# cboin1996/avddpg

Measured on AMD Instinct MI355X. Metric: env-steps/sec + DDPG updates/sec, 4096x5-vehicle platoons, higher is better.
Workload: dtype f32-class (fp16 hi+lo operand pairs on the 16-bit matrix cores, f32 accumulate)

## Files before the change

avddpg_amd/_hip.py:

```python
import ctypes as C
import os

_HERE = os.path.dirname(os.path.abspath(__file__))
LIB_PATH = os.path.join(_HERE, "lib", "libavddpg_hip.so")
if os.environ.get("AVDDPG_HIP_LIB"):
    LIB_PATH = os.path.abspath(os.environ["AVDDPG_HIP_LIB"])
HEADER_PATH = os.path.join(os.path.dirname(_HERE), "include", "avddpg_hip.h")
AVD_MAX_L = 16
AVD_EVAL_NMETRIC = 8


class AvdError(RuntimeError):
    pass


class EnvConsts(C.Structure):
    _fields_ = [("L", C.c_int32), ("model_a", C.c_int32), ("can_terminate", C.c_int32), ("uniform_reset", C.c_int32),
                ("max_ep", C.c_float), ("max_ev", C.c_float), ("abs_action_high", C.c_float),
                ("two_max_a", C.c_float), ("T", C.c_float),
                ("ca", C.c_float), ("cb", C.c_float), ("cc", C.c_float), ("cd", C.c_float),
                ("re_scalar", C.c_float), ("terminal_reward", C.c_float),
                ("stand_still", C.c_float), ("timegap", C.c_float),
                ("reset_ep_max", C.c_float), ("reset_max_ev", C.c_float), ("reset_max_a", C.c_float),
                ("reset_ep_eval", C.c_float), ("reset_ev_eval", C.c_float), ("reset_a_eval", C.c_float),
                ("leader_reset_a", C.c_float),
                ("A", (C.c_float * 16) * AVD_MAX_L), ("B", (C.c_float * 4) * AVD_MAX_L),
                ("C", (C.c_float * 4) * AVD_MAX_L)]


class HParams(C.Structure):
    _fields_ = [("actor_lr", C.c_float), ("critic_lr", C.c_float), ("tau", C.c_float), ("one_minus_tau", C.c_float),
                ("gamma", C.c_float), ("ou_theta", C.c_float), ("ou_scale", C.c_float), ("reserved", C.c_float)]


_LAYOUT_FIELDS = ["S", "A", "H1", "H2", "Ha", "B",
                  "aW1", "ab1", "ag1", "abe1", "aW2", "ab2", "ag2", "abe2", "aW3", "ab3", "actor_size",
                  "cWs", "cbs", "cgs", "cbes", "cWa", "cba", "cga", "cbea", "cW2", "cb2", "cg3", "cbe3", "cW3", "cb3",
                  "theta_size",
                  "amm1", "amv1", "amm2", "amv2", "cmms", "cmvs", "cmma", "cmva", "cmm3", "cmv3", "stats_size"]


class MlpLayout(C.Structure):
    _fields_ = [(n, C.c_int32) for n in _LAYOUT_FIELDS]


_P = C.c_void_p
_i, _f, _d, _u64, _i64 = C.c_int, C.c_float, C.c_double, C.c_uint64, C.c_int64
_LP = C.POINTER(MlpLayout)

_PROTOS = {
    "avd_mlp_layout_init": [_LP, _i, _i, _i, _i, _i, _i],
    "avd_env_step_f32": [_P, _i, _i, _P, _P, _P, _P, _P, _P, _P, _P, _P, _P, _P, _P],
    "avd_env_reset_f32": [_P, _i, _i, _P, _P, _P, _P, _P, _i, _u64, _u64, _P, _P],
    "avd_episode_end_f32": [_P, _i, _i, _i, _P, _P, _P, _P, _P, _P, _i, _P, _P, _P, _P, _i, _u64, _u64, _P],
    "avd_ou_step_f32": [_i, _P, _P, _f, _f, _f, _f, _u64, _u64, _P],
    "avd_policy_f32": [_i, _P, _P, _f, _f, _P, _P],
    "avd_normal_f32": [_i, _P, _f, _u64, _u64, _P],
    "avd_uniform_f32": [_i, _P, _f, _u64, _u64, _P],
    "avd_step_fused_f32": [_P, _i, _i, _i, _P, _P, _P, _P, _P, _P, _P, _P, _P, _P, _P, _P, _P, _f, _f, _f, _f, _f, _f, _f, _i, _u64, _u64,
                           _u64, _P, _i, _i64, _P, _P],
    "avd_replay_sample_f32": [_i, _i, _i, _i, _i, _P, _i, _u64, _u64, _P, _P, _P, _P, _P, _P],
    "avd_step_fused_seeds_f32": [_P, _i, _i, _i, _P, _P, _P, _P, _P, _P, _P, _P, _P, _P, _P, _P, _P, _f, _f, _f, _f, _f, _f, _f, _i, _P,
                                 _i, _u64, _u64, _P, _i, _i64, _P, _P],
    "avd_env_reset_seeds_f32": [_P, _i, _i, _P, _P, _P, _i, _P, _i, _u64, _P, _P],
    "avd_episode_end_seeds_f32": [_P, _i, _i, _i, _P, _P, _P, _P, _P, _P, _i, _P, _P, _P, _P, _i, _P, _i, _u64, _P],
    "avd_replay_sample_seeds_f32": [_i, _i, _i, _i, _i, _P, _i, _P, _i, _i, _u64, _P, _P, _P, _P, _P, _P],
    "avd_step_fused_hp_f32": [_P, _i, _i, _i, _P, _P, _P, _P, _P, _P, _P, _P, _P, _P, _P, _P, _P, _f, _f, _f, _f, _f, _i, _P, _P, _i,
                              _u64, _u64, _P, _i, _i64, _P, _P],
    "avd_learn_hp_f32": [_LP, _i, _i, _P, _P, _P, _P, _P, _P, _P, _P, _f, _P, _P, _P, _i, _i, _P],
    "avd_learn_update_hp_f32": [_LP, _i, _P, _P, _P, _P, _P, _P, _P, _P, _P, _P, _P, _P, _f, _P, _P, _P, _i, _i, _P],
    "avd_learn_update_act_hp_f32": [_LP, _i, _P, _P, _P, _P, _P, _P, _P, _P, _P, _P, _P, _P, _f, _P, _P, _P, _i, _P, _P, _i, _i, _P],
    "avd_adam_polyak_hp_f32": [_LP, _i, _P, _P, _P, _P, _P, _P, _P, _P, _P, _i, _i, _P],
    "avd_adam_polyak_guarded_hp_f32": [_LP, _i, _P, _P, _P, _P, _P, _P, _P, _P, _P, _P, _i, _i, _P],
    "avd_learn_set_split_hp_f16x3": [_LP, _i, _i, _P, _P, _P, _P, _P, _P, _P, _P, _P, _f, _P, _P, _P, C.c_size_t, _P, _i, _i, _P],
    "avd_actor_forward_set_f32": [_LP, _i, _i, _P, _P, _P, _i, _f, _P, _P, _P],
    "avd_copy_experiment_sets_f32": [_LP, _i, _i, _i, _P, _i, _P, _P, _P, _P, _P, _P, _P, _P],
    "avd_replay_add_f32": [_i, _i, _i, _i, _P, _i64, _P, _P, _i, _P, _P, _P],
    "avd_replay_indices": [_i, _i, _i, _u64, _u64, _P, _P],
    "avd_replay_gather_f32": [_i, _i, _i, _i, _i, _P, _P, _P, _P, _P, _P, _P],
    "avd_actor_forward_f32": [_LP, _i, _i, _P, _P, _P, _i, _f, _P, _P],
    "avd_actor_forward_cond_f32": [_LP, _i, _i, _P, _P, _P, _i, _f, _P, _P, _P],
    "avd_critic_forward_f32": [_LP, _i, _i, _P, _P, _P, _i, _P, _P, _P],
    "avd_learn_f32": [_LP, _i, _i, _P, _P, _P, _P, _P, _P, _P, _P, _f, _f, _P, _P, _P],
    "avd_learn_check_shape": [_LP],
    "avd_learn_update_f32": [_LP, _i, _P, _P, _P, _P, _P, _P, _P, _P, _P, _P, _P, _P, _f, _f, _f, _f, _d, _P, _P, _P],
    "avd_learn_update_act_f32": [_LP, _i, _P, _P, _P, _P, _P, _P, _P, _P, _P, _P, _P, _P, _f, _f, _f, _f, _d, _P, _P, _P, _i, _P, _P],
    "avd_learn_update_plan": [_LP, _i, C.POINTER(C.c_int), C.POINTER(C.c_int), C.POINTER(C.c_int)],
    "avd_adam_polyak_f32": [_LP, _i, _P, _P, _P, _P, _P, _P, _P, _P, _f, _f, _d, _P],
    "avd_adam_polyak_guarded_f32": [_LP, _i, _P, _P, _P, _P, _P, _P, _P, _P, _f, _f, _d, _P, _P],
    "avd_polyak_f32": [_i64, _P, _P, _d, _P],
    "avd_fed_sum_f32": [_i, _i, _i, _i, _i, _P, _P, _P, _P, _P],
    "avd_fed_finalize_f32": [_i, _i, _P, _f, _P, _P],
    "avd_fed_scatter_f32": [_i, _i, _i, _i, _i, _i, _P, _P, _P],
    "avd_adam_polyak_intra_f32": [_LP, _i, _i, _i, _P, _P, _P, _P, _P, _P, _P, _P, _P, _f, _f, _d, _P],
    "avd_fed_history_push_f32": [_i, _i, _i, _P, _P, _P, _i, _P, _i, _i, _P, _P, _P],
    "avd_fed_weights_f32": [_i, _i, _i, _P, _P, _i, _P, _P, _P, _P],
    "avd_learn_shared_workspace": [_LP, _i, _i, C.POINTER(C.c_size_t)],
    "avd_learn_shared_bf16": [_LP, _i, _i, _P, _P, _P, _P, _P, _P, _P, _P, _P, _f, _f, _P, _P, _P, C.c_size_t, _P],
    "avd_learn_set_fused_workspace": [_LP, _i, _i, C.POINTER(C.c_size_t)],
    "avd_learn_set_fused_bf16": [_LP, _i, _i, _P, _P, _P, _P, _P, _P, _P, _P, _P, _f, _f, _P, _P, _P, C.c_size_t, _P],
    "avd_learn_set_split_workspace": [_LP, _i, _i, C.POINTER(C.c_size_t)],
    "avd_learn_set_split_mfma_count": [_LP, _i, _i, C.POINTER(C.c_ulonglong)],
    "avd_learn_set_split_critic": [_LP, _i, _i, _P, _P, _P, _P, _P, _P, _P, _P, _P, _f, _f, _P, _P, _P, C.c_size_t, _P],
    "avd_learn_set_split_actor": [_LP, _i, _i, _P, _P, _P, _f, _P, _P, C.c_size_t, _P],
    "avd_learn_set_split_bf16x3": [_LP, _i, _i, _P, _P, _P, _P, _P, _P, _P, _P, _P, _f, _f, _P, _P, _P, C.c_size_t, _P],
    "avd_learn_set_split_f16x3": [_LP, _i, _i, _P, _P, _P, _P, _P, _P, _P, _P, _P, _f, _f, _P, _P, _P, C.c_size_t, _P],
    "avd_actor_forward_shared_workspace": [_LP, _i, _i, C.POINTER(C.c_size_t)],
    "avd_actor_forward_shared_bf16": [_LP, _i, _i, _P, _P, _P, _f, _P, _P, C.c_size_t, _P],
    "avd_eval_rollout_f32": [_LP, _P, _i, _i, _i, _i, _P, _P, _i, _P, _P, _P, _P, _i, _P, _f, _f, _f, _f, _P, _i, _P, _P, _P, _P,
                             _P],
    "avd_eval_cases_f32": [_LP, _P, _i, _i, _i, _i, _i, _P, _P, _i, _P, _P, _P, _P, _f, _f, _f, _f, _P, _P, _P],
    "avd_eval_cases_block": [_i, _i],
    "avd_gemm_bt_bf16": [_i, _i, _i, _P, C.c_long, _P, C.c_long, _P, C.c_long, _P],
}

_lib = None
DIAG_LIB_PATH = os.path.join(_HERE, "lib", "libavddpg_hip_diag.so")


def _load(path):
    if not os.path.exists(path):
        raise AvdError(f"{path} not found: build the HIP extension first (__graft_entry__.build()); "
                       "avddpg_amd has no CPU fallback")
    l = C.CDLL(path)
    missing = []
    for name, args in _PROTOS.items():
        fn = getattr(l, name, None)
        if fn is None:
            missing.append(name)
            continue
        fn.argtypes = args
        fn.restype = C.c_int
    if missing and not os.environ.get("AVDDPG_HIP_LIB"):
        raise AvdError(f"{path} does not export {', '.join(missing)}: rebuild it (make -C avddpg_amd/csrc)")
    l.avd_last_error.restype = C.c_char_p
    l.avd_last_error.argtypes = []
    l.avd_version.restype, l.avd_version.argtypes = C.c_int, []
    if getattr(l, "avd_diagnostics_enabled", None) is None:
        l.avd_diagnostics_enabled = lambda: 0
    else:
        l.avd_diagnostics_enabled.restype, l.avd_diagnostics_enabled.argtypes = C.c_int, []
    return l


def lib():
    global _lib
    if _lib is None:
        _lib = _load(LIB_PATH)
    return _lib


class diag_library:
    _cached = None
    _stack = []

    def __enter__(self):
        global _lib, LIB_PATH
        if diag_library._cached is None:
            diag_library._cached = _load(DIAG_LIB_PATH)
            if not diag_library._cached.avd_diagnostics_enabled():
                raise AvdError(f"{DIAG_LIB_PATH} is not a diagnostic build")
        diag_library._stack.append((lib(), LIB_PATH))
        _lib, LIB_PATH = diag_library._cached, DIAG_LIB_PATH
        return _lib

    def __exit__(self, *exc):
        global _lib, LIB_PATH
        _lib, LIB_PATH = diag_library._stack.pop()
        return False


def call(name, *args):
    fn = getattr(lib(), name, None)
    if fn is None:
        raise AvdError(f"{name} is not exported by the loaded library (an older build?)")
    rc = fn(*args)
    if rc != 0:
        raise AvdError(f"{name} failed ({rc}): {lib().avd_last_error().decode()}")


def ptr(t):
    if t is None:
        return None
    if not t.is_contiguous():
        raise AvdError("non-contiguous tensor passed to the C ABI")
    return C.c_void_p(t.data_ptr())


def stream_handle():
    import torch
    return C.c_void_p(torch.cuda.current_stream().cuda_stream)


def make_layout(S, A, H1, H2, Ha, B):
    lay = MlpLayout()
    call("avd_mlp_layout_init", C.byref(lay), S, A, H1, H2, Ha, B)
    return lay
```

avddpg_amd/csrc/fsplit.hip:

```cpp
#include <type_traits>

#include "fset_common.h"

namespace avd {
namespace fsplit {
using namespace fset;

struct ActorS {
    static constexpr int K = 256, KP = 256, NFT = 8, NKS = 16, LD = 264, NGT = 9, KG = 288;
    static constexpr bool critic = false;
};
struct CriticS {
    static constexpr int K = 304, KP = 320, NFT = 10, NKS = 19, LD = 312, NGT = 10, KG = 320;
    static constexpr bool critic = true;
};
constexpr int NGT_MAX = 10;

template <int I, int N, class F>
__device__ __forceinline__ void static_for(F&& f) {
    if constexpr (I < N) {
        f(std::integral_constant<int, I>{});
        static_for<I + 1, N>(f);
    }
}

typedef _Float16 f16;
typedef _Float16 f16x2 __attribute__((ext_vector_type(2)));
typedef _Float16 f16x8 __attribute__((ext_vector_type(8)));
constexpr float S1 = 64.f;
constexpr float F16_OVERFLOW = 65520.f;
#if defined(FSPLIT_ABL_CONST)
#define FSPLIT_ABL(x) FSPLIT_ABL_CONST
#elif defined(AVD_DIAG)
#define FSPLIT_ABL(x) (x)
#else
#define FSPLIT_ABL(x) 0
#endif
__device__ __forceinline__ void split2h(float a, float b, unsigned& hi, unsigned& lo) {
    const f32x2 f = {a, b};
    const f16x2 h = __builtin_convertvector(f, f16x2);
    hi = __builtin_bit_cast(unsigned, h);
    f32x2 l;
#ifdef __HIP_DEVICE_COMPILE__
    asm("v_fma_mix_f32 %0, -%1, 1.0, %2 op_sel:[0,0,0] op_sel_hi:[1,0,0]" : "=v"(l[0]) : "v"(hi), "v"(a));
    asm("v_fma_mix_f32 %0, -%1, 1.0, %2 op_sel:[1,0,0] op_sel_hi:[1,0,0]" : "=v"(l[1]) : "v"(hi), "v"(b));
#else
    l[0] = a - (float)h[0], l[1] = b - (float)h[1];
#endif
    lo = __builtin_bit_cast(unsigned, __builtin_convertvector(l, f16x2));
}
__device__ __forceinline__ void split1h(float x, f16& hi, f16& lo) {
    hi = (f16)x;
    lo = (f16)(x - (float)hi);
}
template <class V>
__device__ __forceinline__ void pin16(V& x) {
#pragma unroll
    for (int q = 0; q < 2; ++q) {
        float a = x[8 * q], b = x[8 * q + 1], c = x[8 * q + 2], d = x[8 * q + 3], e = x[8 * q + 4], f = x[8 * q + 5], g = x[8 * q + 6], h = x[8 * q + 7];
        asm volatile("" : "+v"(a), "+v"(b), "+v"(c), "+v"(d), "+v"(e), "+v"(f), "+v"(g), "+v"(h));
        x[8 * q] = a, x[8 * q + 1] = b, x[8 * q + 2] = c, x[8 * q + 3] = d, x[8 * q + 4] = e, x[8 * q + 5] = f, x[8 * q + 6] = g, x[8 * q + 7] = h;
    }
}
__device__ __forceinline__ f16x8 fragh(unsigned a, unsigned b, unsigned c, unsigned d) {
    uint4 o;
    o.x = a, o.y = b, o.z = c, o.w = d;
    return __builtin_bit_cast(f16x8, o);
}
__device__ __forceinline__ f32x16 mfmah(f16x8 a, f16x8 b, f32x16 c) {
    return __builtin_amdgcn_mfma_f32_32x32x16_f16(a, b, c, 0, 0, 0);
}
__device__ __forceinline__ f16x8 make_xh(float x0, float x1, float x2, float x3, int h) {
    f16 a0, a1, a2, a3, l0, l1, l2, l3;
    split1h(x0, a0, l0), split1h(x1, a1, l1), split1h(x2, a2, l2), split1h(x3, a3, l3);
    const f16 one = (f16)1.f, zero = (f16)0.f;
    f16x8 v;
    v[0] = a0, v[1] = a1, v[2] = a2, v[3] = a3;
    v[4] = h ? one : l0, v[5] = h ? one : l1, v[6] = h ? zero : l2, v[7] = h ? zero : l3;
    return v;
}
__device__ __forceinline__ f16x8 make_wh(float w0, float w1, float w2, float w3, float b, float sc, int h) {
    f16 a0, a1, a2, a3, l0, l1, l2, l3, bh, bl;
    split1h(sc * w0, a0, l0), split1h(sc * w1, a1, l1), split1h(sc * w2, a2, l2), split1h(sc * w3, a3, l3), split1h(sc * b, bh, bl);
    const f16 zero = (f16)0.f;
    f16x8 v;
    v[0] = h ? l0 : a0, v[1] = h ? l1 : a1, v[2] = h ? l2 : a2, v[3] = h ? l3 : a3;
    v[4] = h ? bh : a0, v[5] = h ? bl : a1, v[6] = h ? bh : a2, v[7] = h ? zero : a3;
    return v;
}
__device__ __forceinline__ f16x8 make_xg(float x0, float x1, float x2, float x3, float g, int h) {
    f16 a0, a1, a2, a3, l0, l1, l2, l3, gh, gl;
    split1h(x0, a0, l0), split1h(x1, a1, l1), split1h(x2, a2, l2), split1h(x3, a3, l3), split1h(g, gh, gl);
    const f16 zero = (f16)0.f;
    f16x8 v;
    v[0] = a0, v[1] = a1, v[2] = a2, v[3] = a3;
    v[4] = h ? gh : l0, v[5] = h ? gh : l1, v[6] = h ? gl : l2, v[7] = h ? zero : l3;
    return v;
}

template <int S>
__device__ __forceinline__ void load_x(const float* xa, long row, float (&x)[4]) {
    if (S == 4) {
        const float4 v = *(const float4*)(xa + 4 * row);
        x[0] = v.x, x[1] = v.y, x[2] = v.z, x[3] = v.w;
    } else {
#pragma unroll
        for (int k = 0; k < 4; ++k) x[k] = k < S ? xa[S * row + k] : 0.f;
    }
}

__host__ __device__ constexpr int wpos(int f) { return (f & ~12) | ((f & 4) << 1) | ((f & 8) >> 1); }

struct NetP {
    const float* th;
    long th_stride;
    const f16* Whi;
    const f16* Wlo;
    const f16* Wchi;
    const f16* Wclo;
    const f16x8* wf1h;
    const float* vec;
    const unsigned* wap;
};

struct PackArgs {
    const float* x[2];
    const float* extra[2];
    f16x8* outh[2];
    long rows;
};
__device__ __forceinline__ void front_flag(unsigned* wave_flags, bool hit) {
    const bool any = __ballot(hit) != 0;
    if ((threadIdx.x & 63) == 0) wave_flags[threadIdx.x >> 6] = any;
}
template <int S>
__device__ __forceinline__ void pack_x_role(const PackArgs& a, int which, long bx, unsigned* wave_flags) {
    const float* x = a.x[which];
    const float* extra = a.extra[which];
    const bool extra_is_action = which == 0;
    const long i = bx * 256 + threadIdx.x;
    bool nf = false;
    if (i < 2 * a.rows) {
        float v[4];
        load_x<S>(x, i >> 1, v);
        nf = not_finite(v[0]) || not_finite(v[1]) || not_finite(v[2]) || not_finite(v[3]);
        nf = nf || fmaxf(fmaxf(fabsf(v[0]), fabsf(v[1])), fmaxf(fabsf(v[2]), fabsf(v[3]))) >= F16_OVERFLOW;
        if (!(i & 1)) {
            const float e = extra[i >> 1];
            nf = nf || not_finite(e) || (extra_is_action && fabsf(e) >= F16_OVERFLOW);
        }
        a.outh[which][i] = make_xh(v[0], v[1], v[2], v[3], (int)(i & 1));
    }
    front_flag(wave_flags, nf);
}

struct PrepArgs {
    avd_mlp_layout L;
    int S;
    const float *theta, *stats, *theta_t, *stats_t;
    f16 *Whi[4], *Wlo[4];
    f16 *Wchi[4], *Wclo[4];
    f16x8* wf1h[4];
    float* vec[4];
    unsigned* wap;
    unsigned* smax;
    int* bad;
    unsigned* fflag;
    int n_fflag;
};
constexpr int SCALE_SLICES = 16;
__device__ __forceinline__ float pow2_for(float mx) {
    int e = 0;
    if (mx > 0.f && !not_finite(mx)) (void)frexpf(mx, &e);
    int k = 13 - e;
    k = k < -14 ? -14 : (k > 30 ? 30 : k);
    return ldexpf(1.f, k);
}
__device__ __forceinline__ void scale_role(const PrepArgs& a, int net, int set, int slice, int n_sets) {
    __shared__ float red[256], red2[256], c3a[H2], inva[CriticS::K];
    const int tid = threadIdx.x;
    const bool critic = net & 1, target = net >= 2;
    const avd_mlp_layout& L = a.L;
    const float* th = (target ? a.theta_t : a.theta) + (long)set * L.theta_size + (critic ? L.actor_size : 0);
    const float* st = (target ? a.stats_t : a.stats) + (long)set * L.stats_size;
    const int K = critic ? CriticS::K : ActorS::K, oW2 = critic ? L.cW2 : L.aW2;
    const int og2 = critic ? L.cg3 : L.ag2, omv2 = critic ? L.cmv3 : L.amv2, oW3 = critic ? L.cW3 : L.aW3;
    if (tid < H2) c3a[tid] = fabsf((1.0f / sqrtf(st[omv2 + tid] + BN_EPS)) * th[og2 + tid] * th[oW3 + tid]);
    for (int f = tid; f < K; f += 256) {
        int og, omv, ff = f;
        if (!critic) og = L.ag1, omv = L.amv1;
        else if (f < H1) og = L.cgs, omv = L.cmvs;
        else og = L.cga, omv = L.cmva, ff = f - H1;
        inva[f] = fabsf((1.0f / sqrtf(st[omv + ff] + BN_EPS)) * th[og + ff]);
    }
    __syncthreads();
    const int total = K * H2, per = (total + SCALE_SLICES - 1) / SCALE_SLICES, lo = slice * per, hi = min(total, lo + per);
    float m = 0.f, m2 = 0.f;
    for (int i = lo + tid; i < hi; i += 256) {
        const float w = fabsf(th[oW2 + i]);
        m = fmaxf(m, inva[i / H2] * w);
        m2 = fmaxf(m2, c3a[i % H2] * w);
    }
    red[tid] = m, red2[tid] = m2;
    __syncthreads();
    for (int o = 128; o > 0; o >>= 1) {
        if (tid < o) red[tid] = fmaxf(red[tid], red[tid + o]), red2[tid] = fmaxf(red2[tid], red2[tid + o]);
        __syncthreads();
    }
    if (tid == 0) {
        unsigned* dst = a.smax + (((long)net * n_sets + set) * SCALE_SLICES + slice) * 2;
        dst[0] = __float_as_uint(red[0]);
        dst[1] = __float_as_uint(red2[0]);
    }
}
__global__ __launch_bounds__(320) void prep_kernel(const PrepArgs a) {
    __shared__ float red[320];
    const int n = blockIdx.x, net = blockIdx.y, set = blockIdx.z, f = threadIdx.x;
    const bool critic = net & 1, target = net >= 2;
    const avd_mlp_layout& L = a.L;
    const float* th = (target ? a.theta_t : a.theta) + (long)set * L.theta_size + (critic ? L.actor_size : 0);
    const float* st = (target ? a.stats_t : a.stats) + (long)set * L.stats_size;
    const int K = critic ? CriticS::K : ActorS::K, KP = critic ? CriticS::KP : ActorS::KP;
    const int oW2 = critic ? L.cW2 : L.aW2, ob2 = critic ? L.cb2 : L.ab2, oW3 = critic ? L.cW3 : L.aW3, ob3 = critic ? L.cb3 : L.ab3;
    const int og2 = critic ? L.cg3 : L.ag2, obe2 = critic ? L.cbe3 : L.abe2, omm2 = critic ? L.cmm3 : L.amm2, omv2 = critic ? L.cmv3 : L.amv2;
    const float inv2n = (1.0f / sqrtf(st[omv2 + n] + BN_EPS)) * th[og2 + n], c3n = inv2n * th[oW3 + n];
    const unsigned* smax = a.smax + ((long)net * gridDim.z + set) * SCALE_SLICES * 2;
    unsigned mx = 0, mxc = 0;
#pragma unroll
    for (int sl = 0; sl < SCALE_SLICES; ++sl) mx = max(mx, smax[2 * sl]), mxc = max(mxc, smax[2 * sl + 1]);
    const float SW = pow2_for(__uint_as_float(mx)), SWC = pow2_for(__uint_as_float(mxc));
    if (net == 0 && set == 0)
        for (int w = n * 320 + f; w < a.n_fflag; w += H2 * 320)
            if (a.fflag[w]) atomicOr(a.bad, 1);
    float shw = 0.f;
    if (f < KP) {
        float w = 0.f, inv = 0.f;
        if (f < K) {
            int og, obe, omm, omv, ff = f;
            if (!critic) og = L.ag1, obe = L.abe1, omm = L.amm1, omv = L.amv1;
            else if (f < H1) og = L.cgs, obe = L.cbes, omm = L.cmms, omv = L.cmvs;
            else og = L.cga, obe = L.cbea, omm = L.cmma, omv = L.cmva, ff = f - H1;
            inv = (1.0f / sqrtf(st[omv + ff] + BN_EPS)) * th[og + ff];
            const float sh = th[obe + ff] - st[omm + ff] * inv;
            w = th[oW2 + (long)f * H2 + n];
            shw = sh * w;
            if (not_finite(w) || not_finite(inv) || not_finite(sh)) atomicOr(a.bad, 1);
            f16 hi, lo;
            const float ws = SW * (inv * w);
            if (fabsf(ws) >= F16_OVERFLOW) atomicOr(a.bad, 1);
            split1h(ws, hi, lo);
            const long at = ((long)set * H2 + n) * K + wpos(f);
            a.Whi[net][at] = hi, a.Wlo[net][at] = lo;
        }
        if (!target) {
            f16 hi, lo;
            const float wc = SWC * (c3n * w);
            if (fabsf(wc) >= F16_OVERFLOW) atomicOr(a.bad, 1);
            split1h(wc, hi, lo);
            const long at = ((long)set * KP + f) * H2 + n;
            a.Wchi[net][at] = hi, a.Wclo[net][at] = lo;
        }
    }
    red[f] = shw;
    __syncthreads();
    if (f < 64) red[f] += red[f + 256];
    __syncthreads();
    for (int o = 128; o > 0; o >>= 1) {
        if (f < o) red[f] += red[f + o];
        __syncthreads();
    }
    float* vec = a.vec[net] + (long)set * VEC;
    if (f == 0) {
        if (n == 0) vec[2 * H2 + 1] = SW, vec[2 * H2 + 2] = SWC;
        vec[n] = th[ob2 + n] + red[0];
        vec[H2 + n] = c3n;
        if (not_finite(vec[n]) || not_finite(c3n) || not_finite(th[ob3])) atomicOr(a.bad, 1);
    }
    if (n == 0) {
        __syncthreads();
        float v = 0.f;
        if (f < H2) {
            const float inv2 = (1.0f / sqrtf(st[omv2 + f] + BN_EPS)) * th[og2 + f];
            v = (th[obe2 + f] - st[omm2 + f] * inv2) * th[oW3 + f];
        }
        red[f] = v;
        __syncthreads();
        for (int o = 64; o > 0; o >>= 1) {
            if (f < o) red[f] += red[f + o];
            __syncthreads();
        }
        if (f == 0) vec[2 * H2] = th[ob3] + red[0];
    }
}
__device__ __forceinline__ bool prep1_role(const PrepArgs& a, int ft, int net, int set, int lane) {
    const int r = lane & 31, h = lane >> 5;
    bool hit = false;
    const bool critic = net & 1, target = net >= 2;
    const avd_mlp_layout& L = a.L;
    const float* th = (target ? a.theta_t : a.theta) + (long)set * L.theta_size + (critic ? L.actor_size : 0);
    const int K = critic ? CriticS::K : ActorS::K;
    const int f = 32 * ft + r;
    float w[4] = {0.f, 0.f, 0.f, 0.f}, b = 0.f;
    if (f == K) {
        b = 1.f;
    } else if (f < K) {
        if (critic && ft >= 8) {
            w[0] = th[L.cWa + (f - H1)], b = th[L.cba + (f - H1)];
        } else {
            const float* W = th + (critic ? L.cWs : L.aW1);
#pragma unroll
            for (int k = 0; k < 4; ++k) w[k] = k < a.S ? W[k * H1 + f] : 0.f;
            b = th[(critic ? L.cbs : L.ab1) + f];
        }
        if (not_finite(w[0]) || not_finite(w[1]) || not_finite(w[2]) || not_finite(w[3]) || not_finite(b)) hit = true;
        if (S1 * fmaxf(fmaxf(fabsf(w[0]), fabsf(w[1])), fmaxf(fmaxf(fabsf(w[2]), fabsf(w[3])), fabsf(b))) >= F16_OVERFLOW) hit = true;
    }
    a.wf1h[net][((long)set * NGT_MAX + ft) * 64 + lane] = make_wh(w[0], w[1], w[2], w[3], b, S1, h);
    if (net == 1 && ft == 0 && lane < 48) {
        const int hl = lane / 24, hh = (lane / 12) & 1, ks = (lane / 4) % 3, m = lane & 3;
        unsigned v = 0;
#pragma unroll
        for (int e = 0; e < 2; ++e) {
            const int jj = 2 * m + e, fa = 16 * ks + 8 * (jj >> 2) + 4 * hh + (jj & 3);
            f16 hi, lo;
            split1h(S1 * th[L.cWa + fa], hi, lo);
            v |= (unsigned)__builtin_bit_cast(unsigned short, hl ? lo : hi) << (16 * e);
        }
        a.wap[(long)set * 48 + lane] = v;
    }
    return hit;
}

struct FrontArgs {
    PrepArgs pa;
    PackArgs pk;
    float* grads;
    long n_grads;
    int n_sets, n_scale, n_prep1, n_zero, n_pack;
};
constexpr int ZERO_PER_BLOCK = 4096;
template <int S>
__global__ __launch_bounds__(256) void front_kernel(const FrontArgs a) {
    int b = blockIdx.x;
    if (b < a.n_scale) {
        scale_role(a.pa, b & 3, (b >> 2) % a.n_sets, (b >> 2) / a.n_sets, a.n_sets);
        return;
    }
    b -= a.n_scale;
    if (b < a.n_prep1) {
        const int q = 4 * b + (threadIdx.x >> 6);
        bool hit = false;
        if (q < NGT_MAX * 4 * a.n_sets) hit = prep1_role(a.pa, q % NGT_MAX, (q / NGT_MAX) & 3, q / (NGT_MAX * 4), threadIdx.x & 63);
        front_flag(a.pa.fflag + 4 * (long)b, hit);
        return;
    }
    b -= a.n_prep1;
    if (b < a.n_zero) {
        if (b == 0 && threadIdx.x == 0) *a.pa.bad = 0;
        const long base = (long)b * ZERO_PER_BLOCK + threadIdx.x;
#pragma unroll
        for (int k = 0; k < ZERO_PER_BLOCK / 256; ++k)
            if (base + 256 * k < a.n_grads) a.grads[base + 256 * k] = 0.f;
        return;
    }
    b -= a.n_zero;
    const int which = b >= a.n_pack;
    pack_x_role<S>(a.pk, which, b - which * a.n_pack, a.pa.fflag + 4 * ((long)a.n_prep1 + b));
}

enum HeadMode { OUT_TANH = 0, OUT_TD = 1, HEAD_BOTH = 5, OUT_TANH_SAVE = 6 };
struct HeadArgs {
    unsigned long long* stamp;
    NetP net;
    int n_agents, n_sets;
    const f16x8* xf;
    const float* act;
    const float* act2;
    const float* r;
    const float* yin;
    const float* aw;
    float* out;
    unsigned* sm;
    float* g3;
    float* dmu;
    float* part_s;
    float* part_s2;
    float* part_m;
    float* tz;
    float gamma, high, inv_n;
    int* bad;
    int abl;
};
#ifndef HEAD_FAST
#define HEAD_FAST 5
#define HEAD_SLOW 3
#endif

template <int S, class NET, int MODE, bool HP = false, class... H>
__global__ __launch_bounds__(NT) void head_kernel(const HeadArgs p, H... hp) {
    constexpr int K = NET::K, NKS = NET::NKS, NFT = NET::NFT, LD = NET::LD;
    constexpr int NTH = NT;
    constexpr bool BOTH = (MODE == HEAD_BOTH);
    static_assert(!BOTH || NET::critic, "HEAD_BOTH is a critic mode");
    __shared__ __attribute__((aligned(16))) f16 wimg[2][H2 * LD];
    __shared__ __attribute__((aligned(16))) float b2s[H2];
    __shared__ __attribute__((aligned(16))) float c3s[H2];
    __shared__ __attribute__((aligned(16))) unsigned waps[BOTH ? 48 : 4];
    const int tid = threadIdx.x, w = tid >> 6, lane = tid & 63, r = lane & 31, h = lane >> 5, q = w >> 1, rh = w & 1;
    const int set = blockIdx.x % p.n_sets, j0 = blockIdx.x / p.n_sets, J = gridDim.x / p.n_sets, P = p.n_agents / p.n_sets;
    for (int i = tid; i < 2 * H2 * (K / 8); i += NTH) {
        const int hl = i / (H2 * (K / 8)), rem = i - hl * (H2 * (K / 8)), n = rem / (K / 8), c = rem - n * (K / 8);
        const f16* src = (hl ? p.net.Wlo : p.net.Whi) + ((long)set * H2 + n) * K + 8 * c;
        *(uint4*)(&wimg[hl][n * LD + 8 * c]) = *(const uint4*)src;
    }
    const float* vec = p.net.vec + (long)set * VEC;
    const float SW = vec[2 * H2 + 1], sc = SW * S1, isc = 1.f / sc;
    if (tid < H2) b2s[tid] = vec[tid] * sc, c3s[tid] = vec[H2 + tid] * isc;
    if (BOTH && tid < 48) waps[tid] = p.net.wap[(long)set * 48 + tid];
    const float d3 = vec[2 * H2];
    const f16x8* wf1 = p.net.wf1h + (long)set * NGT_MAX * 64 + lane;
    const f32x16 zero16 = {};
#ifdef AVD_STAMP
    unsigned long long hacc[4] = {0, 0, 0, 0}, hlast = __builtin_amdgcn_s_memtime();
    const unsigned long long hstart = hlast;
#define HSTAMP(i) { const unsigned long long t_ = __builtin_amdgcn_s_memtime(); hacc[i] += t_ - hlast; hlast = t_; }
#else
#define HSTAMP(i)
#endif
    float Dacc = 0.f, Lacc = 0.f, Dacc2 = 0.f, Lacc2 = 0.f, gmax = 0.f;
    unsigned watch = 0;
    auto look = [&](float x) {
        unsigned u = __float_as_uint(x);
        asm volatile("" : "+v"(u));
        u &= 0x7fffffffu;
        watch = watch > u ? watch : u;
    };
    __syncthreads();

    const int ntile = j0 < P ? (P - j0 + J - 1) / J : 0;
    const int row = 32 * rh + r;
    f16x8 nx = {};
    float na = 0.f, nb = 0.f, ny = 0.f, nw = 1.f;
    auto fetch_in = [&](int k) {
        const int agent = (j0 + k * J) * p.n_sets + set;
        const long ri = (long)agent * TILE + row;
        nx = p.xf[2 * ri + h];
        if (NET::critic) na = p.act[ri];
        if (BOTH) nb = p.act2[ri];
        if (MODE == OUT_TD) ny = p.r[ri];
        if (BOTH) ny = p.yin[ri];
        if (BOTH && p.aw) nw = p.aw[agent];
    };
    const f16* whi0 = &wimg[0][r * LD + 8 * h];
    const f16* wlo0 = &wimg[1][r * LD + 8 * h];
    constexpr int NSEQ = BOTH ? 8 : NFT;
    HSTAMP(3);
    constexpr int FAST = HEAD_FAST, SLOW = HEAD_SLOW, PERIOD = 2 * (FAST + SLOW);
    const int qs = __builtin_amdgcn_readfirstlane(q);
    const int cnt = qs < 2 ? FAST : SLOW, start = qs < 2 ? qs * FAST : 2 * FAST + (qs - 2) * SLOW;
    int k = start, pos = 0;
    auto next_tile = [&](int kk, int pp) { return pp + 1 == cnt ? kk + PERIOD - cnt + 1 : kk + 1; };
    if (k < ntile) fetch_in(k);
    for (int ui = 0; k < ntile; ++ui, k = next_tile(k, pos), pos = pos + 1 == cnt ? 0 : pos + 1) {
        const int agent = (j0 + k * J) * p.n_sets + set;
        const long ri = (long)agent * TILE + row;
        const f16x8 xs = nx, xa = make_xh(na, 0.f, 0.f, 0.f, h), xb = BOTH ? make_xh(nb, 0.f, 0.f, 0.f, h) : xa;
        const float ty = ny, tw = nw;
        if (next_tile(k, pos) < ntile) fetch_in(next_tile(k, pos));
        f32x16 acc[4];
#pragma unroll
        for (int t = 0; t < 4; ++t)
#pragma unroll
            for (int g = 0; g < 4; ++g) {
                const float4 b = *(const float4*)(b2s + 32 * t + 8 * g + 4 * h);
                acc[t][4 * g] = b.x, acc[t][4 * g + 1] = b.y, acc[t][4 * g + 2] = b.z, acc[t][4 * g + 3] = b.w;
            }
        unsigned ph[8], pl[8];
        auto split16 = [&](const f32x16& p1) {
            if (FSPLIT_ABL(p.abl) & 4) {
#pragma unroll
                for (int m = 0; m < 8; ++m) ph[m] = __float_as_uint(p1[2 * m]), pl[m] = __float_as_uint(p1[2 * m + 1]);
                return;
            }
#pragma unroll
            for (int m = 0; m < 8; ++m) split2h(relu(p1[2 * m]), relu(p1[2 * m + 1]), ph[m], pl[m]);
        };
        auto zdot_t = [&](f32x16& a, int t) {
            float zp = 0.f;
#pragma unroll
            for (int g = 0; g < 4; ++g) {
                const float4 c = *(const float4*)(c3s + 32 * t + 8 * g + 4 * h);
                const float cc[4] = {c.x, c.y, c.z, c.w};
#pragma unroll
                for (int j = 0; j < 4; ++j) {
                    a[4 * g + j] = relu(a[4 * g + j]);
                    zp = fmaf(a[4 * g + j], cc[j], zp);
                }
            }
            return zp;
        };
        auto zdot_nd = [&](const f32x16& a, int t) {
            float zp = 0.f;
#pragma unroll
            for (int g = 0; g < 4; ++g) {
                const float4 c = *(const float4*)(c3s + 32 * t + 8 * g + 4 * h);
                const float cc[4] = {c.x, c.y, c.z, c.w};
#pragma unroll
                for (int j = 0; j < 4; ++j) zp = fmaf(relu(a[4 * g + j]), cc[j], zp);
            }
            return zp;
        };
        auto mask_t = [&](const f32x16& a) {
            unsigned b = 0;
#pragma unroll
            for (int g = 0; g < 4; ++g)
#pragma unroll
                for (int j = 0; j < 4; ++j) b |= a[4 * g + j] > 0.f ? 1u << (4 * g + (j >> 1) + 16 * (j & 1)) : 0u;
            return b;
        };
        auto mask_store = [&](const unsigned (&b)[4], unsigned* dst) {
            const auto s0 = __builtin_amdgcn_permlane32_swap(b[0], b[2], false, false);
            const auto s1 = __builtin_amdgcn_permlane32_swap(b[1], b[3], false, false);
            uint2 o;
            o.x = s0[0] | (s0[1] << 2), o.y = s1[0] | (s1[1] << 2);
            *(uint2*)(dst + 2 * h) = o;
        };
        auto out_z = [&](f32x16 (&ac)[4]) {
            float zp = 0.f;
#pragma unroll
            for (int t = 0; t < 4; ++t) zp += zdot_t(ac[t], t);
            zp += __shfl_xor(zp, 32);
            return d3 + zp;
        };
        split16(mfmah(wf1[0], xs, zero16));
        f16x8 wfn = wf1[64];
        f16x8 wg[2][2][2];
        auto read_group = [&](int g, f16x8 (&dst)[2][2]) {
            const int ks = g >> 1, th = g & 1;
#pragma unroll
            for (int tt = 0; tt < 2; ++tt) {
                dst[tt][0] = *(const f16x8*)(whi0 + 32 * (2 * th + tt) * LD + 16 * ks);
                dst[tt][1] = *(const f16x8*)(wlo0 + 32 * (2 * th + tt) * LD + 16 * ks);
            }
        };
        read_group(0, wg[0]);
        auto tile = [&](auto si_c, f32x16 (&ac)[4]) {
            constexpr int si = decltype(si_c)::value;
            constexpr int ft = si;
            f32x16 p1n = zero16;
            if constexpr (si + 1 < NSEQ) {
                p1n = mfmah(wfn, (NET::critic && si + 1 >= 8) ? xa : xs, zero16);
                if constexpr (si + 2 < NSEQ) wfn = wf1[64 * (si + 2)];
            }
#pragma unroll
            for (int s = 0; s < 2; ++s) {
                const int ks = 2 * ft + s;
                if (ks >= NKS) continue;
                const f16x8 bhi = fragh(ph[4 * s], ph[4 * s + 1], ph[4 * s + 2], ph[4 * s + 3]);
                const f16x8 blo = fragh(pl[4 * s], pl[4 * s + 1], pl[4 * s + 2], pl[4 * s + 3]);
#pragma unroll
                for (int th = 0; th < 2; ++th) {
                    const int g = 2 * ks + th;
                    if (g + 1 < 2 * (BOTH ? 16 : NKS)) read_group(g + 1, wg[(g + 1) & 1]);
#pragma unroll
                    for (int tt = 0; tt < 2; ++tt) {
                        const int t = 2 * th + tt;
                        const f16x8 whi = wg[g & 1][tt][0], wlo = wg[g & 1][tt][1];
                        ac[t] = mfmah(whi, bhi, ac[t]);
                        ac[t] = mfmah(wlo, bhi, ac[t]);
                        ac[t] = mfmah(whi, blo, ac[t]);
                    }
                }
            }
            if constexpr (si + 1 < NSEQ) split16(p1n);
            __builtin_amdgcn_sched_group_barrier(0x008, 1, 0);
#pragma unroll
            for (int gi = 0; gi < 4; ++gi) {
                __builtin_amdgcn_sched_group_barrier(0x100, 4, 0);
#pragma unroll
                for (int i = 0; i < 6; ++i) {
                    __builtin_amdgcn_sched_group_barrier(0x008, 1, 0);
                    __builtin_amdgcn_sched_group_barrier(0x002, 3, 0);
                }
            }
            __builtin_amdgcn_sched_barrier(0);
        };
        HSTAMP(0);
        static_for<0, NSEQ>([&](auto si_c) { tile(si_c, acc); });
        HSTAMP(1);
        if constexpr (BOTH) {
            f16x8 fh[3], fl[3];
            auto act_sweep = [&](f32x16 (&c)[4]) {
                f16x8 wq[2][2][2];
                read_group(2 * 16, wq[0]);
#pragma unroll
                for (int g = 0; g < 6; ++g) {
                    if (g + 1 < 6) read_group(2 * 16 + g + 1, wq[(g + 1) & 1]);
#pragma unroll
                    for (int tt = 0; tt < 2; ++tt) {
                        const int t = 2 * (g & 1) + tt;
                        const f16x8 whi = wq[g & 1][tt][0], wlo = wq[g & 1][tt][1];
                        c[t] = mfmah(whi, fh[g >> 1], c[t]);
                        c[t] = mfmah(wlo, fh[g >> 1], c[t]);
                        c[t] = mfmah(whi, fl[g >> 1], c[t]);
                    }
                }
            };
#pragma unroll
            for (int tl = 0; tl < 2; ++tl) {
                const f32x16 p1 = mfmah(wf1[64 * (8 + tl)], xa, zero16);
                split16(p1);
#pragma unroll
                for (int ss = 0; ss < 2 - tl; ++ss) {
                    fh[2 * tl + ss] = fragh(ph[4 * ss], ph[4 * ss + 1], ph[4 * ss + 2], ph[4 * ss + 3]);
                    fl[2 * tl + ss] = fragh(pl[4 * ss], pl[4 * ss + 1], pl[4 * ss + 2], pl[4 * ss + 3]);
                }
            }
            act_sweep(acc);
            look(acc[0][0]);
            {
                float zp = 0.f;
#pragma unroll
                for (int t = 0; t < 4; ++t) zp += zdot_nd(acc[t], t);
                zp += __shfl_xor(zp, 32);
                const float diff = d3 + zp - ty, g3a = 2.f * diff * p.inv_n * tw;
                if (h == 0) p.g3[ri] = g3a, Dacc += g3a, Lacc += diff * diff;
                gmax = fmaxf(gmax, fabsf(g3a));
                unsigned mb[4];
#pragma unroll
                for (int t = 0; t < 4; ++t) mb[t] = mask_t(acc[t]);
                mask_store(mb, p.sm + ri * 4);
            }
            __builtin_amdgcn_sched_barrier(0);
            f16x8 mh[3], ml[3];
#pragma unroll
            for (int tl = 0; tl < 2; ++tl) {
                const f32x16 pa = mfmah(wf1[64 * (8 + tl)], xa, zero16), pm = mfmah(wf1[64 * (8 + tl)], xb, zero16);
                unsigned dh[8], dl[8], mk[8];
#pragma unroll
                for (int m = 0; m < 4 * (2 - tl); ++m) {
                    split2h(relu(pm[2 * m]) - relu(pa[2 * m]), relu(pm[2 * m + 1]) - relu(pa[2 * m + 1]), dh[m], dl[m]);
                    mk[m] = (pm[2 * m] > 0.f ? 0xffffu : 0u) | (pm[2 * m + 1] > 0.f ? 0xffff0000u : 0u);
                }
#pragma unroll
                for (int ss = 0; ss < 2 - tl; ++ss) {
                    const int kk = 2 * tl + ss;
                    fh[kk] = fragh(dh[4 * ss], dh[4 * ss + 1], dh[4 * ss + 2], dh[4 * ss + 3]);
                    fl[kk] = fragh(dl[4 * ss], dl[4 * ss + 1], dl[4 * ss + 2], dl[4 * ss + 3]);
                    const uint4 ch = *(const uint4*)(waps + (0 * 2 + h) * 12 + 4 * kk), cl = *(const uint4*)(waps + (1 * 2 + h) * 12 + 4 * kk);
                    mh[kk] = fragh(ch.x & mk[4 * ss], ch.y & mk[4 * ss + 1], ch.z & mk[4 * ss + 2], ch.w & mk[4 * ss + 3]);
                    ml[kk] = fragh(cl.x & mk[4 * ss], cl.y & mk[4 * ss + 1], cl.z & mk[4 * ss + 2], cl.w & mk[4 * ss + 3]);
                }
            }
            act_sweep(acc);
            look(acc[0][0]);
            float zq = 0.f;
            unsigned pos[2] = {0u, 0u};
#pragma unroll
            for (int t = 0; t < 4; ++t) {
                zq += zdot_nd(acc[t], t);
#pragma unroll
                for (int i = 0; i < 16; ++i) pos[t >> 1] |= acc[t][i] > 0.f ? 1u << (16 * (t & 1) + i) : 0u;
            }
            zq += __shfl_xor(zq, 32);
            asm volatile("" : "+v"(pos[0]), "+v"(pos[1]));
#pragma unroll
            for (int kk = 0; kk < 3; ++kk) fh[kk] = mh[kk], fl[kk] = ml[kk];
#pragma unroll
            for (int t = 0; t < 4; ++t) acc[t] = zero16;
            act_sweep(acc);
// ... 345 lines not shown
    const float* g3;
    const float* part_m;
    const unsigned* sm;
    float* partV;
    int abl;
    unsigned long long* stamp;
};
template <int S, class NET>
__global__ __launch_bounds__(NT) void dx_kernel(const DxArgs p) {
    constexpr int KP = NET::KP, LDZ = 136;
    constexpr float VSH = 1.f / 32.f;
    __shared__ __attribute__((aligned(16))) f16 smimg[2][TILE * LDZ];
    __shared__ __attribute__((aligned(16))) f16 xt[3][2][32 * 32];
    __shared__ __attribute__((aligned(16))) float g3s[3][TILE];
    __shared__ float gred[8];
    const int tid = threadIdx.x, w = __builtin_amdgcn_readfirstlane(tid >> 6), lane = tid & 63, r = lane & 31, h = lane >> 5, ft = w;
    const int set = blockIdx.x % p.n_sets, j0 = blockIdx.x / p.n_sets, J = gridDim.x / p.n_sets, P = p.n_agents / p.n_sets;
    const f32x16 zero16 = {};
    const float gsc = set_gscale(p.part_m, set, p.n_sets, J, gred);
    f16x8 wch[8], wcl[8];
    {
        const long at = ((long)set * KP + 32 * ft + r) * H2 + 8 * h;
#pragma unroll
        for (int s = 0; s < 8; ++s) wch[s] = *(const f16x8*)(p.net.Wchi + at + 16 * s), wcl[s] = *(const f16x8*)(p.net.Wclo + at + 16 * s);
    }
    const float swc = __uint_as_float(__builtin_amdgcn_readfirstlane(__float_as_uint(p.net.vec[(long)set * VEC + 2 * H2 + 2])));
    const float gv = gsc * VSH, vs = gsc * swc * VSH;
    const f16x8 wf = p.net.wf1h[((long)set * NGT_MAX + ft) * 64 + lane];
    f32x16 V = zero16;
    for (int i = tid; i < 3 * 2 * 32 * 32; i += NT) {
        const int k = (i >> 5) & 31;
        (&xt[0][0][0])[i] = (f16)(k == 8 ? 1.f : 0.f);
    }
    const int srow = tid >> 3, sch = tid & 7;
    unsigned dm = 0;
    float gn = 0.f, gs = 0.f;
    auto fetch = [&](int pl) {
        if (FSPLIT_ABL(p.abl) & 1) pl = j0;
        const long agent = (long)pl * p.n_sets + set;
        dm = p.sm[(agent * TILE + srow) * 4 + (sch >> 1)];
        if (NET::critic) gs = p.g3[agent * TILE + srow];
        if (tid < TILE) gn = p.g3[agent * TILE + tid];
    };
    auto stage = [&](int buf, int slot) {
        uint4* dst = (uint4*)(smimg[buf] + srow * LDZ + 16 * sch);
        mask_chunk16(dm, sch, mask_one(gs, NET::critic), dst[0], dst[1]);
        if (tid < TILE) g3s[slot][tid] = (NET::critic ? fabsf(gn) : gn) * gv;
    };
    f16x8 xfn0 = {}, xfn1 = {};
    auto fetch_x = [&](int pl) {
        const long agent = (long)pl * p.n_sets + set;
        xfn0 = p.xfh[(agent * TILE + r) * 2 + h];
        xfn1 = p.xfh[(agent * TILE + 32 + r) * 2 + h];
    };
    auto stage_x = [&](int slot) {
        if (w < 2 && h == 0) {
            f16x8 src = xfn0;
            if (w == 1) src = xfn1;
            asm volatile("" : "+v"(src));
#pragma unroll
            for (int k = 0; k < 8; ++k) xt[slot][w][k * 32 + r] = src[k];
        }
    };
#ifdef AVD_STAMP
    unsigned long long dacc[4] = {0, 0, 0, 0}, dlast = __builtin_amdgcn_s_memtime();
#define DXSTAMP(i) { const unsigned long long t_ = __builtin_amdgcn_s_memtime(); dacc[i] += t_ - dlast; dlast = t_; }
#else
#define DXSTAMP(i)
#endif
    auto read_a = [&](int buf, int e, f16x8 (&smf)[8]) {
        const f16* arow = smimg[buf] + (32 * e + r) * LDZ + 8 * h;
#pragma unroll
        for (int s = 0; s < 8; ++s) smf[s] = *(const f16x8*)(arow + 16 * s);
    };
    typedef _Float16 f16x4 __attribute__((ext_vector_type(4)));
    auto read_img = [&](const f16* img, f16x8 (&xb)[2]) {
#pragma unroll
        for (int s = 0; s < 2; ++s) {
            const f16x4 lo = *(const f16x4*)(img + r * 32 + 16 * s + 4 * h);
            const f16x4 hi = *(const f16x4*)(img + r * 32 + 16 * s + 8 + 4 * h);
#pragma unroll
            for (int j = 0; j < 4; ++j) xb[s][j] = lo[j], xb[s][4 + j] = hi[j];
        }
    };
    auto dc_product = [&](const f16x8 (&smf)[8]) {
        f32x16 dc = zero16;
#pragma unroll
        for (int s = 0; s < 8; ++s) dc = mfmah(smf[s], wch[s], dc), dc = mfmah(smf[s], wcl[s], dc);
        return dc;
    };
    auto backward = [&](int slot, int e, const f32x16& dc, const f32x16& p1, unsigned (&vh)[8], unsigned (&vl)[8]) {
        if (FSPLIT_ABL(p.abl) & 4) {
#pragma unroll
            for (int m = 0; m < 8; ++m) vh[m] = __float_as_uint(dc[2 * m]) ^ __float_as_uint(p1[2 * m]), vl[m] = __float_as_uint(dc[2 * m + 1]);
            return;
        }
#pragma unroll
        for (int g = 0; g < 4; ++g) {
            const float4 gq = *(const float4*)(&g3s[slot][32 * e + 8 * g + 4 * h]);
            const float gg[4] = {gq.x, gq.y, gq.z, gq.w};
            float dm[4];
#pragma unroll
            for (int j = 0; j < 4; ++j) {
                const int k = 4 * g + j;
                dm[j] = p1[k] > 0.f ? dc[k] * gg[j] : 0.f;
            }
            split2h(dm[0], dm[1], vh[2 * g], vl[2 * g]);
            split2h(dm[2], dm[3], vh[2 * g + 1], vl[2 * g + 1]);
        }
    };
    auto v_product = [&](const unsigned (&vh)[8], const unsigned (&vl)[8], const f16x8 (&xb)[2]) {
#pragma unroll
        for (int s = 0; s < 2; ++s) {
            V = mfmah(fragh(vh[4 * s], vh[4 * s + 1], vh[4 * s + 2], vh[4 * s + 3]), xb[s], V);
            V = mfmah(fragh(vl[4 * s], vl[4 * s + 1], vl[4 * s + 2], vl[4 * s + 3]), xb[s], V);
        }
    };
    f16x8 xf0, xf1;
    f32x16 dc1 = zero16, p11 = zero16;
    auto iteration = [&](auto has_prev_c, int pi, int buf, int slot) {
        constexpr bool has_prev = decltype(has_prev_c)::value;
        const int pslot = slot == 0 ? 2 : slot - 1, nslot = slot == 2 ? 0 : slot + 1;
        const int nn = pi + 2 * J < P ? pi + 2 * J : (pi + J < P ? pi + J : pi);
        DXSTAMP(0);
        f16x8 smf[8], xb0[2], xb1[2];
        unsigned vh0[8], vl0[8], vh1[8], vl1[8];
        read_a(buf, 0, smf);
        const f32x16 dc0 = dc_product(smf);
        const f32x16 p10 = mfmah(xf0, wf, zero16);
        if constexpr (has_prev) {
            read_img(xt[pslot][1], xb1);
            backward(pslot, 1, dc1, p11, vh1, vl1);
            __builtin_amdgcn_sched_group_barrier(0x100, 12, 0);
#pragma unroll
            for (int i = 0; i < 17; ++i) {
                __builtin_amdgcn_sched_group_barrier(0x008, 1, 0);
                __builtin_amdgcn_sched_group_barrier(0x002, 5, 0);
                __builtin_amdgcn_sched_group_barrier(0x100, 1, 0);
            }
        }
        __builtin_amdgcn_sched_barrier(0);
        DXSTAMP(1);
        if constexpr (has_prev) v_product(vh1, vl1, xb1);
        read_a(buf, 1, smf);
        read_img(xt[slot][0], xb0);
        dc1 = dc_product(smf);
        p11 = mfmah(xf1, wf, zero16);
        backward(slot, 0, dc0, p10, vh0, vl0);
        stage(buf ^ 1, nslot);
        stage_x(nslot);
        xf0 = xfn0, xf1 = xfn1;
        fetch(nn), fetch_x(nn);
        __builtin_amdgcn_sched_group_barrier(0x100, 16, 0);
#pragma unroll
        for (int i = 0; i < (has_prev ? 21 : 17); ++i) {
            __builtin_amdgcn_sched_group_barrier(0x008, 1, 0);
            __builtin_amdgcn_sched_group_barrier(0x002, 6, 0);
            __builtin_amdgcn_sched_group_barrier(0x200, 1, 0);
        }
        __builtin_amdgcn_sched_barrier(0);
        v_product(vh0, vl0, xb0);
        DXSTAMP(2);
        if (!(FSPLIT_ABL(p.abl) & 2)) __syncthreads();
        DXSTAMP(3);
    };
    __syncthreads();
    if (j0 < P) {
        fetch(j0), fetch_x(j0), stage(0, 0), stage_x(0);
        xf0 = xfn0, xf1 = xfn1;
        const int n1 = j0 + J < P ? j0 + J : j0;
        fetch(n1), fetch_x(n1);
    }
    __syncthreads();
    if (j0 < P) {
        iteration(std::false_type{}, j0, 0, 0);
        int buf = 1, slot = 1, pi = j0 + J;
        for (; pi < P; pi += J, buf ^= 1, slot = slot == 2 ? 0 : slot + 1) iteration(std::true_type{}, pi, buf, slot);
        const int pslot = slot == 0 ? 2 : slot - 1;
        f16x8 xb1[2];
        unsigned vh1[8], vl1[8];
        read_img(xt[pslot][1], xb1);
        backward(pslot, 1, dc1, p11, vh1, vl1);
        v_product(vh1, vl1, xb1);
    }
#ifdef AVD_STAMP
    if (p.stamp && blockIdx.x == 16 && lane == 0)
        for (int i = 0; i < 4; ++i) p.stamp[w * 8 + i] = dacc[i];
#endif
    const float ivs = 1.f / vs;
    if (r < 16) {
        float* pv = p.partV + ((long)blockIdx.x * KP + 32 * ft) * 16 + r;
#pragma unroll
        for (int k = 0; k < 16; ++k) pv[(long)acc_row(k, h) * 16] = V[k] * ivs;
    }
}

template <int S>
__global__ __launch_bounds__(NT) void dxa_kernel(const DxArgs p) {
    typedef CriticS NET;
    constexpr int KP = NET::KP;
    constexpr float VSH = 1.f / 32.f;
    __shared__ __attribute__((aligned(16))) float ga[8][2][2][32];
    __shared__ float comb[8][64][2];
    __shared__ float gred[8];
    const int tid = threadIdx.x, w = __builtin_amdgcn_readfirstlane(tid >> 6), lane = tid & 63, r = lane & 31, h = lane >> 5;
    const int rh = w & 1, ftl = (w >> 1) & 1, par = w >> 2;
    const int set = blockIdx.x % p.n_sets, j0 = blockIdx.x / p.n_sets, J = gridDim.x / p.n_sets, P = p.n_agents / p.n_sets;
    const f32x16 zero16 = {};
    const int ft = 8 + ftl, f = 32 * ftl + r;
    const float gsc = set_gscale(p.part_m, set, p.n_sets, J, gred);
    f16x8 wch[8], wcl[8];
    {
        const long at = ((long)set * KP + 32 * ft + r) * H2 + 8 * h;
#pragma unroll
        for (int s = 0; s < 8; ++s) wch[s] = *(const f16x8*)(p.net.Wchi + at + 16 * s), wcl[s] = *(const f16x8*)(p.net.Wclo + at + 16 * s);
    }
    const float swc = __uint_as_float(__builtin_amdgcn_readfirstlane(__float_as_uint(p.net.vec[(long)set * VEC + 2 * H2 + 2])));
    const float gv = gsc * VSH, vs = gsc * swc * VSH;
    const float* th = p.net.th + (long)set * p.net.th_stride;
    const float wa = f < HA ? th[p.L_cWa + f] : 0.f, ba = f < HA ? th[p.L_cba + f] : 0.f;
    float Sa = 0.f, Sb = 0.f;
    const int ntile = j0 < P ? (P - j0 + J - 1) / J : 0;
    uint4 mA = {}, mB = {};
    float gA = 0.f, aA = 0.f, gB = 0.f, aB = 0.f;
#define DXA_FETCH(k_, m_, g_, a_)                                                                                   \
    {                                                                                                               \
        const long r0_ = (long)((j0 + (k_) * J) * p.n_sets + set) * TILE + 32 * rh;                                 \
        m_ = *(const uint4*)(p.sm + (r0_ + r) * 4);                                                                 \
        g_ = p.g3[r0_ + r], a_ = p.act[r0_ + r];                                                                    \
    }
#define DXA_PUT(buf_, g_, a_)                                                                                       \
    {                                                                                                               \
        if (h == 0) ga[w][buf_][0][r] = fabsf(g_) * gv, ga[w][buf_][1][r] = a_;                                     \
        __builtin_amdgcn_fence(__ATOMIC_RELEASE, "wavefront");                                                      \
        __builtin_amdgcn_wave_barrier();                                                                            \
    }
    auto unit = [&](int buf, const uint4 mw, float g) {
        f32x16 dc = zero16;
        const unsigned m = mask_one(g, true);
        const unsigned mwt[4] = {mw.x >> (4 * h), mw.y >> (4 * h), mw.z >> (4 * h), mw.w >> (4 * h)};
#pragma unroll
        for (int s = 0; s < 8; ++s) {
            const unsigned d = mwt[s >> 1] >> (8 * (s & 1));
            const f16x8 af = fragh(mask_pair(d, 0, m), mask_pair(d, 1, m >> 1), mask_pair(d, 2, m >> 2), mask_pair(d, 3, m >> 3));
            dc = mfmah(af, wch[s], dc), dc = mfmah(af, wcl[s], dc);
        }
        float sa = 0.f, sb = 0.f;
#pragma unroll
        for (int q = 0; q < 4; ++q) {
            const float4 gq = *(const float4*)(&ga[w][buf][0][8 * q + 4 * h]), aq = *(const float4*)(&ga[w][buf][1][8 * q + 4 * h]);
            const float gg[4] = {gq.x, gq.y, gq.z, gq.w}, av[4] = {aq.x, aq.y, aq.z, aq.w};
#pragma unroll
            for (int j = 0; j < 4; ++j) {
                const float m = fmaf(av[j], wa, ba) > 0.f ? dc[4 * q + j] * gg[j] : 0.f;
                sa = fmaf(m, av[j], sa);
                sb += m;
            }
        }
        Sa += sa, Sb += sb;
        __builtin_amdgcn_fence(__ATOMIC_ACQ_REL, "wavefront");
        __builtin_amdgcn_wave_barrier();
    };
    if (par < ntile) DXA_FETCH(par, mA, gA, aA);
    if (par + 2 < ntile) DXA_FETCH(par + 2, mB, gB, aB);
    for (int k = par; k < ntile; k += 4) {
        DXA_PUT(0, gA, aA);
        {
            const uint4 mc = mA;
            const float gc = gA;
            if (k + 4 < ntile) DXA_FETCH(k + 4, mA, gA, aA);
            unit(0, mc, gc);
        }
        if (k + 2 < ntile) {
            DXA_PUT(1, gB, aB);
            const uint4 mc = mB;
            const float gc = gB;
            if (k + 6 < ntile) DXA_FETCH(k + 6, mB, gB, aB);
            unit(1, mc, gc);
        }
    }
#undef DXA_FETCH
#undef DXA_PUT
    comb[w][lane][0] = Sa, comb[w][lane][1] = Sb;
    __syncthreads();
    if (rh == 0 && par == 0 && h == 0) {
        const int ws[4] = {w, w + 1, w + 4, w + 5};
        float t[2] = {0.f, 0.f};
#pragma unroll
        for (int i = 0; i < 4; ++i)
#pragma unroll
            for (int c = 0; c < 2; ++c) t[c] += comb[ws[i]][r][c] + comb[ws[i]][32 + r][c];
        const float ivs = 1.f / vs;
        float* pv = p.partV + ((long)blockIdx.x * KP + 32 * ft + r) * 16;
#pragma unroll
        for (int c = 0; c < 9; ++c) pv[c] = c == 0 ? t[0] * ivs : (c == 8 ? t[1] * ivs : 0.f);
    }
}

struct Plan {
    int grid, J;
    size_t Whi[4], Wlo[4], Wchi[2], Wclo[2], wf1h[4], vec[4], wap, a2, y, mu, dmu, g3, sm, sma, tz, t1p, s2raw, xfs, xfs2, partHs[3], partM[2],
        partV[2], partG[2], bad, smax, fflag, total;
    int n_prep1, n_pack, n_fflag;
};
static Plan make_plan(int n_agents, int n_sets) {
    Plan pl;
    const int P = n_agents / n_sets;
    int J = cu_count() / n_sets;
    if (const char* e = AVD_DIAG_ENV("FSPLIT_J")) J = atoi(e);
    if (J < 1) J = 1;
    if (J > P) J = P;
    pl.J = J, pl.grid = J * n_sets;
    size_t o = 0;
    auto take = [&](size_t bytes) {
        const size_t at = o;
        o += (bytes + 255) / 256 * 256;
        return at;
    };
    for (int i = 0; i < 4; ++i) {
        const int K = (i & 1) ? CriticS::K : ActorS::K, KP = (i & 1) ? CriticS::KP : ActorS::KP;
        pl.Whi[i] = take(sizeof(f16) * (size_t)n_sets * H2 * K), pl.Wlo[i] = take(sizeof(f16) * (size_t)n_sets * H2 * K);
        pl.vec[i] = take(sizeof(float) * (size_t)n_sets * VEC);
        pl.wf1h[i] = take(16 * (size_t)n_sets * NGT_MAX * 64);
        if (i < 2) pl.Wchi[i] = take(sizeof(f16) * (size_t)n_sets * KP * H2), pl.Wclo[i] = take(sizeof(f16) * (size_t)n_sets * KP * H2);
    }
    pl.wap = take(4 * (size_t)n_sets * 48);
    const size_t rows = (size_t)n_agents * TILE;
    pl.a2 = take(4 * rows), pl.y = take(4 * rows), pl.mu = take(4 * rows), pl.dmu = take(4 * rows), pl.g3 = take(4 * rows);
    pl.sm = take(16 * rows);
    pl.sma = take(16 * rows);
    pl.tz = take(4 * rows);
    pl.t1p = take(2 * 4 * (size_t)n_sets * CriticS::K * H2), pl.s2raw = take(2 * 4 * (size_t)n_sets * H2);
    pl.xfs = take(32 * rows), pl.xfs2 = take(32 * rows);
    for (int i = 0; i < 2; ++i) {
        const int KP = i ? CriticS::KP : ActorS::KP, KG = i ? CriticS::KG : ActorS::KG;
        pl.partM[i] = take(4 * (size_t)pl.grid * 8);
        pl.partV[i] = take(4 * (size_t)pl.grid * KP * 16);
        pl.partG[i] = take(4 * (size_t)pl.grid * KG * H2);
    }
    for (int i = 0; i < 3; ++i) pl.partHs[i] = take(4 * (size_t)pl.grid * 8 * 2);
    pl.n_prep1 = (NGT_MAX * 4 * n_sets + 3) / 4, pl.n_pack = (int)((2 * rows + 255) / 256);
    pl.n_fflag = 4 * (pl.n_prep1 + 2 * pl.n_pack);
    pl.bad = take(sizeof(int));
    pl.smax = take(sizeof(unsigned) * 4 * (size_t)n_sets * SCALE_SLICES * 2);
    pl.fflag = take(sizeof(unsigned) * (size_t)pl.n_fflag);
    pl.total = o;
    return pl;
}
static int check_shape(const avd_mlp_layout* L, int n_agents, int n_sets, const char* who) {
    AVD_REQUIRE(L, "%s: null layout", who);
    if (L->H1 != H1 || L->H2 != H2 || L->Ha != HA || L->A != 1 || (L->S != 3 && L->S != 4) || L->B != TILE) {
        set_error("%s: serves the reference widths only (layer1 256, layer2 128, action layer 48, A = 1, S in {3, 4}, B = 64); "
                  "got H1=%d H2=%d Ha=%d A=%d S=%d B=%d (avd_learn_shared_bf16 takes other widths)",
                  who, L->H1, L->H2, L->Ha, L->A, L->S, L->B);
        return AVD_E_UNSUPPORTED;
    }
    AVD_REQUIRE(n_sets > 0 && n_sets <= 64 && n_agents > 0 && n_agents % n_sets == 0, "%s: n_agents=%d n_sets=%d", who, n_agents,
                n_sets);
    return AVD_OK;
}

enum Phase { PH_CRITIC = 1, PH_ACTOR = 2, PH_BOTH = 3 };
template <int S, class... H>
static int run(int phases, const avd_mlp_layout& L, int n_agents, int n_sets, const float* theta, const float* stats, const float* theta_t,
               const float* stats_t, const float* s, const float* a, const float* r, const float* s2, const float* aw, float gamma,
               float high, float* grads, float* losses, unsigned char* ws, const Plan& pl, hipStream_t st, H... hp) {
    PrepArgs pa;
    pa.L = L, pa.S = S, pa.theta = theta, pa.stats = stats, pa.theta_t = theta_t, pa.stats_t = stats_t;
    pa.wap = (unsigned*)(ws + pl.wap), pa.bad = (int*)(ws + pl.bad), pa.smax = (unsigned*)(ws + pl.smax);
    pa.fflag = (unsigned*)(ws + pl.fflag), pa.n_fflag = pl.n_fflag;
    NetP net[4];
    for (int i = 0; i < 4; ++i) {
        const bool critic = i & 1, target = i >= 2;
        pa.Whi[i] = (f16*)(ws + pl.Whi[i]), pa.Wlo[i] = (f16*)(ws + pl.Wlo[i]), pa.vec[i] = (float*)(ws + pl.vec[i]);
        pa.wf1h[i] = (f16x8*)(ws + pl.wf1h[i]);
        pa.Wchi[i] = i < 2 ? (f16*)(ws + pl.Wchi[i]) : nullptr, pa.Wclo[i] = i < 2 ? (f16*)(ws + pl.Wclo[i]) : nullptr;
        NetP& n = net[i];
        n.th = (target ? theta_t : theta) + (critic ? L.actor_size : 0), n.th_stride = L.theta_size;
        n.Whi = pa.Whi[i], n.Wlo = pa.Wlo[i], n.Wchi = pa.Wchi[i], n.Wclo = pa.Wclo[i], n.wf1h = pa.wf1h[i], n.vec = pa.vec[i];
        n.wap = pa.wap;
    }
    const int P = n_agents / n_sets;
    const float inv_n = 1.0f / ((float)P * TILE);
    const long nrows = (long)n_agents * TILE;
    f16x8 *xfs = (f16x8*)(ws + pl.xfs), *xfs2 = (f16x8*)(ws + pl.xfs2);
    int* bad = (int*)(ws + pl.bad);
    float *a2 = (float*)(ws + pl.a2), *y = (float*)(ws + pl.y), *mu = (float*)(ws + pl.mu), *dmu = (float*)(ws + pl.dmu);
    float* g3 = (float*)(ws + pl.g3);
    unsigned *sm = (unsigned*)(ws + pl.sm), *sma = (unsigned*)(ws + pl.sma);
    auto F = [&](size_t off) { return (float*)(ws + off); };
    const dim3 grid(pl.grid), block(NT);
    HeadArgs h;
    h.n_agents = n_agents, h.n_sets = n_sets, h.gamma = gamma, h.high = high, h.inv_n = inv_n, h.aw = aw, h.sm = sm, h.g3 = g3, h.dmu = dmu;
    h.act2 = nullptr, h.part_s2 = nullptr, h.stamp = nullptr, h.bad = bad, h.part_m = nullptr, h.tz = F(pl.tz), h.abl = 0;
    if (const char* e = AVD_DIAG_ENV("FSPLIT_ABL")) h.abl = atoi(e);
    auto head = [&](auto kern, int ni, const f16x8* x, const float* act, const float* rr, const float* yin, float* out, float* part_s,
                    auto... extra) {
        h.net = net[ni], h.xf = x, h.act = act, h.r = rr, h.yin = yin, h.out = out, h.part_s = part_s;
        hipLaunchKernelGGL(kern, grid, block, 0, st, h, extra...);
    };
    DwArgs dw;
    dw.n_agents = n_agents, dw.n_sets = n_sets, dw.sm = sm, dw.g3 = g3, dw.x = s, dw.stamp = nullptr, dw.abl = 0;
    if (const char* e = AVD_DIAG_ENV("FSPLIT_ABL")) dw.abl = atoi(e);
#ifdef AVD_STAMP
    static unsigned long long* d_stamp = nullptr;
    if (!d_stamp) (void)hipMalloc(&d_stamp, 128 * 8);
    dw.stamp = d_stamp;
#endif
    DxArgs dx;
    dx.n_agents = n_agents, dx.n_sets = n_sets, dx.sm = sm, dx.g3 = g3, dx.xfh = xfs, dx.stamp = nullptr, dx.L_cWa = dx.L_cba = 0;
    dx.abl = dw.abl;
#ifdef AVD_STAMP
    dx.stamp = d_stamp;
#endif
    FinArgs fa;
    fa.L = L, fa.n_sets = n_sets, fa.J = pl.J, fa.S = S, fa.nrh = 1, fa.theta = theta, fa.stats = stats, fa.grads = grads, fa.losses = losses;
    fa.inv_n = inv_n, fa.partLa = F(pl.partHs[2]), fa.bad = bad;
    for (int i = 0; i < 2; ++i)
        fa.partH[i] = nullptr, fa.partHs[i] = F(pl.partHs[i]), fa.partU[i] = nullptr, fa.partV[i] = F(pl.partV[i]),
        fa.partG[i] = F(pl.partG[i]), fa.c3[i] = F(pl.vec[i]);
    fa.t1_from_g[0] = fa.t1_from_g[1] = 1, fa.t1p = F(pl.t1p), fa.s2raw = F(pl.s2raw);
    if (phases & PH_CRITIC) {
        FrontArgs fr;
        fr.pa = pa, fr.grads = grads, fr.n_grads = (long)n_sets * L.theta_size, fr.n_sets = n_sets;
        fr.pk.x[0] = s, fr.pk.extra[0] = a, fr.pk.outh[0] = xfs, fr.pk.x[1] = s2, fr.pk.extra[1] = r, fr.pk.outh[1] = xfs2, fr.pk.rows = nrows;
        fr.n_scale = 4 * n_sets * SCALE_SLICES, fr.n_prep1 = pl.n_prep1, fr.n_pack = pl.n_pack;
        fr.n_zero = (int)((fr.n_grads + ZERO_PER_BLOCK - 1) / ZERO_PER_BLOCK);
        hipLaunchKernelGGL(front_kernel<S>, dim3((unsigned)(fr.n_scale + fr.n_prep1 + fr.n_zero + 2 * fr.n_pack)), dim3(256), 0, st, fr);
        hipLaunchKernelGGL(prep_kernel, dim3(H2, 4, n_sets), dim3(320), 0, st, pa);
        head(head_kernel<S, ActorS, OUT_TANH>, 2, xfs2, nullptr, nullptr, nullptr, a2, nullptr);
        if constexpr (sizeof...(H) > 0)
            head(head_kernel<S, CriticS, OUT_TD, true, H...>, 3, xfs2, a2, r, nullptr, y, nullptr, hp...);
        else
            head(head_kernel<S, CriticS, OUT_TD>, 3, xfs2, a2, r, nullptr, y, nullptr);
        h.sm = sma;
        head(head_kernel<S, ActorS, OUT_TANH_SAVE>, 0, xfs, nullptr, nullptr, nullptr, mu, nullptr);
        h.sm = sm;
        h.act2 = mu, h.part_s2 = F(pl.partHs[2]), h.part_m = F(pl.partM[1]);
        head(head_kernel<S, CriticS, HEAD_BOTH>, 1, xfs, a, nullptr, y, nullptr, F(pl.partHs[1]));
        dw.net = net[1], dw.act = a, dw.partG = F(pl.partG[1]), dw.part_m = F(pl.partM[1]);
        hipLaunchKernelGGL((dw_kernel<S, CriticS>), grid, block, 0, st, dw);
        dx.net = net[1], dx.partV = F(pl.partV[1]), dx.act = a, dx.part_m = F(pl.partM[1]);
        hipLaunchKernelGGL((dx_kernel<S, CriticS>), grid, block, 0, st, dx);
        dx.L_cWa = L.cWa, dx.L_cba = L.cba;
        hipLaunchKernelGGL((dxa_kernel<S>), grid, block, 0, st, dx);
        if (phases == PH_CRITIC) launch_finalize(fa, st, 1, 1);
    }
    if (phases & PH_ACTOR) {
        SeedArgs sd;
        sd.n_agents = n_agents, sd.n_sets = n_sets, sd.dmu = dmu, sd.tz = F(pl.tz), sd.high = high, sd.g3 = g3, sd.part_m = F(pl.partM[0]),
        sd.part_s = F(pl.partHs[0]);
        hipLaunchKernelGGL(actor_seed_kernel, grid, block, 0, st, sd);
        dw.sm = sma, dx.sm = sma;
        dw.net = net[0], dw.act = nullptr, dw.partG = F(pl.partG[0]), dw.part_m = F(pl.partM[0]);
        hipLaunchKernelGGL((dw_kernel<S, ActorS>), grid, block, 0, st, dw);
        dx.net = net[0], dx.partV = F(pl.partV[0]), dx.act = nullptr, dx.part_m = F(pl.partM[0]), dx.L_cWa = dx.L_cba = 0;
        hipLaunchKernelGGL((dx_kernel<S, ActorS>), grid, block, 0, st, dx);
        if (phases == PH_ACTOR) launch_finalize(fa, st, 0, 1);
        else launch_finalize(fa, st, 0, 2);
    }
    return check_launch("avd_learn_set_split");
}

}
}

using namespace avd;

namespace avd { namespace fsplit {
constexpr long MFMA_PER_TILE = 2 * (200 + 238 + 200 + 314)
                               + 8 * (2 + 32 + 1 + 2 * 2 * 2)
                               + 8 * (2 + 32 + 1 + 2 * 1 * 2)
                               + 2 * 8 * (32 + 2 + 8)
                               + 4 * 16;
static_assert(MFMA_PER_TILE == 3296, "update DESIGN.md 3.4 and the count above together");
}}
extern "C" int avd_learn_set_split_mfma_count(const avd_mlp_layout* lay, int n_agents, int n_sets, unsigned long long* mfma_32x32x16) {
    int rc = fsplit::check_shape(lay, n_agents, n_sets, "avd_learn_set_split_mfma_count");
    if (rc) return rc;
    AVD_REQUIRE(mfma_32x32x16, "avd_learn_set_split_mfma_count: null pointer");
    *mfma_32x32x16 = (unsigned long long)fsplit::MFMA_PER_TILE * (unsigned long long)n_agents;
    return AVD_OK;
}

extern "C" int avd_learn_set_split_workspace(const avd_mlp_layout* lay, int n_agents, int n_sets, size_t* bytes) {
    int rc = fsplit::check_shape(lay, n_agents, n_sets, "avd_learn_set_split_workspace");
    if (rc) return rc;
    AVD_REQUIRE(bytes, "avd_learn_set_split_workspace: null pointer");
    *bytes = fsplit::make_plan(n_agents, n_sets).total;
    return AVD_OK;
}

template <class... H>
static int split_entry(int phases, const char* who, const avd_mlp_layout* lay, int n_agents, int n_sets, const float* theta, const float* stats,
                       const float* theta_t, const float* stats_t, const float* s, const float* a, const float* r, const float* s2,
                       const float* agent_weight, float gamma, float high, float* grads, float* losses, void* workspace,
                       size_t workspace_bytes, void* stream, H... hp) {
    int rc = fsplit::check_shape(lay, n_agents, n_sets, who);
    if (rc) return rc;
    const bool cr = phases & fsplit::PH_CRITIC;
    AVD_REQUIRE(theta && stats && s && grads && workspace && (!cr || (theta_t && stats_t && a && r && s2)), "%s: null pointer", who);
    const fsplit::Plan pl = fsplit::make_plan(n_agents, n_sets);
    AVD_REQUIRE(workspace_bytes >= pl.total, "%s: workspace %zu B < %zu B", who, workspace_bytes, pl.total);
    if (lay->S == 4)
        return fsplit::run<4>(phases, *lay, n_agents, n_sets, theta, stats, theta_t, stats_t, s, a, r, s2, agent_weight, gamma, high, grads,
                              losses, (unsigned char*)workspace, pl, (hipStream_t)stream, hp...);
    return fsplit::run<3>(phases, *lay, n_agents, n_sets, theta, stats, theta_t, stats_t, s, a, r, s2, agent_weight, gamma, high, grads, losses,
                          (unsigned char*)workspace, pl, (hipStream_t)stream, hp...);
}

extern "C" int avd_learn_set_split_f16x3(const avd_mlp_layout* lay, int n_agents, int n_sets, const float* theta, const float* stats,
                                          const float* theta_t, const float* stats_t, const float* s, const float* a, const float* r,
                                          const float* s2, const float* agent_weight, float gamma, float high, float* grads,
                                          float* losses, void* workspace, size_t workspace_bytes, void* stream) {
    return split_entry(fsplit::PH_BOTH, "avd_learn_set_split_f16x3", lay, n_agents, n_sets, theta, stats, theta_t, stats_t, s, a, r, s2,
                       agent_weight, gamma, high, grads, losses, workspace, workspace_bytes, stream);
}

extern "C" int avd_learn_set_split_hp_f16x3(const avd_mlp_layout* lay, int n_agents, int n_sets, const float* theta, const float* stats,
                                            const float* theta_t, const float* stats_t, const float* s, const float* a, const float* r,
                                            const float* s2, const float* agent_weight, float high, float* grads, float* losses,
                                            void* workspace, size_t workspace_bytes, const avd_hparams* d_hp, int n_groups, int set_block,
                                            void* stream) {
    AVD_REQUIRE_HP("avd_learn_set_split_hp_f16x3", d_hp, n_groups, set_block, n_sets);
    return split_entry(fsplit::PH_BOTH, "avd_learn_set_split_hp_f16x3", lay, n_agents, n_sets, theta, stats, theta_t, stats_t, s, a, r, s2,
                       agent_weight, 0.f, high, grads, losses, workspace, workspace_bytes, stream, HpRef{d_hp, n_groups, set_block});
}

extern "C" int avd_learn_set_split_bf16x3(const avd_mlp_layout* lay, int n_agents, int n_sets, const float* theta, const float* stats,
                                          const float* theta_t, const float* stats_t, const float* s, const float* a, const float* r,
                                          const float* s2, const float* agent_weight, float gamma, float high, float* grads,
                                          float* losses, void* workspace, size_t workspace_bytes, void* stream) {
    return avd_learn_set_split_f16x3(lay, n_agents, n_sets, theta, stats, theta_t, stats_t, s, a, r, s2, agent_weight, gamma, high, grads,
                                     losses, workspace, workspace_bytes, stream);
}

extern "C" int avd_learn_set_split_critic(const avd_mlp_layout* lay, int n_agents, int n_sets, const float* theta, const float* stats,
                                          const float* theta_t, const float* stats_t, const float* s, const float* a, const float* r,
                                          const float* s2, const float* agent_weight, float gamma, float high, float* grads,
                                          float* losses, void* workspace, size_t workspace_bytes, void* stream) {
    return split_entry(fsplit::PH_CRITIC, "avd_learn_set_split_critic", lay, n_agents, n_sets, theta, stats, theta_t, stats_t, s, a, r, s2,
                       agent_weight, gamma, high, grads, losses, workspace, workspace_bytes, stream);
}

extern "C" int avd_learn_set_split_actor(const avd_mlp_layout* lay, int n_agents, int n_sets, const float* theta, const float* stats,
                                         const float* s, float high, float* grads, void* workspace, size_t workspace_bytes, void* stream) {
    return split_entry(fsplit::PH_ACTOR, "avd_learn_set_split_actor", lay, n_agents, n_sets, theta, stats, nullptr, nullptr, s, nullptr, nullptr,
                       nullptr, nullptr, 0.f, high, grads, nullptr, workspace, workspace_bytes, stream);
}
```

avddpg_amd/csrc/replay.hip:

```cpp
#include "common.h"

namespace avd {

__global__ void replay_add_kernel(int n_agents, int cap, int S, int A, float* __restrict__ ring, int slot,
                                  const float* __restrict__ s_prev, const float* __restrict__ s_next, int x_stride,
                                  const float* __restrict__ action, const float* __restrict__ reward) {
    const int row = 2 * S + A + 1;
    const long t = (long)blockIdx.x * blockDim.x + threadIdx.x;
    if (t >= (long)n_agents * row) return;
    const int a = (int)(t / row);
    const int j = (int)(t - (long)a * row);
    float val;
    if (j < S)
        val = s_prev[(long)a * x_stride + j];
    else if (j < S + A)
        val = action[(long)a * A + (j - S)];
    else if (j == S + A)
        val = reward[a];
    else
        val = s_next[(long)a * x_stride + (j - S - A - 1)];
    ring[((long)a * cap + slot) * row + j] = val;
}

__global__ void replay_indices_kernel(int n_agents, int B, uint32_t range, uint64_t seed, uint64_t counter,
                                      int32_t* __restrict__ idx) {
    const long t = (long)blockIdx.x * blockDim.x + threadIdx.x;
    const long total = (long)n_agents * B;
    const long base = t * 4;
    if (base >= total) return;
    const u32x4 r = philox_at(seed, counter, (uint32_t)t, STREAM_REPLAY);
    const uint32_t w[4] = {r.x, r.y, r.z, r.w};
#pragma unroll
    for (int k = 0; k < 4; ++k)
        if (base + k < total) idx[base + k] = (int32_t)(((uint64_t)w[k] * range) >> 32);
}

__global__ void replay_gather_kernel(int n_agents, int cap, int S, int A, int B, const float* __restrict__ ring,
                                     const int32_t* __restrict__ idx, float* __restrict__ s, float* __restrict__ a,
                                     float* __restrict__ r, float* __restrict__ s2) {
    const int row = 2 * S + A + 1;
    const long t = (long)blockIdx.x * blockDim.x + threadIdx.x;
    const long total = (long)n_agents * B * row;
    if (t >= total) return;
    const long ab = t / row;
    const int j = (int)(t - ab * row);
    const int ag = (int)(ab / B);
    const int ix = idx[ab];
    const float val = ring[((long)ag * cap + ix) * row + j];
    if (j < S)
        s[ab * S + j] = val;
    else if (j < S + A)
        a[ab * A + (j - S)] = val;
    else if (j == S + A)
        r[ab] = val;
    else
        s2[ab * S + (j - S - A - 1)] = val;
}

template <int S, bool G>
__global__ __launch_bounds__(256) void replay_sample_kernel(int n_agents, int cap, int B, const float* __restrict__ ring,
                                                            uint32_t range, uint64_t seed, uint64_t counter,
                                                            int32_t* __restrict__ idx, float* __restrict__ s,
                                                            float* __restrict__ a, float* __restrict__ r,
                                                            float* __restrict__ s2, const uint64_t* __restrict__ seeds, int E,
                                                            int M) {
    constexpr int row = 2 * S + 2;
    const long t = (long)blockIdx.x * blockDim.x + threadIdx.x;
    const long total = (long)n_agents * B, base = t * 4;
    if (base >= total) return;
    const int ag = (int)(base / B);
    uint64_t key = seed;
    uint32_t ti = (uint32_t)t;
    if constexpr (G) {
        const int g = ag / M, e = g % E;
        key = seeds[e];
        ti = (uint32_t)(((long)(g / E) * M + (ag - g * M)) * (B / 4) + (base - (long)ag * B) / 4);
    }
    const u32x4 rr = philox_at(key, counter, ti, STREAM_REPLAY);
    const uint32_t w[4] = {rr.x, rr.y, rr.z, rr.w};
    int ix[4];
    float v[4][row];
#pragma unroll
    for (int k = 0; k < 4; ++k) {
        ix[k] = (int32_t)(((uint64_t)w[k] * range) >> 32);
        const float2* src = (const float2*)(ring + ((long)ag * cap + ix[k]) * row);
#pragma unroll
        for (int j = 0; j < row / 2; ++j) {
            const float2 q = src[j];
            v[k][2 * j] = q.x, v[k][2 * j + 1] = q.y;
        }
    }
    *(int4*)(idx + base) = make_int4(ix[0], ix[1], ix[2], ix[3]);
    *(float4*)(a + base) = make_float4(v[0][S], v[1][S], v[2][S], v[3][S]);
    *(float4*)(r + base) = make_float4(v[0][S + 1], v[1][S + 1], v[2][S + 1], v[3][S + 1]);
#pragma unroll
    for (int k = 0; k < 4; ++k) {
        if (S == 4) {
            *(float4*)(s + (base + k) * 4) = make_float4(v[k][0], v[k][1], v[k][2], v[k][3]);
            *(float4*)(s2 + (base + k) * 4) = make_float4(v[k][6], v[k][7], v[k][8], v[k][9]);
        } else {
#pragma unroll
            for (int j = 0; j < S; ++j) s[(base + k) * S + j] = v[k][j], s2[(base + k) * S + j] = v[k][S + 2 + j];
        }
    }
}

}

using namespace avd;

template <bool G>
static int replay_sample_launch(const char* who, int n_agents, int cap, int S, int A, int B, const float* ring, int range, uint64_t seed,
                                const uint64_t* d_seeds, int n_groups, int M, uint64_t counter, int32_t* idx, float* s, float* a,
                                float* r, float* s2, void* stream) {
    AVD_REQUIRE(n_agents > 0 && cap > 0 && (S == 3 || S == 4) && A == 1 && B > 0 && B % 4 == 0 && range > 0 && range <= cap,
                "%s: n=%d cap=%d S=%d A=%d B=%d range=%d (S in {3, 4}, A = 1, B a multiple of 4)", who, n_agents, cap, S, A, B, range);
    AVD_REQUIRE(ring && idx && s && a && r && s2, "%s: null pointer", who);
    const long calls = (long)n_agents * B / 4;
    const dim3 grid((unsigned)((calls + 255) / 256));
    if (S == 4)
        hipLaunchKernelGGL((replay_sample_kernel<4, G>), grid, dim3(256), 0, (hipStream_t)stream, n_agents, cap, B, ring, (uint32_t)range,
                           seed, counter, idx, s, a, r, s2, d_seeds, n_groups, M);
    else
        hipLaunchKernelGGL((replay_sample_kernel<3, G>), grid, dim3(256), 0, (hipStream_t)stream, n_agents, cap, B, ring, (uint32_t)range,
                           seed, counter, idx, s, a, r, s2, d_seeds, n_groups, M);
    return check_launch(who);
}

extern "C" int avd_replay_sample_f32(int n_agents, int cap, int S, int A, int B, const float* ring, int range, uint64_t seed,
                                     uint64_t counter, int32_t* idx, float* s, float* a, float* r, float* s2, void* stream) {
    return replay_sample_launch<false>("avd_replay_sample_f32", n_agents, cap, S, A, B, ring, range, seed, nullptr, 1, 1, counter, idx, s,
                                       a, r, s2, stream);
}

extern "C" int avd_replay_sample_seeds_f32(int n_agents, int cap, int S, int A, int B, const float* ring, int range,
                                           const uint64_t* d_seeds, int n_groups, int agents_per_platoon, uint64_t counter, int32_t* idx,
                                           float* s, float* a, float* r, float* s2, void* stream) {
    AVD_REQUIRE(d_seeds && n_groups >= 1 && agents_per_platoon >= 1 && n_agents > 0 &&
                    n_agents % ((long)n_groups * agents_per_platoon) == 0,
                "avd_replay_sample_seeds_f32: d_seeds=%p n_groups=%d agents_per_platoon=%d n=%d (n must be a multiple of "
                "n_groups x agents_per_platoon)", (const void*)d_seeds, n_groups, agents_per_platoon, n_agents);
    return replay_sample_launch<true>("avd_replay_sample_seeds_f32", n_agents, cap, S, A, B, ring, range, 0, d_seeds, n_groups,
                                      agents_per_platoon, counter, idx, s, a, r, s2, stream);
}

extern "C" int avd_replay_add_f32(int n_agents, int cap, int S, int A, float* ring, int64_t counter,
                                  const float* s_prev, const float* s_next, int x_stride, const float* action,
                                  const float* reward, void* stream) {
    AVD_REQUIRE(n_agents > 0 && cap > 0 && S > 0 && A > 0 && counter >= 0 && x_stride >= S,
                "avd_replay_add_f32: n=%d cap=%d S=%d A=%d counter=%ld x_stride=%d", n_agents, cap, S, A, (long)counter,
                x_stride);
    AVD_REQUIRE(ring && s_prev && s_next && action && reward, "avd_replay_add_f32: null pointer");
    const int slot = (int)(counter % cap);
    const long total = (long)n_agents * (2 * S + A + 1);
    hipLaunchKernelGGL(replay_add_kernel, dim3((unsigned)((total + 255) / 256)), dim3(256), 0, (hipStream_t)stream,
                       n_agents, cap, S, A, ring, slot, s_prev, s_next, x_stride, action, reward);
    return check_launch("avd_replay_add_f32");
}

extern "C" int avd_replay_indices(int n_agents, int B, int range, uint64_t seed, uint64_t counter, int32_t* idx,
                                  void* stream) {
    AVD_REQUIRE(n_agents > 0 && B > 0 && range > 0 && idx, "avd_replay_indices: n=%d B=%d range=%d", n_agents, B,
                range);
    const long calls = ((long)n_agents * B + 3) / 4;
    hipLaunchKernelGGL(replay_indices_kernel, dim3((unsigned)((calls + 255) / 256)), dim3(256), 0,
                       (hipStream_t)stream, n_agents, B, (uint32_t)range, seed, counter, idx);
    return check_launch("avd_replay_indices");
}

extern "C" int avd_replay_gather_f32(int n_agents, int cap, int S, int A, int B, const float* ring,
                                     const int32_t* idx, float* s, float* a, float* r, float* s2, void* stream) {
    AVD_REQUIRE(n_agents > 0 && cap > 0 && S > 0 && A > 0 && B > 0, "avd_replay_gather_f32: bad sizes");
    AVD_REQUIRE(ring && idx && s && a && r && s2, "avd_replay_gather_f32: null pointer");
    const long total = (long)n_agents * B * (2 * S + A + 1);
    hipLaunchKernelGGL(replay_gather_kernel, dim3((unsigned)((total + 255) / 256)), dim3(256), 0,
                       (hipStream_t)stream, n_agents, cap, S, A, B, ring, idx, s, a, r, s2);
    return check_launch("avd_replay_gather_f32");
}
```

avddpg_amd/trainer.py:

```python
import logging

import numpy as np
import torch

from . import vec
from ._hip import call, ptr, stream_handle

log = logging.getLogger(__name__)


def is_fed_enabled(conf):
    return (conf.fed_method == conf.interfrl or conf.fed_method == conf.intrafrl) and (conf.framework == conf.dcntrl)


def is_gradient_updates_enabled(conf):
    return conf.aggregation_method == conf.gradients


def is_model_weight_updates_enabled(conf):
    return conf.aggregation_method == conf.weights


def is_weighted_fed_enabled(conf, training_episode):
    return conf.weighted_average_enabled and training_episode >= conf.weighted_window


def is_valid_update_episode(conf, training_episode):
    return conf.fed_enabled and (training_episode % conf.fed_update_count) == 0 and \
        training_episode <= conf.fed_cutoff_episode


def is_valid_update_step(conf, training_step):
    return (training_step % conf.fed_update_delay_steps) == 0


def is_valid_step_for_federated_training_with_gradients(conf, training_episode, training_step):
    return is_fed_enabled(conf) and is_valid_update_episode(conf, training_episode) and \
        is_valid_update_step(conf, training_step) and is_gradient_updates_enabled(conf)


def is_valid_step_for_federated_training_with_weights(conf, training_episode, training_step):
    return is_fed_enabled(conf) and is_valid_update_episode(conf, training_episode) and \
        is_valid_update_step(conf, training_step) and is_model_weight_updates_enabled(conf)


def check_seed_batch(conf, rng, auto_reset, group, fused_step=None):
    if rng != "device":
        raise ValueError("a seed batch needs rng='device': the host-RNG parity mode consumes one global np.random stream")
    if auto_reset != "platoon":
        raise ValueError("a seed batch needs per-platoon episodes (auto_reset='platoon', --episodes platoon): the reference rule "
                         "(any terminal platoon ends the episode of all) would couple the experiments")
    if conf.framework == conf.cntrl:
        raise ValueError("a seed batch needs the decentralized framework: the centralized one has no fused step and its draw "
                         "kernels have no seed table")
    if conf.fed_method == conf.intrafrl:
        raise ValueError("a seed batch covers nofrl and interfrl; intrafrl is not supported")
    if is_fed_enabled(conf) and is_model_weight_updates_enabled(conf):
        raise ValueError("a seed batch covers gradient aggregation only: weights aggregation writes one group's average into every "
                         "agent (workers/trainer.py:442-446)")
    if group is not None:
        raise ValueError("a seed batch runs on one GPU: no process group")
    if fused_step is not None and not fused_step:
        raise ValueError("a seed batch needs the fused step (its draws are keyed per experiment; the separate draw kernels are not)")


def check_sweep(conf, seeds, hparams, shared_engine=None, pipeline_chunks=1):
    from .vec import hparams_rows

    hparams = list(hparams)
    if len(hparams) != len(seeds):
        raise ValueError(f"hparams has {len(hparams)} rows for {len(seeds)} seeds: one dict per experiment")
    rows = hparams_rows(conf, hparams)
    pairs = [(int(k), tuple(r[n] for n in sorted(r))) for k, r in zip(seeds, rows)]
    if len(set(pairs)) != len(pairs):
        raise ValueError("a hyperparameter sweep lists the same (seed, hparams) experiment twice: the experiments would be identical")
    if shared_engine not in (None, "per_agent", "fused3"):
        raise ValueError(f"a hyperparameter sweep runs the per_agent and fused3 engines only; shared_engine={shared_engine!r} has no "
                         "per-experiment table")
    widths = (conf.actor_layer1_size, conf.actor_layer2_size, conf.critic_layer1_size, conf.critic_layer2_size,
              conf.critic_act_layer_size, conf.batch_size)
    if widths != (256, 128, 256, 128, 48, 64):
        raise ValueError(f"a hyperparameter sweep runs the reference widths 256/128/48 with batch 64 only, got layers {widths[:5]} and "
                         f"batch {widths[5]}")
    if int(pipeline_chunks) > 1:
        raise ValueError("a hyperparameter sweep does not run the chunked learn || update pipeline (pipeline_chunks > 1)")
    return rows


SET_ENGINE_MAX_SETS = {"fused": 64, "fused3": 64}


class VecTrainer:
    def __init__(self, conf, device=None, rng="device", group=None, shared_sets=None, seed=None, auto_reset=False,
                 pipeline_chunks=1, fused_update=False, shared_engine=None, init_seed=None, fused_step=None,
                 replay_ring=None, overlap_allreduce=None, seeds=None, hparams=None):
        conf.refresh()
        self.conf, self.rng, self.group = conf, rng, group
        self.device = torch.device(device if device is not None else "cuda")
        self.seeds = self.hp_rows = None
        if hparams is not None and seeds is None:
            raise ValueError("hparams= needs seeds= (one seed per experiment of the sweep)")
        if seeds is not None:
            if seed is not None or init_seed is not None:
                raise ValueError("seeds= is mutually exclusive with seed= / init_seed=")
            self.seeds = vec.seed_table(seeds, "cpu", distinct=hparams is None)[0]
            check_seed_batch(conf, rng, auto_reset, group, fused_step)
            if hparams is not None:
                self.hp_rows = check_sweep(conf, self.seeds, hparams, shared_engine, pipeline_chunks)
        distinct = self.hp_rows is None
        self.E = 1 if self.seeds is None else len(self.seeds)
        self.P, self.L = conf.num_platoons * self.E, conf.pl_size
        self.P_exp = conf.num_platoons
        seed = (conf.random_seed if seed is None else seed) if self.seeds is None else None
        self.env = vec.VecPlatoon(self.P, self.L, conf, self.device, rand_states=conf.rand_states, rng=rng, seed=seed or 0,
                                  seeds=self.seeds, distinct_seeds=distinct)
        self.centralized = conf.framework == conf.cntrl
        self.M = self.env.num_models
        self.S, self.A = self.env.num_states, self.env.num_actions
        if self.centralized and conf.model == conf.modelA and self.L > 1:
            raise ValueError("centralized + Model A with pl_size > 1: the reference's observation is 4L wide but its "
                             "network input 3L (src/environment.py:45-63, 518); not a runnable configuration")
        self.x_stride = 4 * self.L // self.M
        n_agents = self.P * self.M
        self.n_agents = n_agents
        self.ou = vec.VecOUNoise(n_agents, conf, self.device, rng=rng, seed=seed or 0, seeds=self.seeds, distinct_seeds=distinct)
        fed = is_fed_enabled(conf)
        can_share = (fed and conf.fed_method == conf.interfrl and is_gradient_updates_enabled(conf)
                     and conf.fed_update_delay_steps == 1 and conf.fed_update_count == 1
                     and conf.fed_cutoff_ratio >= 1.0)
        self.shared = can_share if shared_sets is None else bool(shared_sets)
        if self.shared and not can_share:
            raise ValueError("shared weight sets are only exact for interfrl+gradients with every step federated")
        self.Pf, self.Mf = self.P_exp, self.E * self.M
        self.set_mod = self.Mf if self.shared else 0
        self.agents = vec.AgentGroup(self.Mf if self.shared else n_agents, self.S, self.A, conf, self.device,
                                     seed=None if self.seeds else (conf.random_seed if init_seed is None else init_seed),
                                     hidd_mult=self.env.hidden_multiplier, seeds=self.seeds, seed_block=self.M)
        self.d_hp = None
        if self.hp_rows is not None:
            self.d_hp = vec.hparams_table(self.hp_rows, conf.ou_dt, self.device)
            self.agents.set_hparams(self.d_hp, self.E, self.M)
        from . import dist as _dist
        _dist.broadcast_agents(self.agents, group)
        self.total_platoons = _dist.total_platoons(self.P, group, self.device)
        self.replay = vec.VecReplay(n_agents, conf.buffer_size, conf.batch_size, self.S, self.A, self.device, rng=rng,
                                    seed=seed or 0, ring=replay_ring, seeds=self.seeds, agents_per_platoon=self.M,
                                    distinct_seeds=distinct)
        f32 = dict(dtype=torch.float32, device=self.device)
        lay = self.agents.lay
        fits = lay.H2 <= 256
        self.shared_engine = shared_engine or ("batched" if (self.shared and not fits) else "per_agent")
        if self.shared_engine not in ("per_agent", "batched", "fused", "fused3"):
            raise ValueError(f"shared_engine={shared_engine!r}")
        if self.shared_engine in ("batched", "fused", "fused3") and not self.shared:
            raise ValueError("the batched learners need shared weight sets (interfrl + gradients, every step federated)")
        if self.shared_engine in ("fused", "fused3") and (lay.H1, lay.H2, lay.Ha, lay.A, lay.B) != (256, 128, 48, 1, 64):
            raise ValueError("shared_engine='fused' / 'fused3' (csrc/fset.hip, fsplit.hip) serve the reference widths 256/128/48, A = 1, batch 64 only; "
                             f"got {lay.H1}/{lay.H2}/{lay.Ha}, A = {lay.A}, batch {lay.B}: use shared_engine='batched'")
        if self.seeds is not None and self.shared and self.Mf > SET_ENGINE_MAX_SETS.get(self.shared_engine, self.Mf):
            raise ValueError(f"a seed batch of {self.E} experiments x {self.M} weight sets needs {self.Mf} sets; shared_engine="
                             f"{self.shared_engine!r} takes at most {SET_ENGINE_MAX_SETS[self.shared_engine]}")
        if self.shared_engine == "per_agent":
            call("avd_learn_check_shape", self.agents._layp)
        self.actor_out = torch.zeros(n_agents, self.A, **f32)
        self.actions = torch.zeros(self.P, self.M, self.A, **f32)
        self.leader_exog = torch.zeros(self.P, **f32)
        batched = self.shared and self.shared_engine in ("batched", "fused", "fused3")
        self.grads = None if batched else torch.zeros(n_agents, self.agents.lay.theta_size, **f32)
        self.losses = torch.zeros(n_agents, 2, **f32)
        self.ep_reward = torch.zeros(self.P, self.M, **f32)
        self.all_ep_reward_lists = [[[] for _ in range(self.M)] for _ in range(self.P)]
        self.all_avg_reward_lists = [[[] for _ in range(self.M)] for _ in range(self.P)]
        self.fed_weights = None
        self.exog_calls = 0
        self.seed = seed
        if auto_reset not in (False, True, "platoon"):
            raise ValueError(f"auto_reset={auto_reset!r}: False, True (any-terminal, all platoons) or 'platoon'")
        self.auto_reset = auto_reset
        if auto_reset and rng != "device":
            raise ValueError("auto_reset needs rng='device'")
        self._dev_weighted = bool(auto_reset and fed and conf.weighted_average_enabled)
        if self._dev_weighted:
            W = int(conf.weighted_window)
            self._hist_ring = torch.zeros(n_agents, W, **f32)
            self._hist_cnt = torch.zeros(self.P, dtype=torch.int32, device=self.device)
            self._w_raw, self._aw = torch.ones(n_agents, **f32), torch.ones(n_agents, **f32)
            self._wsum = torch.full((self.Mf,), float(self.Pf), **f32)
        self.steps_total = 0
        can_fuse_step = rng == "device" and not self.centralized and self.A == 1 and self.S in (3, 4)
        self.fused_step = can_fuse_step if fused_step is None else bool(fused_step)
        if self.fused_step and not can_fuse_step:
            raise ValueError("fused_step needs rng='device' and the decentralized framework")
        self.act_mfma = (self.shared and self.shared_engine in ("fused", "fused3")
                         and (lay.H1, lay.H2, lay.A) == (256, 128, 1) and lay.S in (3, 4))
        can_overlap = group is not None and self.shared and self.shared_engine == "fused3"
        self.overlap_allreduce = False if overlap_allreduce is None else bool(overlap_allreduce)
        if self.overlap_allreduce and not can_overlap:
            raise ValueError("overlap_allreduce needs a process group and shared_engine='fused3' (the two-phase learn call)")
        self._side = None
        self._xbuf = None
        self._flag_exchanged = False
        ws = 1
        if group is not None:
            import torch.distributed as _td
            ws = _td.get_world_size(group)
        self._equal_shards = abs(self.total_platoons - self.P * ws) < 0.5
        self._step_parity = 0
        self._added = False
        self.fused_update = bool(fused_update)
        self._act_ready = False
        self.pipeline_chunks = int(pipeline_chunks)
        self.intra_fused = True
        self.timers = None
        self.episode, self.ep_step = 0, 0
        self.updates = 0
        self.env_steps = 0

    def _timed(self, name, fn, *args, **kw):
        if self.timers is None:
            return fn(*args, **kw)
        e0, e1 = torch.cuda.Event(enable_timing=True), torch.cuda.Event(enable_timing=True)
        e0.record()
        out = fn(*args, **kw)
        e1.record()
        self.timers.setdefault(name, []).append((e0, e1))
        return out

    def reset_episode(self):
        self._act_ready = False
        self.env.reset()
        self.ep_reward.zero_()
        self.ep_step = 0

    def _act(self):
        conf, P, M = self.conf, self.P, self.M
        states = self.env.x.view(P * M, self.x_stride)
        if self.shared and self.shared_engine == "batched" and self.agents.lay.H2 > 256:
            sm = self.env.x.view(self.Pf, self.Mf, 4)[..., :self.S].transpose(0, 1).contiguous()
            o = self.agents.actor_shared(sm, P * M)
            self.actor_out.copy_(o.transpose(0, 1).reshape(P * M, 1))
        elif self._act_ready:
            self.agents.actor(states, self.set_mod, x_stride=self.x_stride, out=self.actor_out,
                              run_if_nonzero=self.env.any_done)
        elif self.act_mfma:
            self.agents.actor_set(states, P * M, x_stride=self.x_stride, out=self.actor_out.view(-1))
        else:
            self.agents.actor(states, self.set_mod, x_stride=self.x_stride, out=self.actor_out)
        if self.fused_step:
            self._step_fused()
            return
        if self.seeds is not None:
            vec._no_scalar_draw("VecTrainer._act (separate draw kernels)")
        if self.rng == "host":
            normals = np.empty((P, M))
            exog = np.empty(P)
            for p in range(P):
                for m in range(M):
                    normals[p, m] = np.random.normal(0, 1.0)
                exog[p] = (np.random.uniform(-conf.reset_max_u, conf.reset_max_u) if conf.rand_gen == conf.uniform
                           else np.random.normal(0, conf.reset_max_u))
            noise = self.ou(normals.reshape(-1))
            self.leader_exog.copy_(torch.from_numpy(exog.astype(np.float32)))
        else:
            noise = self.ou()
            call("avd_uniform_f32" if conf.rand_gen == conf.uniform else "avd_normal_f32", P, ptr(self.leader_exog),
                 conf.reset_max_u, self.seed, self.exog_calls, stream_handle())
            self.exog_calls += 1
        if self.A > 1:
            noise = noise.view(-1, 1).expand(-1, self.A).contiguous()
        call("avd_policy_f32", self.n_agents * self.A, ptr(self.actor_out), ptr(noise), conf.action_low,
             conf.action_high, ptr(self.actions), stream_handle())
        self.env.any_done.zero_()
        self.env.step(self.actions.view(P, self.L), self.leader_exog)

    def _step_fused(self):
        conf, env, ou, rp = self.conf, self.env, self.ou, self.replay
        k = self._step_parity
        self._step_parity ^= 1
        env.any_done = env._any_flags[k:k + 1]
        other = env._any_flags[1 - k:2 - k]
        env.x, env.x_prev = env.x_prev, env.x
        if self.d_hp is not None:
            call("avd_step_fused_hp_f32", ptr(env.d_consts), self.P, self.L, self.S, ptr(env.x_prev), ptr(env.x), ptr(env.prev_a),
                 ptr(env.cum_accel), ptr(env.reward), ptr(env.term), ptr(env.done), ptr(env.any_done), ptr(other), ptr(self.actor_out),
                 ptr(ou.state), ptr(self.actions), ptr(self.leader_exog), ou.mean, conf.ou_dt, conf.action_low, conf.action_high,
                 conf.reset_max_u, 1 if conf.rand_gen == conf.uniform else 0, ptr(env.d_seeds), ptr(self.d_hp), self.E, ou.calls,
                 self.exog_calls, ptr(rp.ring), rp.cap, rp.buffer_counter, ptr(self.ep_reward), stream_handle())
            ou.calls += 1
            self.exog_calls += 1
            env.step_count += 1
            rp.buffer_counter += 1
            self._added = True
            return
        fn, key = ("avd_step_fused_f32", (self.seed,)) if self.seeds is None else ("avd_step_fused_seeds_f32", (ptr(env.d_seeds), self.E))
        call(fn, ptr(env.d_consts), self.P, self.L, self.S, ptr(env.x_prev), ptr(env.x), ptr(env.prev_a),
             ptr(env.cum_accel), ptr(env.reward), ptr(env.term), ptr(env.done), ptr(env.any_done), ptr(other),
             ptr(self.actor_out), ptr(ou.state), ptr(self.actions), ptr(self.leader_exog), conf.theta, ou.mean, conf.ou_dt,
             conf.std_dev, conf.action_low, conf.action_high, conf.reset_max_u, 1 if conf.rand_gen == conf.uniform else 0,
             *key, ou.calls, self.exog_calls, ptr(rp.ring), rp.cap, rp.buffer_counter, ptr(self.ep_reward), stream_handle())
        ou.calls += 1
        self.exog_calls += 1
        env.step_count += 1
        rp.buffer_counter += 1
        self._added = True

    def _weights_for_fed(self, ep):
        w = np.empty((self.P, self.M), dtype=np.float32)
        for p in range(self.P):
            for m in range(self.M):
                hist = self.all_ep_reward_lists[p][m][-self.conf.weighted_window:]
                if not hist:
                    raise RuntimeError(f"weighted federated averaging at episode {ep} needs the episodic rewards of agent "
                                       f"({p}, {m}), but none were recorded (update_reward_list is called by run())")
                w[p, m] = abs(1 / np.mean(hist))
        if not np.all(np.isfinite(w)):
            raise FloatingPointError(f"non-finite federated weights at episode {ep} (an episodic-reward mean of 0?)")
        return torch.from_numpy(w).to(self.device)

    def _train(self, ep, i):
        conf, P, M = self.conf, self.P, self.M
        env = self.env

        def replay_part():
            reward = env.reward_mean.view(P, 1) if self.centralized else env.reward
            xs = self.x_stride
            if self._added:
                self._added = False
            else:
                self.replay.add(env.x_prev.view(P * M, xs), self.actions.view(P * M, self.A), reward.view(-1),
                                env.x.view(P * M, xs), xs)
                self.ep_reward += reward
            if not self.replay.buffer_counter > conf.batch_size:
                return None
            return self.replay.sample()

        batch = self._timed("replay", replay_part)
        if batch is None:
            return
        s, a, r, s2 = batch
        fed = is_fed_enabled(conf)
        self.updates += self.n_agents
        if not fed and self.fused_update:
            nxt = self.A == 1 and self.auto_reset
            self._timed("learn+update", self.agents.learn_update, s, a, r, s2, self.grads, self.losses,
                        next_states=env.x.view(P * M, self.x_stride) if nxt else None, x_stride=self.x_stride,
                        next_actions=self.actor_out.view(-1) if nxt else None)
            self._act_ready = nxt
            return
        if not fed and self.pipeline_chunks > 1:
            self.agents.learn_apply(s, a, r, s2, self.grads, self.losses, chunks=self.pipeline_chunks,
                                    timers=self.timers)
            return
        if (fed and conf.fed_method == conf.intrafrl and not self.shared and self.pipeline_chunks > 1
                and is_valid_update_step(conf, i) and is_valid_step_for_federated_training_with_gradients(conf, ep, i)):
            w = self._intra_weights(ep)
            e0, e1 = torch.cuda.Event(enable_timing=True), torch.cuda.Event(enable_timing=True)
            if self.timers is not None:
                e0.record()
            self.agents.learn_apply_intra(s, a, r, s2, self.grads, P, M, losses=self.losses, chunks=self.pipeline_chunks, weights=w,
                                          lead_skip=bool(conf.intra_directional_averaging), timers=self.timers)
            if self.timers is not None:
                e1.record()
                self.timers.setdefault("learn+update", []).append((e0, e1))
            return
        if self.shared and self.shared_engine in ("batched", "fused", "fused3"):
            weights = None
            if self._dev_weighted:
                weights = "device"
            elif is_weighted_fed_enabled(conf, ep):
                if self.fed_weights is None or self.fed_weights[0] != ep:
                    self.fed_weights = (ep, self._weights_for_fed(ep))
                weights = self.fed_weights[1]
            self._timed("learn", self._learn_batched, s, a, r, s2, weights)
            self._timed("update", self.agents.apply, self.set_grads, guarded=self.shared_engine in ("fused", "fused3"))
            return
        self._timed("learn", self.agents.learn, s, a, r, s2, self.set_mod, grads=self.grads, losses=self.losses)
        self._timed("update", self._update, ep, i, fed)

    def _learn_batched(self, s, a, r, s2, weights=None):
        P, M, B = self.Pf, self.Mf, self.conf.batch_size
        sm = lambda x: x.view(P, M, *x.shape[1:]).transpose(0, 1).reshape(M, P * B, *x.shape[2:]).contiguous()
        if getattr(self, "set_grads", None) is None:
            from .dist import set_exchange_buffer
            self._xbuf, self.set_grads = set_exchange_buffer(M, self.agents.lay.theta_size, self.device)
            self.set_losses = torch.zeros(M, 2, dtype=torch.float32, device=self.device)
        carry = self.env.any_done if (self.group is not None and self.auto_reset is True) else None
        rw = wsum = aw_dev = None
        if isinstance(weights, str):
            aw_dev, wsum, weights = self._aw, self._wsum, None
        elif weights is not None:
            wsum = weights.sum(dim=0)
        if self.shared_engine in ("fused", "fused3"):
            aw = aw_dev if aw_dev is not None else (None if weights is None else (weights * (float(P) / wsum)).reshape(P * M).contiguous())
            if self.overlap_allreduce:
                self._learn_split_overlapped(s, a, r, s2, aw, wsum, carry)
                self._flag_exchanged = carry is not None
                return
            self.agents.learn_set_fused(s, a, r, s2, P * M, grads=self.set_grads, losses=self.set_losses, agent_weight=aw,
                                        split=self.shared_engine == "fused3")
        else:
            if aw_dev is not None:
                rw = aw_dev.view(P, M).transpose(0, 1).reshape(M, P, 1).expand(M, P, B).reshape(M, P * B).contiguous()
            elif weights is not None:
                rw = (weights * (float(P) / wsum)).transpose(0, 1).reshape(M, P, 1).expand(M, P, B).reshape(M, P * B).contiguous()
            self.agents.learn_shared(sm(s), sm(a), sm(r), sm(s2), P * M, grads=self.set_grads, losses=self.set_losses,
                                     row_weight=rw)
        if self.group is not None:
            from .dist import exchange_set_slab
            self._timed("allreduce", exchange_set_slab, self._xbuf, M, self.agents.lay.theta_size, wsum, P, self.total_platoons,
                        self.group, flag=carry, equal_shards=self._equal_shards)
            self._flag_exchanged = carry is not None

    def _learn_split_overlapped(self, s, a, r, s2, aw, wsum, flag=None):
        from .dist import exchange_two_phase

        P, M = self.P, self.M
        lay = self.agents.lay
        A, T = lay.actor_size, lay.theta_size
        if self._side is None:
            f32 = dict(dtype=torch.float32, device=self.device)
            self._side = dict(stream=torch.cuda.Stream(device=self.device), ready=torch.cuda.Event(),
                              crit=torch.empty(M, T - A, **f32), act=torch.empty(M * A + M + 1, **f32))
        scale = float(P) if wsum is None else wsum.view(M, 1)
        learn = lambda phase: self.agents.learn_set_fused(s, a, r, s2, P * M, grads=self.set_grads, losses=self.set_losses,
                                                          agent_weight=aw, split=True, phase=phase)
        learn("critic")
        exchange_two_phase(self.set_grads, A, scale, wsum, self.total_platoons, self.group, self._side,
                           lambda: learn("actor"), timers=self.timers, flag=flag)

    def _update(self, ep, i, fed):
        conf, P, M = self.conf, self.Pf, self.Mf
        if not fed or not is_valid_update_step(conf, i):
            if self.shared:
                raise RuntimeError("local update requested in shared-set mode")
            self.agents.apply(self.grads)
            return
        weights = None
        if self._dev_weighted:
            weights = self._w_raw.view(P, M)
        elif is_weighted_fed_enabled(conf, ep):
            if self.fed_weights is None or self.fed_weights[0] != ep:
                self.fed_weights = (ep, self._weights_for_fed(ep))
            weights = self.fed_weights[1]
        method = conf.fed_method
        if is_valid_step_for_federated_training_with_gradients(conf, ep, i):
            if method == conf.intrafrl and self.intra_fused and not self.shared:
                self.agents.apply_intra(self.grads, P, M, weights=weights, lead_skip=bool(conf.intra_directional_averaging))
                return
            avg = vec.fed_mean(self.grads, P, M, weights=weights, group=self.group, method=method,
                               total=self.total_platoons)
            if self.shared:
                self.agents.apply(avg)
            elif method == conf.intrafrl and self.intra_fused:
                pass
            else:
                directional = method == conf.intrafrl and conf.intra_directional_averaging
                vec.fed_scatter(avg, self.grads, P, M, method)
                if directional:
                    ag = self.agents
                    lead = lambda x: x.view(P, M, -1)[:, 0]
                    keep = [lead(x).clone() for x in (ag.theta, ag.theta_t, ag.stats_t, ag.m, ag.v)]
                    keep_step = ag.step.view(P, M)[:, 0].clone()
                    ag.apply(self.grads)
                    for x, k in zip((ag.theta, ag.theta_t, ag.stats_t, ag.m, ag.v), keep):
                        lead(x).copy_(k)
                    ag.step.view(P, M)[:, 0].copy_(keep_step)
                else:
                    self.agents.apply(self.grads)
        elif is_valid_step_for_federated_training_with_weights(conf, ep, i):
            if self.shared:
                raise RuntimeError("weights aggregation needs per-agent weight sets")
            ag = self.agents
            tp = self.total_platoons
            avg_th = vec.fed_mean(ag.theta, P, M, weights=weights, group=self.group, method=method, total=tp)[0]
            avg_st = vec.fed_mean(ag.stats, P, M, weights=weights, group=self.group, method=method, total=tp)[0]
            directional = method == conf.intrafrl and conf.intra_directional_averaging
            for dst, src in ((ag.theta, avg_th), (ag.theta_t, avg_th), (ag.stats, avg_st), (ag.stats_t, avg_st)):
                view = dst.view(P, M, -1)
                (view[:, 1:] if directional else view).copy_(src.expand_as(view[:, 1:] if directional else view))

    def step(self, ep=None, i=None, sync=True):
        ep = self.episode if ep is None else ep
        i = self.ep_step if i is None else i
        self._flag_exchanged = False
        self._timed("act+env", self._act)
        self._train(ep, i)
        self.env_steps += self.P
        self.ep_step += 1
        if self.group is not None and self.auto_reset is True and not self._flag_exchanged:
            import torch.distributed as _td
            _td.all_reduce(self.env.any_done, op=_td.ReduceOp.MAX, group=self.group)
        self.steps_total += 1
        limit = self.conf.steps_per_episode
        if self.auto_reset == "platoon":
            if self._dev_weighted:
                self.env.ensure_episode_state()
                self._push_history(done=self.env.done, ep_len=self.env.ep_len, limit=limit, zero_after=0)
            self.env.episode_end(self.ep_reward, self.M, limit, any_reset=self.env.any_done)
            self.episode = self.steps_total // limit
            if self._dev_weighted:
                self._refresh_weights(1 if self.steps_total >= int(self.conf.weighted_window) * limit else 0)
            return None
        if self.auto_reset:
            if self.ep_step >= limit:
                if self._dev_weighted:
                    self._push_history(force=1, zero_after=1)
                self.env.reset()
                self._act_ready = False
                self.ep_step = 0
                self.episode += 1
            else:
                if self._dev_weighted:
                    self._push_history(cond=self.env.any_done, zero_after=1)
                self.env.reset(cond=self.env.any_done)
            if self._dev_weighted:
                self._refresh_weights(-1)
            return None
        if not sync:
            return None
        from .dist import any_terminal
        return any_terminal(self.env.any_done, self.group)

    def _intra_weights(self, ep):
        if self._dev_weighted:
            return self._w_raw.view(self.P, self.M)
        if is_weighted_fed_enabled(self.conf, ep):
            if self.fed_weights is None or self.fed_weights[0] != ep:
                self.fed_weights = (ep, self._weights_for_fed(ep))
            return self.fed_weights[1]
        return None

    def _push_history(self, done=None, ep_len=None, limit=0, cond=None, force=0, zero_after=0):
        call("avd_fed_history_push_f32", self.P, self.M, int(self.conf.weighted_window), ptr(self.ep_reward), ptr(done), ptr(ep_len),
             int(limit), ptr(cond), int(force), int(zero_after), ptr(self._hist_ring), ptr(self._hist_cnt), stream_handle())

    def _refresh_weights(self, host_enabled):
        call("avd_fed_weights_f32", self.Pf, self.Mf, int(self.conf.weighted_window), ptr(self._hist_ring), ptr(self._hist_cnt),
             int(host_enabled), ptr(self._w_raw), ptr(self._aw), ptr(self._wsum), stream_handle())

    def nonfinite_updates(self):
        n = getattr(self.agents, "nonfinite_skipped", None)
        return 0 if n is None else int(n.item())

    def update_reward_list(self, ep):
        rew = self.ep_reward.cpu().numpy()
        for p in range(self.P):
            for m in range(self.M):
                self.all_ep_reward_lists[p][m].append(rew[p, m])
                self.all_avg_reward_lists[p][m].append(
                    np.mean(self.all_ep_reward_lists[p][m][-self.conf.reward_averaging_window:]))

    def run(self, number_of_episodes=None):
        conf = self.conf
        n = conf.number_of_episodes if number_of_episodes is None else number_of_episodes
        for ep in range(n):
            self.episode = ep
            self.reset_episode()
            for i in range(conf.steps_per_episode):
                if self.step(ep, i):
                    break
            self.update_reward_list(ep)
        return self.all_ep_reward_lists, self.all_avg_reward_lists

    def evaluator_scores(self, platoons=None):
        from . import evaluator

        if self.seeds is not None:
            E, M = self.E, self.M
            platoons = list(range(self.P_exp)) if platoons is None else list(platoons)
            if self.shared:
                sc = evaluator.run_many(self.conf, self.agents, list(range(E)), set_mod=M, set_bases=[e * M for e in range(E)])[0]
                return np.repeat(sc[:, :1], len(platoons), axis=1)
            glob = [vec.batch_platoon(e, p, E) for e in range(E) for p in platoons]
            return evaluator.run_many(self.conf, self.agents, glob)[0][:, 0].reshape(E, len(platoons))
        platoons = list(range(self.P)) if platoons is None else list(platoons)
        if self.shared:
            sc = evaluator.run_many(self.conf, self.agents, [0], set_mod=self.M)[0]
            return np.repeat(sc[:, 0], len(platoons))
        return evaluator.run_many(self.conf, self.agents, platoons)[0][:, 0]

    def evaluate_scenarios(self, scenarios, seeds=None, platoons=None, amp=None, period_s=10.0):
        from . import evaluator

        kw = dict(scenarios=scenarios, seeds=seeds, amp=amp, period_s=period_s)
        if self.seeds is not None:
            E, M = self.E, self.M
            platoons = list(range(self.P_exp)) if platoons is None else list(platoons)
            n = len(platoons)
            if self.shared:
                r = evaluator.run_cases(self.conf, self.agents, list(range(E)), set_mod=M, set_bases=[e * M for e in range(E)], **kw)
                lift = lambda x: np.repeat(x[:, None], n, axis=1)
            else:
                r = evaluator.run_cases(self.conf, self.agents, [vec.batch_platoon(e, p, E) for e in range(E) for p in platoons], **kw)
                lift = lambda x: x.reshape(E, n, *x.shape[1:])
            return evaluator.CaseResults(r.scenarios, r.seeds, r.T, lift(r.scores), lift(r.counters), {k: lift(v) for k, v in r.metrics.items()})
        platoons = list(range(self.P)) if platoons is None else list(platoons)
        if self.shared:
            r = evaluator.run_cases(self.conf, self.agents, [0], set_mod=self.M, **kw)
            rep = lambda x: np.repeat(x, len(platoons), axis=0)
            return evaluator.CaseResults(r.scenarios, r.seeds, r.T, rep(r.scores), rep(r.counters), {k: rep(v) for k, v in r.metrics.items()})
        return evaluator.run_cases(self.conf, self.agents, platoons, **kw)

    def run_simulations(self):
        if self.seeds is not None:
            return [[float(r / self.conf.re_scalar) for r in row] for row in self.evaluator_scores()]
        return [float(r / self.conf.re_scalar) for r in self.evaluator_scores()]

    def experiment_agents(self, e):
        if self.seeds is None:
            raise ValueError("experiment_agents needs a seed batch (VecTrainer(seeds=...))")
        return self.agents.experiment_view(e, self.E, self.M, self.shared)

    def exploit(self, pairs):
        if self.seeds is None:
            raise ValueError("exploit needs a seed batch (VecTrainer(seeds=...))")
        self.agents.copy_experiments(pairs, self.E, self.M)
        self._act_ready = False

    def set_hparams(self, hparams):
        if self.hp_rows is None:
            raise ValueError("set_hparams needs a hyperparameter sweep (VecTrainer(seeds=..., hparams=...))")
        hparams = list(hparams)
        if len(hparams) != self.E:
            raise ValueError(f"hparams has {len(hparams)} rows for {self.E} experiments: one dict per experiment")
        rows = vec.hparams_rows(self.conf, hparams)
        self.d_hp.copy_(vec.hparams_table(rows, self.conf.ou_dt, self.device))
        self.hp_rows = rows

    def experiment_conf(self, e):
        import copy

        if self.seeds is None:
            raise ValueError("experiment_conf needs a seed batch (VecTrainer(seeds=...))")
        c = copy.copy(self.conf)
        c.random_seed = self.seeds[e]
        if self.hp_rows is not None:
            for k, v in self.hp_rows[e].items():
                setattr(c, k, v)
        return c


class Trainer:

    def __init__(self, base_dir, timestamp, debug_enabled, conf, rng="host", device=None):
        self.base_dir, self.timestamp, self.debug_enabled, self.conf = base_dir, timestamp, debug_enabled, conf
        self.rng, self.device = rng, device
        self.engine = None

    def initialize(self):
        self.conf.timestamp = str(self.timestamp)
        self.conf.fed_enabled = is_fed_enabled(self.conf)
        self.engine = VecTrainer(self.conf, device=self.device, rng=self.rng)
        self.num_models, self.num_platoons = self.engine.M, self.engine.P
        self.num_states, self.num_actions = self.engine.S, self.engine.A
        self.all_ep_reward_lists = self.engine.all_ep_reward_lists
        self.all_avg_reward_lists = self.engine.all_avg_reward_lists

    def run(self, number_of_episodes=None):
        return self.engine.run(number_of_episodes)


def learn(rbuffer, actor_model, critic_model, target_actor, target_critic, gamma=0.99):
    from . import _hip, params

    lay = actor_model.lay
    s, a, r, s2 = rbuffer.sample()
    A = lay.actor_size
    theta = torch.cat([actor_model.theta[:, :A], critic_model.theta[:, A:]], dim=1).contiguous()
    theta_t = torch.cat([target_actor.theta[:, :A], target_critic.theta[:, A:]], dim=1).contiguous()

    def stats_of(act, cri):
        st = act.stats.clone()
        st[:, lay.cmms:] = cri.stats[:, lay.cmms:]
        return st

    stats, stats_t = stats_of(actor_model, critic_model), stats_of(target_actor, target_critic)
    grads = torch.empty(1, lay.theta_size, dtype=torch.float32, device=theta.device)
    call("avd_learn_f32", _hip.C.byref(lay), 1, 1, ptr(theta), ptr(stats), ptr(theta_t), ptr(stats_t),
         ptr(s.reshape(1, lay.B, lay.S).contiguous()), ptr(a.reshape(1, lay.B, lay.A).contiguous()),
         ptr(r.reshape(1, lay.B).contiguous()), ptr(s2.reshape(1, lay.B, lay.S).contiguous()), gamma,
         actor_model.high, ptr(grads), None, stream_handle())
    g = grads[0].cpu().numpy()
    dummy = np.zeros(lay.stats_size, dtype=np.float32)
    dims = getattr(actor_model, "dims", None)
    return (params.unpack(lay, g, dummy, "critic", trainable_only=True, dims=dims),
            params.unpack(lay, g, dummy, "actor", trainable_only=True, dims=dims))


Trainer.learn = staticmethod(learn)
```

avddpg_amd/vec.py:

```python
import ctypes as C

import numpy as np
import torch

from . import _hip, dynamics, params
from ._hip import call, ptr, stream_handle


def _dev(device):
    return torch.device(device if device is not None else "cuda")


def seed_table(seeds, device, distinct=True):
    seeds = tuple(int(k) for k in seeds)
    if not seeds:
        raise ValueError("an experiment batch needs at least one seed")
    if distinct and len(set(seeds)) != len(seeds):
        raise ValueError(f"duplicate seeds in {list(seeds)}: the experiments would be identical")
    if any(k < 0 or k >= 2 ** 64 for k in seeds):
        raise ValueError(f"seeds must lie in [0, 2**64): {list(seeds)}")
    bits = np.array(seeds, dtype=np.uint64).view(np.int64)
    return seeds, torch.from_numpy(bits.copy()).to(device)


# ... 155 lines not shown
        fa = np.zeros(P, dtype=np.float64)
        train = self._mode() == 0
        for p in range(P):
            fa[p] = self._rand(c.pl_leader_reset_a)
            for i in range(L):
                self.front_u[p] = self._rand(c.reset_max_u)
                if train:
                    draws[p, i, 0] = self._rand(c.reset_ep_max)
                    draws[p, i, 1] = self._rand(c.reset_max_ev)
                    draws[p, i, 2] = self._rand(c.reset_max_a)
        self.front_accel = fa.copy()
        return draws, fa

    def observations(self, x=None):
        x = self.x if x is None else x
        return x[..., : self.obs_width]

    def reset(self, cond=None):
        draws = fa = None
        if self.rng == "host":
            if cond is not None:
                raise ValueError("conditional reset needs rng='device'")
            draws, fa = self._host_reset_draws()
        self._upload_reset(draws, fa, cond)
        self.reset_count += 1
        return self.observations()

    def episode_end(self, ep_reward, M, limit, any_reset=None):
        if self.rng != "device":
            raise ValueError("per-platoon episode ends need rng='device'")
        self.ensure_episode_state()
        st = self.ep_stats
        if self.seeds is not None:
            call("avd_episode_end_seeds_f32", ptr(self.d_consts), self.P, self.L, M, ptr(self.x), ptr(self.prev_a), ptr(self.cum_accel),
                 ptr(self.done), ptr(self.ep_len), ptr(ep_reward), int(limit), ptr(st["ret_sum"]), ptr(st["len_sum"]),
                 ptr(st["count"]), ptr(any_reset), self._mode(), ptr(self.d_seeds), self.n_groups, self.reset_count, stream_handle())
        else:
            call("avd_episode_end_f32", ptr(self.d_consts), self.P, self.L, M, ptr(self.x), ptr(self.prev_a), ptr(self.cum_accel),
                 ptr(self.done), ptr(self.ep_len), ptr(ep_reward), int(limit), ptr(st["ret_sum"]), ptr(st["len_sum"]),
                 ptr(st["count"]), ptr(any_reset), self._mode(), self.seed, self.reset_count, stream_handle())
        self.reset_count += 1

    def ensure_episode_state(self):
        if self.ep_len is None:
            z = lambda dt: torch.zeros(self.P, dtype=dt, device=self.device)
            self.ep_len = z(torch.int32)
            self.ep_stats = dict(ret_sum=z(torch.float32), len_sum=z(torch.float32), count=z(torch.int32))

    def pop_episode_stats(self, per_experiment=False):
        st = self.ep_stats
        if per_experiment:
            E = self.n_groups
            parts = [{k: t.view(-1, E)[:, e].contiguous() for k, t in st.items()} for e in range(E)]
            n = np.array([int(q["count"].sum()) for q in parts], dtype=np.int64)
            ret = np.array([float(q["ret_sum"].double().sum()) for q in parts])
            ln = np.array([float(q["len_sum"].double().sum()) for q in parts])
            for t in st.values():
                t.zero_()
            with np.errstate(invalid="ignore", divide="ignore"):
                return np.where(n > 0, ret / np.maximum(n, 1), np.nan), np.where(n > 0, ln / np.maximum(n, 1), np.nan), n
        n = int(st["count"].sum())
        ret, ln = float(st["ret_sum"].double().sum()), float(st["len_sum"].double().sum())
        for t in st.values():
            t.zero_()
        return (ret / n if n else float("nan")), (ln / n if n else float("nan")), n

    def step(self, actions, leader_exog):
        self.x, self.x_prev = self.x_prev, self.x
        call("avd_env_step_f32", ptr(self.d_consts), self.P, self.L, ptr(self.x_prev), ptr(self.x), ptr(self.prev_a),
             ptr(self.cum_accel), ptr(actions), ptr(leader_exog), ptr(self.reward), ptr(self.term), ptr(self.done),
             ptr(self.reward_mean), ptr(self.any_done), stream_handle())
        self.step_count += 1
        return self.observations(), self.reward, self.done

    def get_jerk_from(self, x_before, prev_a_before):
        return (x_before[..., 2] - prev_a_before) / self.config.sample_rate


class VecOUNoise:

    def __init__(self, n, config, device=None, rng="host", seed=1, mean=0.0, seeds=None, distinct_seeds=True):
        self.n, self.config, self.device = int(n), config, _dev(device)
        self.rng, self.seed, self.calls = rng, int(seed), 0
        self.seeds = None if seeds is None else seed_table(seeds, "cpu", distinct_seeds)[0]
        if self.seeds is not None and rng != "device":
            raise ValueError("an experiment batch (seeds=...) needs rng='device'")
        self.mean = float(mean)
        self.state = torch.zeros(self.n, dtype=torch.float32, device=self.device)

    def reset(self):
        self.state.zero_()

    def __call__(self, normals=None):
        if self.seeds is not None:
            _no_scalar_draw("VecOUNoise()")
        c = self.config
        d_n = None
        if self.rng == "host":
            if normals is None:
                normals = np.random.normal(0, 1.0, size=self.n)
            d_n = torch.from_numpy(np.asarray(normals, dtype=np.float32).reshape(self.n)).to(self.device)
        call("avd_ou_step_f32", self.n, ptr(self.state), ptr(d_n), c.theta, self.mean, c.ou_dt, c.std_dev, self.seed,
             self.calls, stream_handle())
        self.calls += 1
        return self.state


class VecReplay:

    def __init__(self, n_agents, buffer_capacity, batch_size, num_states, num_actions, device=None, rng="host",
                 seed=1, ring=None, seeds=None, agents_per_platoon=1, distinct_seeds=True):
        self.n, self.cap, self.B = int(n_agents), int(buffer_capacity), int(batch_size)
        self.S, self.A = int(num_states), int(num_actions)
        self.row = 2 * self.S + self.A + 1
        self.device, self.rng, self.seed = _dev(device), rng, int(seed)
        self.seeds = self.d_seeds = None
        self.agents_per_platoon = int(agents_per_platoon)
        if seeds is not None:
            if rng != "device":
                raise ValueError("an experiment batch (seeds=...) needs rng='device'")
            self.seeds, self.d_seeds = seed_table(seeds, self.device, distinct_seeds)
            if self.n % (len(self.seeds) * self.agents_per_platoon):
                raise ValueError(f"n_agents={self.n} is not a multiple of {len(self.seeds)} experiments x {self.agents_per_platoon} agents")
        if ring is not None:
            if tuple(ring.shape) != (self.n, self.cap, self.row) or ring.dtype != torch.float32 or not ring.is_contiguous():
                raise _hip.AvdError(f"replay ring must be contiguous float32 {(self.n, self.cap, self.row)}, got {tuple(ring.shape)}")
            self.ring = ring
        else:
            self.ring = torch.zeros(self.n, self.cap, self.row, dtype=torch.float32, device=self.device)
        self.buffer_counter = 0
        self.samples = 0
        f32 = dict(dtype=torch.float32, device=self.device)
        self.idx = torch.zeros(self.n, self.B, dtype=torch.int32, device=self.device)
        self.s = torch.zeros(self.n, self.B, self.S, **f32)
        self.a = torch.zeros(self.n, self.B, self.A, **f32)
        self.r = torch.zeros(self.n, self.B, **f32)
        self.s2 = torch.zeros(self.n, self.B, self.S, **f32)

    def add(self, s_prev, action, reward, s_next, x_stride):
        call("avd_replay_add_f32", self.n, self.cap, self.S, self.A, ptr(self.ring), self.buffer_counter, ptr(s_prev),
             ptr(s_next), x_stride, ptr(action), ptr(reward), stream_handle())
        self.buffer_counter += 1

    def sample_range(self):
        return min(self.buffer_counter, self.cap)

    def draw_indices(self, host_idx=None):
        if self.seeds is not None:
            _no_scalar_draw("VecReplay.draw_indices")
        if self.rng == "host":
            if host_idx is None:
                rr = self.sample_range()
                host_idx = np.stack([np.random.choice(rr, self.B) for _ in range(self.n)])
            self.idx.copy_(torch.from_numpy(np.asarray(host_idx).astype(np.int32)))
        else:
            call("avd_replay_indices", self.n, self.B, self.sample_range(), self.seed, self.samples, ptr(self.idx),
                 stream_handle())
        self.samples += 1
        return self.idx

    def gather(self):
        call("avd_replay_gather_f32", self.n, self.cap, self.S, self.A, self.B, ptr(self.ring), ptr(self.idx),
             ptr(self.s), ptr(self.a), ptr(self.r), ptr(self.s2), stream_handle())
        return self.s, self.a, self.r, self.s2

    def sample(self, host_idx=None):
        if self.seeds is not None:
            if host_idx is not None or not (self.A == 1 and self.S in (3, 4) and self.B % 4 == 0):
                _no_scalar_draw("VecReplay.sample (host indices, or a shape avd_replay_sample_seeds_f32 does not serve)")
            call("avd_replay_sample_seeds_f32", self.n, self.cap, self.S, self.A, self.B, ptr(self.ring), self.sample_range(),
                 ptr(self.d_seeds), len(self.seeds), self.agents_per_platoon, self.samples, ptr(self.idx), ptr(self.s), ptr(self.a),
                 ptr(self.r), ptr(self.s2), stream_handle())
            self.samples += 1
            return self.s, self.a, self.r, self.s2
        if self.rng != "host" and host_idx is None and self.A == 1 and self.S in (3, 4) and self.B % 4 == 0:
            call("avd_replay_sample_f32", self.n, self.cap, self.S, self.A, self.B, ptr(self.ring), self.sample_range(), self.seed,
                 self.samples, ptr(self.idx), ptr(self.s), ptr(self.a), ptr(self.r), ptr(self.s2), stream_handle())
            self.samples += 1
            return self.s, self.a, self.r, self.s2
        self.draw_indices(host_idx)
        return self.gather()


class AgentGroup:

    def __init__(self, n_sets, num_states, num_actions, config, device=None, hidd_mult=1, seed=None, high_bound=None, seeds=None,
                 seed_block=1):
        c = config
        self.config, self.device, self.n_sets = c, _dev(device), int(n_sets)
        if (c.critic_layer1_size, c.critic_layer2_size) != (c.actor_layer1_size, c.actor_layer2_size):
            raise _hip.AvdError("actor and critic layer1/layer2 sizes must match (reference defaults do)")
        self.dims = params.Dims(num_states, num_actions, int(c.actor_layer1_size * hidd_mult),
                                int(c.actor_layer2_size * hidd_mult), int(c.critic_act_layer_size * hidd_mult))
        H1p, H2p, Hap = params.padded_widths(self.dims.H1, self.dims.H2, self.dims.Ha)
        self.lay = _hip.make_layout(num_states, num_actions, H1p, H2p, Hap, c.batch_size)
        self.high = float(c.action_high if high_bound is None else high_bound)
        f32 = dict(dtype=torch.float32, device=self.device)
        n, T, S = self.n_sets, self.lay.theta_size, self.lay.stats_size
        self.theta = torch.zeros(n, T, **f32)
        self.stats = torch.zeros(n, S, **f32)
        self.theta_t = torch.zeros(n, T, **f32)
        self.stats_t = torch.zeros(n, S, **f32)
        self.m = torch.zeros(n, T, **f32)
        self.v = torch.zeros(n, T, **f32)
        self.step = torch.zeros(n, dtype=torch.int32, device=self.device)
        self._layp = C.byref(self.lay)
        if seeds is not None and seed is not None:
            raise ValueError("AgentGroup: seed and seeds are mutually exclusive")
        init = lambda k: params.init_weights(self.lay, np.random.RandomState(k), nominal=(c.actor_layer1_size, c.actor_layer2_size),
                                             dims=self.dims)
        if seeds is None:
            th, st = init(c.random_seed if seed is None else seed)
            self.theta.copy_(torch.from_numpy(th).to(self.device).expand(n, T))
            self.stats.copy_(torch.from_numpy(st).to(self.device).expand(n, S))
        else:
            E, blk = len(seeds), int(seed_block)
            if n % (E * blk):
                raise ValueError(f"AgentGroup: {n} sets are not a multiple of {E} experiments x {blk}")
            for e, k in enumerate(seeds):
                th, st = init(int(k))
                self.theta.view(-1, E, blk, T)[:, e].copy_(torch.from_numpy(th).to(self.device).expand(n // (E * blk), blk, T))
                self.stats.view(-1, E, blk, S)[:, e].copy_(torch.from_numpy(st).to(self.device).expand(n // (E * blk), blk, S))
        self.theta_t.copy_(self.theta)
        self.stats_t.copy_(self.stats)
        self.hp = None

    def set_hparams(self, table, n_groups, set_block):
        if self.n_sets % (int(n_groups) * int(set_block)):
            raise ValueError(f"AgentGroup: {self.n_sets} sets are not a multiple of {n_groups} experiments x {set_block}")
        self.hp = (table, int(n_groups), int(set_block))

    def copy_experiments(self, pairs, n_groups, set_block):
        flat = [int(x) for pr in pairs for x in pr]
        if len(flat) != 2 * len(pairs):
            raise ValueError(f"pairs must be (src, dst) experiment pairs, got {pairs!r}")
        arr = (C.c_int32 * max(1, len(flat)))(*flat)
        call("avd_copy_experiment_sets_f32", self._layp, self.n_sets, int(n_groups), int(set_block), arr, len(pairs), ptr(self.theta),
             ptr(self.stats), ptr(self.theta_t), ptr(self.stats_t), ptr(self.m), ptr(self.v), ptr(self.step), stream_handle())

    def _no_hp(self, what):
        if self.hp is not None:
            raise _hip.AvdError(f"{what}: a hyperparameter sweep (set_hparams) has no per-experiment form of this path")

    def actor(self, states, set_mod, x_stride=None, out=None, target=False, run_if_nonzero=None):
        n_agents = states.shape[0]
        x_stride = states.shape[-1] if x_stride is None else x_stride
        shape = (n_agents,) if self.lay.A == 1 else (n_agents, self.lay.A)
        out = torch.empty(*shape, dtype=torch.float32, device=self.device) if out is None else out
        th, st = (self.theta_t, self.stats_t) if target else (self.theta, self.stats)
        if run_if_nonzero is not None:
            call("avd_actor_forward_cond_f32", self._layp, n_agents, set_mod, ptr(th), ptr(st), ptr(states), x_stride,
                 self.high, ptr(out), ptr(run_if_nonzero), stream_handle())
        else:
            call("avd_actor_forward_f32", self._layp, n_agents, set_mod, ptr(th), ptr(st), ptr(states), x_stride,
                 self.high, ptr(out), stream_handle())
        return out

    def actor_set(self, states, n_agents, x_stride=None, out=None, run_if_nonzero=None):
        x_stride = states.shape[-1] if x_stride is None else x_stride
        out = torch.empty(n_agents, dtype=torch.float32, device=self.device) if out is None else out
        call("avd_actor_forward_set_f32", self._layp, n_agents, self.n_sets, ptr(self.theta), ptr(self.stats), ptr(states), x_stride,
             self.high, ptr(out), ptr(run_if_nonzero), stream_handle())
        return out

    def critic(self, states, actions, set_mod, x_stride=None, out=None, target=False):
        n_agents = states.shape[0]
        x_stride = states.shape[-1] if x_stride is None else x_stride
        shape = (n_agents,) if self.lay.A == 1 else (n_agents, self.lay.A)
        out = torch.empty(*shape, dtype=torch.float32, device=self.device) if out is None else out
        th, st = (self.theta_t, self.stats_t) if target else (self.theta, self.stats)
        call("avd_critic_forward_f32", self._layp, n_agents, set_mod, ptr(th), ptr(st), ptr(states), x_stride,
             ptr(actions), ptr(out), stream_handle())
        return out

    def learn(self, s, a, r, s2, set_mod, grads=None, losses=None):
        n_agents = s.shape[0]
        if grads is None:
            grads = torch.empty(n_agents, self.lay.theta_size, dtype=torch.float32, device=self.device)
        if self.hp is not None:
            tbl, E, blk = self.hp
            call("avd_learn_hp_f32", self._layp, n_agents, set_mod, ptr(self.theta), ptr(self.stats), ptr(self.theta_t),
                 ptr(self.stats_t), ptr(s), ptr(a), ptr(r), ptr(s2), self.high, ptr(grads), ptr(losses), ptr(tbl), E, blk,
                 stream_handle())
            return grads
        call("avd_learn_f32", self._layp, n_agents, set_mod, ptr(self.theta), ptr(self.stats), ptr(self.theta_t),
             ptr(self.stats_t), ptr(s), ptr(a), ptr(r), ptr(s2), self.config.gamma, self.high, ptr(grads),
             ptr(losses), stream_handle())
        return grads

    def learn_shared(self, s, a, r, s2, n_agents, grads=None, losses=None, row_weight=None):
        import ctypes
        if grads is None:
            grads = torch.empty(self.n_sets, self.lay.theta_size, dtype=torch.float32, device=self.device)
        need = ctypes.c_size_t(0)
        call("avd_learn_shared_workspace", self._layp, n_agents, self.n_sets, ctypes.byref(need))
        ws = getattr(self, "_wide_ws", None)
        if ws is None or ws.numel() < need.value:
            ws = self._wide_ws = torch.empty(need.value, dtype=torch.uint8, device=self.device)
        call("avd_learn_shared_bf16", self._layp, n_agents, self.n_sets, ptr(self.theta), ptr(self.stats),
             ptr(self.theta_t), ptr(self.stats_t), ptr(s), ptr(a), ptr(r), ptr(s2), ptr(row_weight), self.config.gamma,
             self.high, ptr(grads), ptr(losses), ptr(ws), ws.numel(), stream_handle())
        return grads

    def learn_set_fused(self, s, a, r, s2, n_agents, grads=None, losses=None, agent_weight=None, split=False, phase=None):
        import ctypes
        if self.hp is not None and not (split and phase is None):
            self._no_hp("learn_set_fused (bf16 operands, or a phase of the split call)")
        self._check_agent_major(s, a, r, s2, n_agents, agent_weight)
        if grads is None:
            grads = torch.empty(self.n_sets, self.lay.theta_size, dtype=torch.float32, device=self.device)
        wsf, fn, attr = (("avd_learn_set_split_workspace", "avd_learn_set_split_f16x3", "_fsplit_ws") if split else
                         ("avd_learn_set_fused_workspace", "avd_learn_set_fused_bf16", "_fset_ws"))
        need = ctypes.c_size_t(0)
        call(wsf, self._layp, n_agents, self.n_sets, ctypes.byref(need))
        ws = getattr(self, attr, None)
        if ws is None or ws.numel() < need.value:
            ws = torch.empty(need.value, dtype=torch.uint8, device=self.device)
            setattr(self, attr, ws)
        if phase is not None and not split:
            raise _hip.AvdError("phase= needs split=True (csrc/fsplit.hip)")
        if phase == "actor":
            call("avd_learn_set_split_actor", self._layp, n_agents, self.n_sets, ptr(self.theta), ptr(self.stats), ptr(s), self.high,
                 ptr(grads), ptr(ws), ws.numel(), stream_handle())
            return grads
        if phase not in (None, "critic"):
            raise _hip.AvdError(f"phase={phase!r}")
        if self.hp is not None:
            tbl, E, blk = self.hp
            call("avd_learn_set_split_hp_f16x3", self._layp, n_agents, self.n_sets, ptr(self.theta), ptr(self.stats), ptr(self.theta_t),
                 ptr(self.stats_t), ptr(s), ptr(a), ptr(r), ptr(s2), ptr(agent_weight), self.high, ptr(grads), ptr(losses), ptr(ws),
                 ws.numel(), ptr(tbl), E, blk, stream_handle())
            return grads
        call("avd_learn_set_split_critic" if phase == "critic" else fn, self._layp, n_agents, self.n_sets, ptr(self.theta), ptr(self.stats),
             ptr(self.theta_t), ptr(self.stats_t), ptr(s), ptr(a), ptr(r), ptr(s2), ptr(agent_weight), self.config.gamma, self.high,
             ptr(grads), ptr(losses), ptr(ws), ws.numel(), stream_handle())
        return grads

    def learn_set_split(self, s, a, r, s2, n_agents, grads=None, losses=None, agent_weight=None):
        return self.learn_set_fused(s, a, r, s2, n_agents, grads=grads, losses=losses, agent_weight=agent_weight, split=True)

    def _check_agent_major(self, s, a, r, s2, n_agents, agent_weight):
        lay = self.lay
        want = {"s": (n_agents, lay.B, lay.S), "s2": (n_agents, lay.B, lay.S), "r": (n_agents, lay.B)}
        for name, x in (("s", s), ("s2", s2), ("r", r)):
            if tuple(x.shape) != want[name] or x.dtype != torch.float32 or not x.is_contiguous():
                raise _hip.AvdError(f"set learner: {name} must be contiguous float32 {want[name]} (agent-major), got "
                                    f"{tuple(x.shape)} {x.dtype} contiguous={x.is_contiguous()}")
        if a.numel() != n_agents * lay.B * lay.A or a.dtype != torch.float32 or not a.is_contiguous() or a.shape[0] != n_agents:
            raise _hip.AvdError(f"set learner: a must be contiguous float32 [{n_agents}, {lay.B}(, {lay.A})], got {tuple(a.shape)} {a.dtype}")
        if n_agents <= 0 or n_agents % self.n_sets:
            raise _hip.AvdError(f"set learner: n_agents={n_agents} is not a multiple of n_sets={self.n_sets}")
        if agent_weight is not None and (agent_weight.numel() != n_agents or agent_weight.dtype != torch.float32
                                         or not agent_weight.is_contiguous()):
            raise _hip.AvdError(f"set learner: agent_weight must be contiguous float32 [{n_agents}]")

    def actor_shared(self, states_set_major, n_agents, out=None):
        import ctypes
        rows = n_agents // self.n_sets
        if out is None:
            out = torch.empty(self.n_sets, rows, dtype=torch.float32, device=self.device)
        need = ctypes.c_size_t(0)
        call("avd_actor_forward_shared_workspace", self._layp, n_agents, self.n_sets, ctypes.byref(need))
        ws = getattr(self, "_wide_act_ws", None)
        if ws is None or ws.numel() < need.value:
            ws = self._wide_act_ws = torch.empty(need.value, dtype=torch.uint8, device=self.device)
        call("avd_actor_forward_shared_bf16", self._layp, n_agents, self.n_sets, ptr(self.theta), ptr(self.stats),
             ptr(states_set_major), self.high, ptr(out), ptr(ws), ws.numel(), stream_handle())
        return out

    def apply(self, grads, guarded=False):
        c = self.config
        self.step += 1
        if self.hp is not None:
            tbl, E, blk = self.hp
            if guarded:
                if getattr(self, "nonfinite_skipped", None) is None:
                    self.nonfinite_skipped = torch.zeros(1, dtype=torch.int32, device=self.device)
                call("avd_adam_polyak_guarded_hp_f32", self._layp, self.n_sets, ptr(self.theta), ptr(self.stats), ptr(self.theta_t),
                     ptr(self.stats_t), ptr(self.m), ptr(self.v), ptr(grads), ptr(self.step), ptr(self.nonfinite_skipped), ptr(tbl), E,
                     blk, stream_handle())
            else:
                call("avd_adam_polyak_hp_f32", self._layp, self.n_sets, ptr(self.theta), ptr(self.stats), ptr(self.theta_t),
                     ptr(self.stats_t), ptr(self.m), ptr(self.v), ptr(grads), ptr(self.step), ptr(tbl), E, blk, stream_handle())
            return
        if guarded:
            if getattr(self, "nonfinite_skipped", None) is None:
                self.nonfinite_skipped = torch.zeros(1, dtype=torch.int32, device=self.device)
            call("avd_adam_polyak_guarded_f32", self._layp, self.n_sets, ptr(self.theta), ptr(self.stats), ptr(self.theta_t),
                 ptr(self.stats_t), ptr(self.m), ptr(self.v), ptr(grads), ptr(self.step), c.actor_lr, c.critic_lr,
                 float(c.tau), ptr(self.nonfinite_skipped), stream_handle())
            return
        call("avd_adam_polyak_f32", self._layp, self.n_sets, ptr(self.theta), ptr(self.stats), ptr(self.theta_t),
             ptr(self.stats_t), ptr(self.m), ptr(self.v), ptr(grads), ptr(self.step), c.actor_lr, c.critic_lr,
             float(c.tau), stream_handle())

    def apply_intra(self, grads, P, M, weights=None, lead_skip=False, lo=0, hi=None, stream=None, advance=True):
        self._no_hp("apply_intra")
        c = self.config
        hi = P if hi is None else hi
        if self.n_sets != P * M:
            raise _hip.AvdError("apply_intra needs one weight set per agent (P * M sets)")
        if advance:
            if stream is None:
                self.step.view(P, M)[lo:hi, (1 if lead_skip else 0):] += 1
            else:
                with torch.cuda.stream(stream):
                    self.step.view(P, M)[lo:hi, (1 if lead_skip else 0):] += 1
        a, b = lo * M, hi * M
        call("avd_adam_polyak_intra_f32", self._layp, hi - lo, M, 1 if lead_skip else 0, ptr(self.theta[a:b]), ptr(self.stats[a:b]),
             ptr(self.theta_t[a:b]), ptr(self.stats_t[a:b]), ptr(self.m[a:b]), ptr(self.v[a:b]), ptr(grads[a:b]), ptr(self.step[a:b]),
             ptr(None if weights is None else weights.reshape(-1)[a:b]), c.actor_lr, c.critic_lr, float(c.tau),
             stream_handle() if stream is None else _hip.C.c_void_p(stream.cuda_stream))

    def learn_apply_intra(self, s, a, r, s2, grads, P, M, losses=None, chunks=8, weights=None, lead_skip=False, timers=None):
        main = torch.cuda.current_stream()
        if getattr(self, "_side", None) is None:
            self._side = torch.cuda.Stream(device=self.device)
        side = self._side
        c = self.config
        chunks = max(1, min(chunks, P))
        bounds = [(P * i) // chunks for i in range(chunks + 1)]
        T = lambda: torch.cuda.Event(enable_timing=timers is not None)
        self.step.view(P, M)[:, (1 if lead_skip else 0):] += 1
        for i in range(chunks):
            lo, hi = bounds[i] * M, bounds[i + 1] * M
            if hi == lo:
                continue
            t0, t1 = T(), T()
            if timers is not None:
                t0.record(main)
            call("avd_learn_f32", self._layp, hi - lo, 0, ptr(self.theta[lo:hi]), ptr(self.stats[lo:hi]), ptr(self.theta_t[lo:hi]),
                 ptr(self.stats_t[lo:hi]), ptr(s[lo:hi]), ptr(a[lo:hi]), ptr(r[lo:hi]), ptr(s2[lo:hi]), c.gamma, self.high,
                 ptr(grads[lo:hi]), ptr(losses[lo:hi]) if losses is not None else None, _hip.C.c_void_p(main.cuda_stream))
            t1.record(main)
            side.wait_event(t1)
            u0, u1 = T(), T()
            if timers is not None:
                u0.record(side)
            self.apply_intra(grads, P, M, weights=weights, lead_skip=lead_skip, lo=bounds[i], hi=bounds[i + 1], stream=side, advance=False)
            if timers is not None:
                u1.record(side)
                timers.setdefault("learn", []).append((t0, t1))
                timers.setdefault("update", []).append((u0, u1))
        done = torch.cuda.Event()
        done.record(side)
        main.wait_event(done)

    def learn_update(self, s, a, r, s2, grads, losses=None, next_states=None, x_stride=None, next_actions=None):
        n = self.n_sets
        if s.shape[0] != n:
            raise _hip.AvdError("learn_update needs one weight set per agent (set_mod == 0)")
        if getattr(self, "theta_alt", None) is None:
            self.theta_alt = self.theta.clone()
        c = self.config
        self.step += 1
        if self.hp is not None:
            tbl, E, blk = self.hp
            args = (self._layp, n, ptr(self.theta), ptr(self.stats), ptr(self.theta_alt), ptr(self.theta_t), ptr(self.stats_t),
                    ptr(self.m), ptr(self.v), ptr(self.step), ptr(s), ptr(a), ptr(r), ptr(s2), self.high, ptr(grads), ptr(losses))
            if next_actions is not None:
                if self.lay.A != 1:
                    raise _hip.AvdError("next-action epilogue: A == 1 only")
                xs = next_states.shape[-1] if x_stride is None else x_stride
                call("avd_learn_update_act_hp_f32", *args, ptr(next_states), xs, ptr(next_actions), ptr(tbl), E, blk, stream_handle())
            else:
                call("avd_learn_update_hp_f32", *args, ptr(tbl), E, blk, stream_handle())
            self.theta, self.theta_alt = self.theta_alt, self.theta
            return
        args = (self._layp, n, ptr(self.theta), ptr(self.stats), ptr(self.theta_alt), ptr(self.theta_t), ptr(self.stats_t),
                ptr(self.m), ptr(self.v), ptr(self.step), ptr(s), ptr(a), ptr(r), ptr(s2), c.gamma, self.high, c.actor_lr,
                c.critic_lr, float(c.tau), ptr(grads), ptr(losses))
        if next_actions is not None:
            if self.lay.A != 1:
                raise _hip.AvdError("next-action epilogue: A == 1 only")
            xs = next_states.shape[-1] if x_stride is None else x_stride
            call("avd_learn_update_act_f32", *args, ptr(next_states), xs, ptr(next_actions), stream_handle())
        else:
            call("avd_learn_update_f32", *args, stream_handle())
        self.theta, self.theta_alt = self.theta_alt, self.theta

    def learn_apply(self, s, a, r, s2, grads, losses=None, chunks=4, timers=None):
        self._no_hp("learn_apply")
        n = self.n_sets
        if s.shape[0] != n:
            raise _hip.AvdError("learn_apply needs one weight set per agent (set_mod == 0)")
        main = torch.cuda.current_stream()
        if getattr(self, "_side", None) is None:
            self._side = torch.cuda.Stream(device=self.device)
        side = self._side
        c = self.config
        self.step += 1
        chunks = max(1, min(chunks, n))
        bounds = [(n * i) // chunks for i in range(chunks + 1)]
        T = lambda: torch.cuda.Event(enable_timing=timers is not None)
        for i in range(chunks):
            lo, hi = bounds[i], bounds[i + 1]
            if hi == lo:
                continue
            t0, t1 = T(), T()
            if timers is not None:
                t0.record(main)
            call("avd_learn_f32", self._layp, hi - lo, 0, ptr(self.theta[lo:hi]), ptr(self.stats[lo:hi]),
                 ptr(self.theta_t[lo:hi]), ptr(self.stats_t[lo:hi]), ptr(s[lo:hi]), ptr(a[lo:hi]), ptr(r[lo:hi]),
                 ptr(s2[lo:hi]), c.gamma, self.high, ptr(grads[lo:hi]), ptr(losses[lo:hi]) if losses is not None else None,
                 _hip.C.c_void_p(main.cuda_stream))
            t1.record(main)
            side.wait_event(t1)
            u0, u1 = T(), T()
            if timers is not None:
                u0.record(side)
            call("avd_adam_polyak_f32", self._layp, hi - lo, ptr(self.theta[lo:hi]), ptr(self.stats[lo:hi]),
                 ptr(self.theta_t[lo:hi]), ptr(self.stats_t[lo:hi]), ptr(self.m[lo:hi]), ptr(self.v[lo:hi]),
                 ptr(grads[lo:hi]), ptr(self.step[lo:hi]), c.actor_lr, c.critic_lr, float(c.tau),
                 _hip.C.c_void_p(side.cuda_stream))
            if timers is not None:
                u1.record(side)
                timers.setdefault("learn", []).append((t0, t1))
                timers.setdefault("update", []).append((u0, u1))
        done = torch.cuda.Event()
        done.record(side)
        main.wait_event(done)

    def experiment_view(self, e, E, M, shared):
        import copy
        g = copy.copy(self)
        T, S = self.lay.theta_size, self.lay.stats_size
        pick = (lambda x, w: x.view(E, M, w)[e]) if shared else (lambda x, w: x.view(-1, E, M, w)[:, e].reshape(-1, w).contiguous())
        for name, w in (("theta", T), ("stats", S), ("theta_t", T), ("stats_t", S)):
            setattr(g, name, pick(getattr(self, name), w))
        g.n_sets = g.theta.shape[0]
        for name in ("m", "v", "step", "theta_alt", "hp"):
            setattr(g, name, None)
        return g

    def get_weights(self, set_idx, which, target=False, trainable_only=False):
        th, st = (self.theta_t, self.stats_t) if target else (self.theta, self.stats)
        return params.unpack(self.lay, th[set_idx].cpu().numpy(), st[set_idx].cpu().numpy(), which, trainable_only,
                             dims=self.dims)

    def set_weights(self, set_idx, which, weights, target=False):
        th, st = (self.theta_t, self.stats_t) if target else (self.theta, self.stats)
        h_th, h_st = th[set_idx].cpu().numpy(), st[set_idx].cpu().numpy()
        params.pack(self.lay, weights, h_th, h_st, which, dims=self.dims)
        th[set_idx].copy_(torch.from_numpy(h_th))
        st[set_idx].copy_(torch.from_numpy(h_st))

    def grads_as_lists(self, grads_row):
        g = grads_row.cpu().numpy()
        dummy = np.zeros(self.lay.stats_size, dtype=np.float32)
        return (params.unpack(self.lay, g, dummy, "critic", trainable_only=True, dims=self.dims),
                params.unpack(self.lay, g, dummy, "actor", trainable_only=True, dims=self.dims))


def fed_mean(grads, P, M, weights=None, group=None, method="interfrl", total=None):
    n = grads.shape[-1]
    if method == "interfrl":
        n_out, n_in, so, si = M, P, 1, M
    elif method == "intrafrl":
        n_out, n_in, so, si = P, M, M, 1
    else:
        raise ValueError(method)
    out = torch.empty(n_out, n, dtype=torch.float32, device=grads.device)
    wsum = torch.empty(n_out, dtype=torch.float32, device=grads.device) if weights is not None else None
    call("avd_fed_sum_f32", n_out, n_in, so, si, n, ptr(grads), ptr(weights), ptr(out), ptr(wsum), stream_handle())
    count = float(n_in)
    if group is not None and method == "interfrl":
        from .dist import exchange_fed_sums
        count = exchange_fed_sums(out, wsum, n_in, group, total=total)
    call("avd_fed_finalize_f32", n_out, n, ptr(out), count, ptr(wsum), stream_handle())
    return out


def fed_scatter(avg, dst, P, M, method="interfrl", i_begin=0):
    n = avg.shape[-1]
    n_out, n_in, so, si = (M, P, 1, M) if method == "interfrl" else (P, M, M, 1)
    call("avd_fed_scatter_f32", n_out, n_in, so, si, i_begin, n, ptr(avg), ptr(dst), stream_handle())
    return dst
```

include/avddpg_hip.h:

```cpp
#ifndef AVDDPG_HIP_H
#define AVDDPG_HIP_H

#include <stddef.h>
#include <stdint.h>

#ifdef __cplusplus
extern "C" {
#pragma GCC visibility push(default)
#endif

#define AVD_MAX_L 16

#define AVD_OK 0
#define AVD_E_INVALID (-1)
#define AVD_E_LAUNCH (-2)
#define AVD_E_UNSUPPORTED (-3)

typedef struct avd_env_consts {
    int32_t L;
    int32_t model_a;
    int32_t can_terminate;
    int32_t uniform_reset;
    float max_ep, max_ev;
    float abs_action_high;
    float two_max_a;
    float T;
    float ca, cb, cc, cd;
    float re_scalar, terminal_reward;
    float stand_still, timegap;
    float reset_ep_max, reset_max_ev, reset_max_a;
    float reset_ep_eval, reset_ev_eval, reset_a_eval;
    float leader_reset_a;
    float A[AVD_MAX_L][16];
    float B[AVD_MAX_L][4];
    float C[AVD_MAX_L][4];
} avd_env_consts;

typedef struct avd_mlp_layout {
    int32_t S, A, H1, H2, Ha, B;
    int32_t aW1, ab1, ag1, abe1, aW2, ab2, ag2, abe2, aW3, ab3;
    int32_t actor_size;
    int32_t cWs, cbs, cgs, cbes, cWa, cba, cga, cbea, cW2, cb2, cg3, cbe3, cW3, cb3;
    int32_t theta_size;
    int32_t amm1, amv1, amm2, amv2, cmms, cmvs, cmma, cmva, cmm3, cmv3;
    int32_t stats_size;
} avd_mlp_layout;

const char* avd_last_error(void);
int avd_version(void);
int avd_diagnostics_enabled(void);

int avd_mlp_layout_init(avd_mlp_layout* out, int S, int A, int H1, int H2, int Ha, int B);

int avd_env_step_f32(const avd_env_consts* d_consts, int P, int L, const float* x_in, float* x_out, float* prev_a,
                     float* cum_accel, const float* u, const float* leader_exog, float* reward, uint8_t* term,
                     uint8_t* done, float* reward_mean, int32_t* any_done, void* stream);

int avd_env_reset_f32(const avd_env_consts* d_consts, int P, int L, float* x, float* prev_a, float* cum_accel,
                      const float* draws, const float* front_accel, int mode, uint64_t seed, uint64_t counter,
                      const int32_t* cond, void* stream);

int avd_episode_end_f32(const avd_env_consts* d_consts, int P, int L, int M, float* x, float* prev_a, float* cum_accel,
                        const uint8_t* done, int32_t* ep_len, float* ep_reward, int limit, float* ret_sum, float* len_sum,
                        int32_t* ep_cnt, int32_t* any_reset, int mode, uint64_t seed, uint64_t counter, void* stream);


int avd_ou_step_f32(int n, float* ou_state, const float* normals, float theta, float mean, float dt, float std_dev,
                    uint64_t seed, uint64_t counter, void* stream);

int avd_policy_f32(int n, const float* actor_out, const float* noise, float lo, float hi, float* action,
                   void* stream);

int avd_normal_f32(int n, float* out, float std_dev, uint64_t seed, uint64_t counter, void* stream);

int avd_uniform_f32(int n, float* out, float half_width, uint64_t seed, uint64_t counter, void* stream);

int avd_replay_add_f32(int n_agents, int cap, int S, int A, float* ring, int64_t counter, const float* s_prev,
                       const float* s_next, int x_stride, const float* action, const float* reward, void* stream);

int avd_replay_indices(int n_agents, int B, int range, uint64_t seed, uint64_t counter, int32_t* idx, void* stream);

int avd_replay_gather_f32(int n_agents, int cap, int S, int A, int B, const float* ring, const int32_t* idx, float* s,
                          float* a, float* r, float* s2, void* stream);


int avd_actor_forward_f32(const avd_mlp_layout* lay, int n_agents, int set_mod, const float* theta, const float* stats,
                          const float* state, int x_stride, float high, float* out, void* stream);

int avd_actor_forward_cond_f32(const avd_mlp_layout* lay, int n_agents, int set_mod, const float* theta,
                               const float* stats, const float* state, int x_stride, float high, float* out,
                               const int32_t* run_if_nonzero, void* stream);

int avd_critic_forward_f32(const avd_mlp_layout* lay, int n_agents, int set_mod, const float* theta,
                           const float* stats, const float* state, int x_stride, const float* action, float* q,
                           void* stream);

int avd_learn_f32(const avd_mlp_layout* lay, int n_agents, int set_mod, const float* theta, const float* stats,
                  const float* theta_t, const float* stats_t, const float* s, const float* a, const float* r,
                  const float* s2, float gamma, float high, float* grads, float* losses, void* stream);

int avd_learn_check_shape(const avd_mlp_layout* lay);

int avd_adam_polyak_f32(const avd_mlp_layout* lay, int n_sets, float* theta, float* stats, float* theta_t,
                        float* stats_t, float* m, float* v, const float* grads, const int32_t* step, float actor_lr,
                        float critic_lr, double tau, void* stream);

int avd_adam_polyak_guarded_f32(const avd_mlp_layout* lay, int n_sets, float* theta, float* stats, float* theta_t, float* stats_t,
                                float* m, float* v, const float* grads, int32_t* step, float actor_lr, float critic_lr, double tau,
                                int32_t* skipped, void* stream);

int avd_learn_update_f32(const avd_mlp_layout* lay, int n_agents, const float* theta, const float* stats,
                         float* theta_out, float* theta_t, float* stats_t, float* m, float* v, const int32_t* step,
                         const float* s, const float* a, const float* r, const float* s2, float gamma, float high,
                         float actor_lr, float critic_lr, double tau, float* grads_scratch, float* losses,
                         void* stream);

int avd_learn_update_plan(const avd_mlp_layout* lay, int n_agents, int* chunk_agents, int* n_chunks, int* update_groups);

int avd_learn_update_act_f32(const avd_mlp_layout* lay, int n_agents, const float* theta, const float* stats,
                             float* theta_out, float* theta_t, float* stats_t, float* m, float* v, const int32_t* step,
                             const float* s, const float* a, const float* r, const float* s2, float gamma, float high,
                             float actor_lr, float critic_lr, double tau, float* grads_scratch, float* losses,
                             const float* next_state, int x_stride, float* next_action, void* stream);

int avd_polyak_f32(int64_t n, const float* w, float* t, double tau, void* stream);

int avd_fed_sum_f32(int n_out, int n_in, int stride_out, int stride_in, int n, const float* g, const float* weights,
                    float* out, float* wsum, void* stream);
int avd_fed_finalize_f32(int n_out, int n, float* out, float count, const float* wsum, void* stream);
int avd_fed_scatter_f32(int n_out, int n_in, int stride_out, int stride_in, int i_begin, int n, const float* src,
                        float* dst, void* stream);

int avd_adam_polyak_intra_f32(const avd_mlp_layout* lay, int P, int M, int lead_skip, float* theta, float* stats, float* theta_t,
                              float* stats_t, float* m, float* v, const float* grads, const int32_t* step, const float* weights,
                              float actor_lr, float critic_lr, double tau, void* stream);

int avd_fed_history_push_f32(int P, int M, int W, float* ep_reward, const uint8_t* done, const int32_t* ep_len, int limit,
                             const int32_t* cond, int force, int zero_after, float* ring, int32_t* hist_cnt, void* stream);
int avd_fed_weights_f32(int P, int M, int W, const float* ring, const int32_t* hist_cnt, int host_enabled, float* w_raw,
                        float* agent_weight, float* wsum, void* stream);

int avd_step_fused_f32(const avd_env_consts* d_consts, int P, int L, int S, const float* x_in, float* x_out, float* prev_a,
                       float* cum_accel, float* reward, uint8_t* term, uint8_t* done, int32_t* any_done, int32_t* any_done_other,
                       const float* actor_out, float* ou_state, float* action, float* leader_exog, float ou_theta, float ou_mean,
                       float ou_dt, float ou_std_dev, float action_low, float action_high, float exog_scale, int exog_uniform,
                       uint64_t seed, uint64_t ou_counter, uint64_t exog_counter, float* ring, int cap, int64_t replay_counter,
                       float* ep_reward, void* stream);

int avd_replay_sample_f32(int n_agents, int cap, int S, int A, int B, const float* ring, int range, uint64_t seed, uint64_t counter,
                          int32_t* idx, float* s, float* a, float* r, float* s2, void* stream);

int avd_step_fused_seeds_f32(const avd_env_consts* d_consts, int P, int L, int S, const float* x_in, float* x_out, float* prev_a,
                             float* cum_accel, float* reward, uint8_t* term, uint8_t* done, int32_t* any_done, int32_t* any_done_other,
                             const float* actor_out, float* ou_state, float* action, float* leader_exog, float ou_theta,
                             float ou_mean, float ou_dt, float ou_std_dev, float action_low, float action_high, float exog_scale,
                             int exog_uniform, const uint64_t* d_seeds, int n_groups, uint64_t ou_counter, uint64_t exog_counter,
                             float* ring, int cap, int64_t replay_counter, float* ep_reward, void* stream);
int avd_env_reset_seeds_f32(const avd_env_consts* d_consts, int P, int L, float* x, float* prev_a, float* cum_accel, int mode,
                            const uint64_t* d_seeds, int n_groups, uint64_t counter, const int32_t* cond, void* stream);
int avd_episode_end_seeds_f32(const avd_env_consts* d_consts, int P, int L, int M, float* x, float* prev_a, float* cum_accel,
                              const uint8_t* done, int32_t* ep_len, float* ep_reward, int limit, float* ret_sum, float* len_sum,
                              int32_t* ep_cnt, int32_t* any_reset, int mode, const uint64_t* d_seeds, int n_groups, uint64_t counter,
                              void* stream);
int avd_replay_sample_seeds_f32(int n_agents, int cap, int S, int A, int B, const float* ring, int range, const uint64_t* d_seeds,
                                int n_groups, int agents_per_platoon, uint64_t counter, int32_t* idx, float* s, float* a, float* r,
                                float* s2, void* stream);

typedef struct avd_hparams {
    float actor_lr, critic_lr;
    float tau, one_minus_tau;
    float gamma;
    float ou_theta, ou_scale;
    float reserved;
} avd_hparams;

int avd_step_fused_hp_f32(const avd_env_consts* d_consts, int P, int L, int S, const float* x_in, float* x_out, float* prev_a,
                          float* cum_accel, float* reward, uint8_t* term, uint8_t* done, int32_t* any_done, int32_t* any_done_other,
                          const float* actor_out, float* ou_state, float* action, float* leader_exog, float ou_mean, float ou_dt,
                          float action_low, float action_high, float exog_scale, int exog_uniform, const uint64_t* d_seeds,
                          const avd_hparams* d_hp, int n_groups, uint64_t ou_counter, uint64_t exog_counter, float* ring, int cap,
                          int64_t replay_counter, float* ep_reward, void* stream);
int avd_learn_hp_f32(const avd_mlp_layout* lay, int n_agents, int set_mod, const float* theta, const float* stats,
                     const float* theta_t, const float* stats_t, const float* s, const float* a, const float* r, const float* s2,
                     float high, float* grads, float* losses, const avd_hparams* d_hp, int n_groups, int set_block, void* stream);
int avd_learn_update_hp_f32(const avd_mlp_layout* lay, int n_agents, const float* theta, const float* stats, float* theta_out,
                            float* theta_t, float* stats_t, float* m, float* v, const int32_t* step, const float* s, const float* a,
                            const float* r, const float* s2, float high, float* grads_scratch, float* losses, const avd_hparams* d_hp,
                            int n_groups, int set_block, void* stream);
int avd_learn_update_act_hp_f32(const avd_mlp_layout* lay, int n_agents, const float* theta, const float* stats, float* theta_out,
                                float* theta_t, float* stats_t, float* m, float* v, const int32_t* step, const float* s,
                                const float* a, const float* r, const float* s2, float high, float* grads_scratch, float* losses,
                                const float* next_state, int x_stride, float* next_action, const avd_hparams* d_hp, int n_groups,
                                int set_block, void* stream);
int avd_adam_polyak_hp_f32(const avd_mlp_layout* lay, int n_sets, float* theta, float* stats, float* theta_t, float* stats_t,
                           float* m, float* v, const float* grads, const int32_t* step, const avd_hparams* d_hp, int n_groups,
                           int set_block, void* stream);
int avd_adam_polyak_guarded_hp_f32(const avd_mlp_layout* lay, int n_sets, float* theta, float* stats, float* theta_t,
                                   float* stats_t, float* m, float* v, const float* grads, int32_t* step, int32_t* skipped,
                                   const avd_hparams* d_hp, int n_groups, int set_block, void* stream);

int avd_learn_set_split_hp_f16x3(const avd_mlp_layout* lay, int n_agents, int n_sets, const float* theta, const float* stats,
                                 const float* theta_t, const float* stats_t, const float* s, const float* a, const float* r, const float* s2,
                                 const float* agent_weight, float high, float* grads, float* losses, void* workspace, size_t workspace_bytes,
                                 const avd_hparams* d_hp, int n_groups, int set_block, void* stream);

int avd_copy_experiment_sets_f32(const avd_mlp_layout* lay, int n_sets, int n_groups, int set_block, const int32_t* pairs, int n_pairs,
                                 float* theta, float* stats, float* theta_t, float* stats_t, float* m, float* v, int32_t* step,
                                 void* stream);

int avd_actor_forward_set_f32(const avd_mlp_layout* lay, int n_agents, int n_sets, const float* theta, const float* stats,
                              const float* states, int x_stride, float high, float* out, const int32_t* run_if_nonzero, void* stream);

int avd_learn_shared_workspace(const avd_mlp_layout* lay, int n_agents, int n_sets, size_t* bytes);
int avd_learn_shared_bf16(const avd_mlp_layout* lay, int n_agents, int n_sets, const float* theta, const float* stats,
                          const float* theta_t, const float* stats_t, const float* s, const float* a, const float* r,
                          const float* s2, const float* row_weight, float gamma, float high, float* grads, float* losses,
                          void* workspace, size_t workspace_bytes, void* stream);

int avd_learn_set_fused_workspace(const avd_mlp_layout* lay, int n_agents, int n_sets, size_t* bytes);
int avd_learn_set_fused_bf16(const avd_mlp_layout* lay, int n_agents, int n_sets, const float* theta, const float* stats,
                             const float* theta_t, const float* stats_t, const float* s, const float* a, const float* r,
                             const float* s2, const float* agent_weight, float gamma, float high, float* grads, float* losses,
                             void* workspace, size_t workspace_bytes, void* stream);

int avd_learn_set_split_mfma_count(const avd_mlp_layout* lay, int n_agents, int n_sets, unsigned long long* mfma_32x32x16);
int avd_learn_set_split_critic(const avd_mlp_layout* lay, int n_agents, int n_sets, const float* theta, const float* stats,
                               const float* theta_t, const float* stats_t, const float* s, const float* a, const float* r,
                               const float* s2, const float* agent_weight, float gamma, float high, float* grads, float* losses,
                               void* workspace, size_t workspace_bytes, void* stream);
int avd_learn_set_split_actor(const avd_mlp_layout* lay, int n_agents, int n_sets, const float* theta, const float* stats,
                              const float* s, float high, float* grads, void* workspace, size_t workspace_bytes, void* stream);
int avd_learn_set_split_workspace(const avd_mlp_layout* lay, int n_agents, int n_sets, size_t* bytes);
int avd_learn_set_split_f16x3(const avd_mlp_layout* lay, int n_agents, int n_sets, const float* theta, const float* stats,
                               const float* theta_t, const float* stats_t, const float* s, const float* a, const float* r,
                               const float* s2, const float* agent_weight, float gamma, float high, float* grads, float* losses,
                               void* workspace, size_t workspace_bytes, void* stream);

int avd_learn_set_split_bf16x3(const avd_mlp_layout* lay, int n_agents, int n_sets, const float* theta, const float* stats,
                               const float* theta_t, const float* stats_t, const float* s, const float* a, const float* r,
                               const float* s2, const float* agent_weight, float gamma, float high, float* grads, float* losses,
                               void* workspace, size_t workspace_bytes, void* stream);

int avd_actor_forward_shared_workspace(const avd_mlp_layout* lay, int n_agents, int n_sets, size_t* bytes);
int avd_actor_forward_shared_bf16(const avd_mlp_layout* lay, int n_agents, int n_sets, const float* theta,
                                  const float* stats, const float* state, float high, float* out, void* workspace,
                                  size_t workspace_bytes, void* stream);

int avd_eval_rollout_f32(const avd_mlp_layout* lay, const avd_env_consts* d_consts, int R, int L, int M, int T, const float* theta,
                         const float* stats, int n_sets, const int32_t* set_base, const float* x0, const float* prev_a0,
                         const float* leader, int n_start, const int32_t* start_idx, float high, float lo, float hi,
                         float sample_rate, float* counters, int n_trace, const int32_t* trace_idx, float* tr_states,
                         float* tr_actions, float* tr_jerks, void* stream);

#define AVD_EVAL_NMETRIC 8
int avd_eval_cases_f32(const avd_mlp_layout* lay, const avd_env_consts* d_consts, int G, int K, int L, int M, int T,
                       const float* theta, const float* stats, int n_sets, const int32_t* set_base, const float* x0,
                       const float* prev_a0, const float* leader, float high, float lo, float hi, float sample_rate,
                       float* counters, float* metrics, void* stream);

int avd_eval_cases_block(int K, int L);

int avd_gemm_bt_bf16(int M, int Nc, int K, const void* A, long lda, const void* B, long ldb, float* D, long ldd,
                     void* stream);

#ifdef __cplusplus
#pragma GCC visibility pop
}
#endif
#endif
```

Before: 2.108 million.

## Fuse replay sampling into the split learner's front kernel

Adds a sample_front kernel that draws the replay batch and, in the same launch, scales and preps the weights, zeroes the gradients and packs the sampled states into f16 hi/lo operands with the finite/overflow flag check. A 'prepared' learn path then skips the separate front kernel. This removes one kernel launch and a global round-trip of the sampled batch between the sampler and the pack stage. In exchange the sampler must run on device with a matching shape, and the Python side has to track that the workspace and grads buffers line up with the prepared batch.

```diff
diff --git a/avddpg_amd/_hip.py b/avddpg_amd/_hip.py
--- a/avddpg_amd/_hip.py
+++ b/avddpg_amd/_hip.py
@@ -105,6 +105,12 @@
     "avd_learn_set_split_actor": [_LP, _i, _i, _P, _P, _P, _f, _P, _P, C.c_size_t, _P],
     "avd_learn_set_split_bf16x3": [_LP, _i, _i, _P, _P, _P, _P, _P, _P, _P, _P, _P, _f, _f, _P, _P, _P, C.c_size_t, _P],
     "avd_learn_set_split_f16x3": [_LP, _i, _i, _P, _P, _P, _P, _P, _P, _P, _P, _P, _f, _f, _P, _P, _P, C.c_size_t, _P],
+    "avd_replay_sample_split_front_f32": [_LP, _i, _i, _i, _P, _i, _u64, _u64, _P, _P, _P, _P, _P, _P, _P, _P, _P, _P, _P, C.c_size_t, _P],
+    "avd_replay_sample_seeds_split_front_f32": [_LP, _i, _i, _i, _P, _i, _P, _i, _i, _u64, _P, _P, _P, _P, _P, _P, _P, _P, _P, _P, _P,
+                                                C.c_size_t, _P],
+    "avd_learn_set_split_prepared_f16x3": [_LP, _i, _i, _P, _P, _P, _P, _P, _P, _P, _P, _P, _f, _f, _P, _P, _P, C.c_size_t, _P],
+    "avd_learn_set_split_hp_prepared_f16x3": [_LP, _i, _i, _P, _P, _P, _P, _P, _P, _P, _P, _P, _f, _P, _P, _P, C.c_size_t, _P, _i, _i, _P],
+    "avd_learn_set_split_critic_prepared": [_LP, _i, _i, _P, _P, _P, _P, _P, _P, _P, _P, _P, _f, _f, _P, _P, _P, C.c_size_t, _P],
     "avd_actor_forward_shared_workspace": [_LP, _i, _i, C.POINTER(C.c_size_t)],
     "avd_actor_forward_shared_bf16": [_LP, _i, _i, _P, _P, _P, _f, _P, _P, C.c_size_t, _P],
     "avd_eval_rollout_f32": [_LP, _P, _i, _i, _i, _i, _P, _P, _i, _P, _P, _P, _P, _i, _P, _f, _f, _f, _f, _P, _i, _P, _P, _P, _P,
diff --git a/avddpg_amd/csrc/fsplit.hip b/avddpg_amd/csrc/fsplit.hip
--- a/avddpg_amd/csrc/fsplit.hip
+++ b/avddpg_amd/csrc/fsplit.hip
@@ -1,6 +1,7 @@
 #include <type_traits>
 
 #include "fset_common.h"
+#include "replay_sample.h"
 
 namespace avd {
 namespace fsplit {
@@ -339,33 +340,85 @@
     int n_sets, n_scale, n_prep1, n_zero, n_pack;
 };
 constexpr int ZERO_PER_BLOCK = 4096;
+__device__ __forceinline__ bool front_small_roles(const PrepArgs& pa, float* grads, long n_grads, int n_sets, int n_scale, int n_prep1,
+                                                  int n_zero, int& b) {
+    if (b < n_scale) {
+        scale_role(pa, b & 3, (b >> 2) % n_sets, (b >> 2) / n_sets, n_sets);
+        return true;
+    }
+    b -= n_scale;
+    if (b < n_prep1) {
+        const int q = 4 * b + (threadIdx.x >> 6);
+        bool hit = false;
+        if (q < NGT_MAX * 4 * n_sets) hit = prep1_role(pa, q % NGT_MAX, (q / NGT_MAX) & 3, q / (NGT_MAX * 4), threadIdx.x & 63);
+        front_flag(pa.fflag + 4 * (long)b, hit);
+        return true;
+    }
+    b -= n_prep1;
+    if (b < n_zero) {
+        if (b == 0 && threadIdx.x == 0) *pa.bad = 0;
+        const long base = (long)b * ZERO_PER_BLOCK + threadIdx.x;
+#pragma unroll
+        for (int k = 0; k < ZERO_PER_BLOCK / 256; ++k)
+            if (base + 256 * k < n_grads) grads[base + 256 * k] = 0.f;
+        return true;
+    }
+    b -= n_zero;
+    return false;
+}
 template <int S>
 __global__ __launch_bounds__(256) void front_kernel(const FrontArgs a) {
     int b = blockIdx.x;
-    if (b < a.n_scale) {
-        scale_role(a.pa, b & 3, (b >> 2) % a.n_sets, (b >> 2) / a.n_sets, a.n_sets);
-        return;
-    }
-    b -= a.n_scale;
-    if (b < a.n_prep1) {
-        const int q = 4 * b + (threadIdx.x >> 6);
-        bool hit = false;
-        if (q < NGT_MAX * 4 * a.n_sets) hit = prep1_role(a.pa, q % NGT_MAX, (q / NGT_MAX) & 3, q / (NGT_MAX * 4), threadIdx.x & 63);
-        front_flag(a.pa.fflag + 4 * (long)b, hit);
-        return;
-    }
-    b -= a.n_prep1;
-    if (b < a.n_zero) {
-        if (b == 0 && threadIdx.x == 0) *a.pa.bad = 0;
-        const long base = (long)b * ZERO_PER_BLOCK + threadIdx.x;
-#pragma unroll
-        for (int k = 0; k < ZERO_PER_BLOCK / 256; ++k)
-            if (base + 256 * k < a.n_grads) a.grads[base + 256 * k] = 0.f;
-        return;
-    }
-    b -= a.n_zero;
+    if (front_small_roles(a.pa, a.grads, a.n_grads, a.n_sets, a.n_scale, a.n_prep1, a.n_zero, b)) return;
     const int which = b >= a.n_pack;
     pack_x_role<S>(a.pk, which, b - which * a.n_pack, a.pa.fflag + 4 * ((long)a.n_prep1 + b));
+}
+
+struct SampleArgs {
+    int n_agents, cap, B;
+    const float* ring;
+    uint32_t range;
+    uint64_t seed, counter;
+    int32_t* idx;
+    float *s, *a, *r, *s2;
+    const uint64_t* seeds;
+    int E, M;
+    f16x8 *xfs, *xfs2;
+};
+struct SampleFrontArgs {
+    PrepArgs pa;
+    SampleArgs sa;
+    float* grads;
+    long n_grads;
+    int n_sets, n_scale, n_prep1, n_zero;
+};
+template <int S, bool G>
+__global__ __launch_bounds__(256) void sample_front_kernel(const SampleFrontArgs a) {
+    int b = blockIdx.x;
+    if (front_small_roles(a.pa, a.grads, a.n_grads, a.n_sets, a.n_scale, a.n_prep1, a.n_zero, b)) return;
+    const SampleArgs& q = a.sa;
+    bool nf = false;
+    replay_sample_body<S, G>((long)b * 256 + threadIdx.x, q.n_agents, q.cap, q.B, q.ring, q.range, q.seed, q.counter, q.idx, q.s, q.a, q.r,
+                             q.s2, q.seeds, q.E, q.M, [&](long base, const float(&v)[4][2 * S + 2]) {
+#pragma unroll
+        for (int k = 0; k < 4; ++k) {
+            float x[4], x2[4];
+#pragma unroll
+            for (int j = 0; j < 4; ++j) x[j] = j < S ? v[k][j] : 0.f, x2[j] = j < S ? v[k][S + 2 + j] : 0.f;
+            const float ea = v[k][S], er = v[k][S + 1];
+            nf = nf || not_finite(x[0]) || not_finite(x[1]) || not_finite(x[2]) || not_finite(x[3]);
+            nf = nf || fmaxf(fmaxf(fabsf(x[0]), fabsf(x[1])), fmaxf(fabsf(x[2]), fabsf(x[3]))) >= F16_OVERFLOW;
+            nf = nf || not_finite(ea) || fabsf(ea) >= F16_OVERFLOW;
+            nf = nf || not_finite(x2[0]) || not_finite(x2[1]) || not_finite(x2[2]) || not_finite(x2[3]);
+            nf = nf || fmaxf(fmaxf(fabsf(x2[0]), fabsf(x2[1])), fmaxf(fabsf(x2[2]), fabsf(x2[3]))) >= F16_OVERFLOW;
+            nf = nf || not_finite(er);
+            const long ri = base + k;
+#pragma unroll
+            for (int h = 0; h < 2; ++h)
+                q.xfs[2 * ri + h] = make_xh(x[0], x[1], x[2], x[3], h), q.xfs2[2 * ri + h] = make_xh(x2[0], x2[1], x2[2], x2[3], h);
+        }
+    });
+    front_flag(a.pa.fflag + 4 * ((long)a.n_prep1 + b), nf);
 }
 
 enum HeadMode { OUT_TANH = 0, OUT_TD = 1, HEAD_BOTH = 5, OUT_TANH_SAVE = 6 };
@@ -1317,6 +1370,7 @@
     size_t Whi[4], Wlo[4], Wchi[2], Wclo[2], wf1h[4], vec[4], wap, a2, y, mu, dmu, g3, sm, sma, tz, t1p, s2raw, xfs, xfs2, partHs[3], partM[2],
         partV[2], partG[2], bad, smax, fflag, total;
     int n_prep1, n_pack, n_fflag;
+    int n_samp, n_fflag_s;
 };
 static Plan make_plan(int n_agents, int n_sets) {
     Plan pl;
@@ -1356,9 +1410,10 @@
     for (int i = 0; i < 3; ++i) pl.partHs[i] = take(4 * (size_t)pl.grid * 8 * 2);
     pl.n_prep1 = (NGT_MAX * 4 * n_sets + 3) / 4, pl.n_pack = (int)((2 * rows + 255) / 256);
     pl.n_fflag = 4 * (pl.n_prep1 + 2 * pl.n_pack);
+    pl.n_samp = (int)((rows / 4 + 255) / 256), pl.n_fflag_s = 4 * (pl.n_prep1 + pl.n_samp);
     pl.bad = take(sizeof(int));
     pl.smax = take(sizeof(unsigned) * 4 * (size_t)n_sets * SCALE_SLICES * 2);
-    pl.fflag = take(sizeof(unsigned) * (size_t)pl.n_fflag);
+    pl.fflag = take(sizeof(unsigned) * (size_t)(pl.n_fflag > pl.n_fflag_s ? pl.n_fflag : pl.n_fflag_s));
     pl.total = o;
     return pl;
 }
@@ -1375,21 +1430,30 @@
     return AVD_OK;
 }
 
-enum Phase { PH_CRITIC = 1, PH_ACTOR = 2, PH_BOTH = 3 };
-template <int S, class... H>
-static int run(int phases, const avd_mlp_layout& L, int n_agents, int n_sets, const float* theta, const float* stats, const float* theta_t,
-               const float* stats_t, const float* s, const float* a, const float* r, const float* s2, const float* aw, float gamma,
-               float high, float* grads, float* losses, unsigned char* ws, const Plan& pl, hipStream_t st, H... hp) {
-    PrepArgs pa;
+enum Phase { PH_CRITIC = 1, PH_ACTOR = 2, PH_BOTH = 3, PH_PREPARED = 4 };
+static void fill_prep_args(PrepArgs& pa, const avd_mlp_layout& L, int S, const float* theta, const float* stats, const float* theta_t,
+                           const float* stats_t, unsigned char* ws, const Plan& pl) {
     pa.L = L, pa.S = S, pa.theta = theta, pa.stats = stats, pa.theta_t = theta_t, pa.stats_t = stats_t;
     pa.wap = (unsigned*)(ws + pl.wap), pa.bad = (int*)(ws + pl.bad), pa.smax = (unsigned*)(ws + pl.smax);
     pa.fflag = (unsigned*)(ws + pl.fflag), pa.n_fflag = pl.n_fflag;
+    for (int i = 0; i < 4; ++i) {
+        pa.Whi[i] = (f16*)(ws + pl.Whi[i]), pa.Wlo[i] = (f16*)(ws + pl.Wlo[i]), pa.vec[i] = (float*)(ws + pl.vec[i]);
+        pa.wf1h[i] = (f16x8*)(ws + pl.wf1h[i]);
+        pa.Wchi[i] = i < 2 ? (f16*)(ws + pl.Wchi[i]) : nullptr, pa.Wclo[i] = i < 2 ? (f16*)(ws + pl.Wclo[i]) : nullptr;
+    }
+}
+template <int S, class... H>
+static int run(int phases_in, const avd_mlp_layout& L, int n_agents, int n_sets, const float* theta, const float* stats, const float* theta_t,
+               const float* stats_t, const float* s, const float* a, const float* r, const float* s2, const float* aw, float gamma,
+               float high, float* grads, float* losses, unsigned char* ws, const Plan& pl, hipStream_t st, H... hp) {
+    const int phases = phases_in & PH_BOTH;
+    const bool prepared = phases_in & PH_PREPARED;
+    PrepArgs pa;
+    fill_prep_args(pa, L, S, theta, stats, theta_t, stats_t, ws, pl);
+    if (prepared) pa.n_fflag = pl.n_fflag_s;
     NetP net[4];
     for (int i = 0; i < 4; ++i) {
         const bool critic = i & 1, target = i >= 2;
-        pa.Whi[i] = (f16*)(ws + pl.Whi[i]), pa.Wlo[i] = (f16*)(ws + pl.Wlo[i]), pa.vec[i] = (float*)(ws + pl.vec[i]);
-        pa.wf1h[i] = (f16x8*)(ws + pl.wf1h[i]);
-        pa.Wchi[i] = i < 2 ? (f16*)(ws + pl.Wchi[i]) : nullptr, pa.Wclo[i] = i < 2 ? (f16*)(ws + pl.Wclo[i]) : nullptr;
         NetP& n = net[i];
         n.th = (target ? theta_t : theta) + (critic ? L.actor_size : 0), n.th_stride = L.theta_size;
         n.Whi = pa.Whi[i], n.Wlo = pa.Wlo[i], n.Wchi = pa.Wchi[i], n.Wclo = pa.Wclo[i], n.wf1h = pa.wf1h[i], n.vec = pa.vec[i];
@@ -1436,12 +1500,14 @@
         fa.partG[i] = F(pl.partG[i]), fa.c3[i] = F(pl.vec[i]);
     fa.t1_from_g[0] = fa.t1_from_g[1] = 1, fa.t1p = F(pl.t1p), fa.s2raw = F(pl.s2raw);
     if (phases & PH_CRITIC) {
-        FrontArgs fr;
-        fr.pa = pa, fr.grads = grads, fr.n_grads = (long)n_sets * L.theta_size, fr.n_sets = n_sets;
-        fr.pk.x[0] = s, fr.pk.extra[0] = a, fr.pk.outh[0] = xfs, fr.pk.x[1] = s2, fr.pk.extra[1] = r, fr.pk.outh[1] = xfs2, fr.pk.rows = nrows;
-        fr.n_scale = 4 * n_sets * SCALE_SLICES, fr.n_prep1 = pl.n_prep1, fr.n_pack = pl.n_pack;
-        fr.n_zero = (int)((fr.n_grads + ZERO_PER_BLOCK - 1) / ZERO_PER_BLOCK);
-        hipLaunchKernelGGL(front_kernel<S>, dim3((unsigned)(fr.n_scale + fr.n_prep1 + fr.n_zero + 2 * fr.n_pack)), dim3(256), 0, st, fr);
+        if (!prepared) {
+            FrontArgs fr;
+            fr.pa = pa, fr.grads = grads, fr.n_grads = (long)n_sets * L.theta_size, fr.n_sets = n_sets;
+            fr.pk.x[0] = s, fr.pk.extra[0] = a, fr.pk.outh[0] = xfs, fr.pk.x[1] = s2, fr.pk.extra[1] = r, fr.pk.outh[1] = xfs2, fr.pk.rows = nrows;
+            fr.n_scale = 4 * n_sets * SCALE_SLICES, fr.n_prep1 = pl.n_prep1, fr.n_pack = pl.n_pack;
+            fr.n_zero = (int)((fr.n_grads + ZERO_PER_BLOCK - 1) / ZERO_PER_BLOCK);
+            hipLaunchKernelGGL(front_kernel<S>, dim3((unsigned)(fr.n_scale + fr.n_prep1 + fr.n_zero + 2 * fr.n_pack)), dim3(256), 0, st, fr);
+        }
         hipLaunchKernelGGL(prep_kernel, dim3(H2, 4, n_sets), dim3(320), 0, st, pa);
         head(head_kernel<S, ActorS, OUT_TANH>, 2, xfs2, nullptr, nullptr, nullptr, a2, nullptr);
         if constexpr (sizeof...(H) > 0)
@@ -1477,6 +1543,22 @@
     return check_launch("avd_learn_set_split");
 }
 
+
+template <int S, bool G>
+static int sample_front(const avd_mlp_layout& L, int n_agents, int n_sets, const SampleArgs& sa, const float* theta, const float* stats,
+                        const float* theta_t, const float* stats_t, float* grads, unsigned char* ws, const Plan& pl, hipStream_t st,
+                        const char* who) {
+    SampleFrontArgs fr;
+    fill_prep_args(fr.pa, L, S, theta, stats, theta_t, stats_t, ws, pl);
+    fr.pa.n_fflag = pl.n_fflag_s;
+    fr.sa = sa, fr.sa.xfs = (f16x8*)(ws + pl.xfs), fr.sa.xfs2 = (f16x8*)(ws + pl.xfs2);
+    fr.grads = grads, fr.n_grads = (long)n_sets * L.theta_size, fr.n_sets = n_sets;
+    fr.n_scale = 4 * n_sets * SCALE_SLICES, fr.n_prep1 = pl.n_prep1;
+    fr.n_zero = (int)((fr.n_grads + ZERO_PER_BLOCK - 1) / ZERO_PER_BLOCK);
+    hipLaunchKernelGGL((sample_front_kernel<S, G>), dim3((unsigned)(fr.n_scale + fr.n_prep1 + fr.n_zero + pl.n_samp)), dim3(256), 0, st, fr);
+    return check_launch(who);
+}
+
 }
 }
 
@@ -1504,6 +1586,50 @@
     AVD_REQUIRE(bytes, "avd_learn_set_split_workspace: null pointer");
     *bytes = fsplit::make_plan(n_agents, n_sets).total;
     return AVD_OK;
+}
+
+static int sample_front_entry(const char* who, const avd_mlp_layout* lay, int n_agents, int n_sets, int cap, const float* ring, int range,
+                              uint64_t seed, const uint64_t* d_seeds, int n_groups, int M, uint64_t counter, int32_t* idx, float* s, float* a,
+                              float* r, float* s2, const float* theta, const float* stats, const float* theta_t, const float* stats_t,
+                              float* grads, void* workspace, size_t workspace_bytes, void* stream) {
+    int rc = fsplit::check_shape(lay, n_agents, n_sets, who);
+    if (rc) return rc;
+    AVD_REQUIRE(cap > 0 && range > 0 && range <= cap, "%s: cap=%d range=%d", who, cap, range);
+    AVD_REQUIRE(ring && idx && s && a && r && s2 && theta && stats && theta_t && stats_t && grads && workspace, "%s: null pointer", who);
+    const fsplit::Plan pl = fsplit::make_plan(n_agents, n_sets);
+    AVD_REQUIRE(workspace_bytes >= pl.total, "%s: workspace %zu B < %zu B", who, workspace_bytes, pl.total);
+    fsplit::SampleArgs sa;
+    sa.n_agents = n_agents, sa.cap = cap, sa.B = lay->B, sa.ring = ring, sa.range = (uint32_t)range, sa.seed = seed, sa.counter = counter;
+    sa.idx = idx, sa.s = s, sa.a = a, sa.r = r, sa.s2 = s2, sa.seeds = d_seeds, sa.E = n_groups, sa.M = M, sa.xfs = sa.xfs2 = nullptr;
+    unsigned char* ws = (unsigned char*)workspace;
+    hipStream_t st = (hipStream_t)stream;
+    if (lay->S == 4)
+        return d_seeds ? fsplit::sample_front<4, true>(*lay, n_agents, n_sets, sa, theta, stats, theta_t, stats_t, grads, ws, pl, st, who)
+                       : fsplit::sample_front<4, false>(*lay, n_agents, n_sets, sa, theta, stats, theta_t, stats_t, grads, ws, pl, st, who);
+    return d_seeds ? fsplit::sample_front<3, true>(*lay, n_agents, n_sets, sa, theta, stats, theta_t, stats_t, grads, ws, pl, st, who)
+                   : fsplit::sample_front<3, false>(*lay, n_agents, n_sets, sa, theta, stats, theta_t, stats_t, grads, ws, pl, st, who);
+}
+
+extern "C" int avd_replay_sample_split_front_f32(const avd_mlp_layout* lay, int n_agents, int n_sets, int cap, const float* ring, int range,
+                                                 uint64_t seed, uint64_t counter, int32_t* idx, float* s, float* a, float* r, float* s2,
+                                                 const float* theta, const float* stats, const float* theta_t, const float* stats_t,
+                                                 float* grads, void* workspace, size_t workspace_bytes, void* stream) {
+    return sample_front_entry("avd_replay_sample_split_front_f32", lay, n_agents, n_sets, cap, ring, range, seed, nullptr, 1, 1, counter, idx,
+                              s, a, r, s2, theta, stats, theta_t, stats_t, grads, workspace, workspace_bytes, stream);
+}
+
+extern "C" int avd_replay_sample_seeds_split_front_f32(const avd_mlp_layout* lay, int n_agents, int n_sets, int cap, const float* ring,
+                                                       int range, const uint64_t* d_seeds, int n_groups, int agents_per_platoon,
+                                                       uint64_t counter, int32_t* idx, float* s, float* a, float* r, float* s2,
+                                                       const float* theta, const float* stats, const float* theta_t, const float* stats_t,
+                                                       float* grads, void* workspace, size_t workspace_bytes, void* stream) {
+    AVD_REQUIRE(d_seeds && n_groups >= 1 && agents_per_platoon >= 1 && n_agents > 0 &&
+                    n_agents % ((long)n_groups * agents_per_platoon) == 0,
+                "avd_replay_sample_seeds_split_front_f32: d_seeds=%p n_groups=%d agents_per_platoon=%d n=%d (n must be a multiple of "
+                "n_groups x agents_per_platoon)", (const void*)d_seeds, n_groups, agents_per_platoon, n_agents);
+    return sample_front_entry("avd_replay_sample_seeds_split_front_f32", lay, n_agents, n_sets, cap, ring, range, 0, d_seeds, n_groups,
+                              agents_per_platoon, counter, idx, s, a, r, s2, theta, stats, theta_t, stats_t, grads, workspace,
+                              workspace_bytes, stream);
 }
 
 template <class... H>
@@ -1563,3 +1689,30 @@
     return split_entry(fsplit::PH_ACTOR, "avd_learn_set_split_actor", lay, n_agents, n_sets, theta, stats, nullptr, nullptr, s, nullptr, nullptr,
                        nullptr, nullptr, 0.f, high, grads, nullptr, workspace, workspace_bytes, stream);
 }
+
+extern "C" int avd_learn_set_split_prepared_f16x3(const avd_mlp_layout* lay, int n_agents, int n_sets, const float* theta, const float* stats,
+                                                   const float* theta_t, const float* stats_t, const float* s, const float* a,
+                                                   const float* r, const float* s2, const float* agent_weight, float gamma, float high,
+                                                   float* grads, float* losses, void* workspace, size_t workspace_bytes, void* stream) {
+    return split_entry(fsplit::PH_BOTH | fsplit::PH_PREPARED, "avd_learn_set_split_prepared_f16x3", lay, n_agents, n_sets, theta, stats, theta_t,
+                       stats_t, s, a, r, s2, agent_weight, gamma, high, grads, losses, workspace, workspace_bytes, stream);
+}
+
+extern "C" int avd_learn_set_split_hp_prepared_f16x3(const avd_mlp_layout* lay, int n_agents, int n_sets, const float* theta,
+                                                      const float* stats, const float* theta_t, const float* stats_t, const float* s,
+                                                      const float* a, const float* r, const float* s2, const float* agent_weight, float high,
+                                                      float* grads, float* losses, void* workspace, size_t workspace_bytes,
+                                                      const avd_hparams* d_hp, int n_groups, int set_block, void* stream) {
+    AVD_REQUIRE_HP("avd_learn_set_split_hp_prepared_f16x3", d_hp, n_groups, set_block, n_sets);
+    return split_entry(fsplit::PH_BOTH | fsplit::PH_PREPARED, "avd_learn_set_split_hp_prepared_f16x3", lay, n_agents, n_sets, theta, stats,
+                       theta_t, stats_t, s, a, r, s2, agent_weight, 0.f, high, grads, losses, workspace, workspace_bytes, stream,
+                       HpRef{d_hp, n_groups, set_block});
+}
+
+extern "C" int avd_learn_set_split_critic_prepared(const avd_mlp_layout* lay, int n_agents, int n_sets, const float* theta, const float* stats,
+                                                   const float* theta_t, const float* stats_t, const float* s, const float* a,
+                                                   const float* r, const float* s2, const float* agent_weight, float gamma, float high,
+                                                   float* grads, float* losses, void* workspace, size_t workspace_bytes, void* stream) {
+    return split_entry(fsplit::PH_CRITIC | fsplit::PH_PREPARED, "avd_learn_set_split_critic_prepared", lay, n_agents, n_sets, theta, stats,
+                       theta_t, stats_t, s, a, r, s2, agent_weight, gamma, high, grads, losses, workspace, workspace_bytes, stream);
+}
diff --git a/avddpg_amd/csrc/replay.hip b/avddpg_amd/csrc/replay.hip
--- a/avddpg_amd/csrc/replay.hip
+++ b/avddpg_amd/csrc/replay.hip
@@ -1,4 +1,5 @@
 #include "common.h"
+#include "replay_sample.h"
 
 namespace avd {
 
@@ -64,45 +65,9 @@
                                                             float* __restrict__ a, float* __restrict__ r,
                                                             float* __restrict__ s2, const uint64_t* __restrict__ seeds, int E,
                                                             int M) {
-    constexpr int row = 2 * S + 2;
     const long t = (long)blockIdx.x * blockDim.x + threadIdx.x;
-    const long total = (long)n_agents * B, base = t * 4;
-    if (base >= total) return;
-    const int ag = (int)(base / B);
-    uint64_t key = seed;
-    uint32_t ti = (uint32_t)t;
-    if constexpr (G) {
-        const int g = ag / M, e = g % E;
-        key = seeds[e];
-        ti = (uint32_t)(((long)(g / E) * M + (ag - g * M)) * (B / 4) + (base - (long)ag * B) / 4);
-    }
-    const u32x4 rr = philox_at(key, counter, ti, STREAM_REPLAY);
-    const uint32_t w[4] = {rr.x, rr.y, rr.z, rr.w};
-    int ix[4];
-    float v[4][row];
-#pragma unroll
-    for (int k = 0; k < 4; ++k) {
-        ix[k] = (int32_t)(((uint64_t)w[k] * range) >> 32);
-        const float2* src = (const float2*)(ring + ((long)ag * cap + ix[k]) * row);
-#pragma unroll
-        for (int j = 0; j < row / 2; ++j) {
-            const float2 q = src[j];
-            v[k][2 * j] = q.x, v[k][2 * j + 1] = q.y;
-        }
-    }
-    *(int4*)(idx + base) = make_int4(ix[0], ix[1], ix[2], ix[3]);
-    *(float4*)(a + base) = make_float4(v[0][S], v[1][S], v[2][S], v[3][S]);
-    *(float4*)(r + base) = make_float4(v[0][S + 1], v[1][S + 1], v[2][S + 1], v[3][S + 1]);
-#pragma unroll
-    for (int k = 0; k < 4; ++k) {
-        if (S == 4) {
-            *(float4*)(s + (base + k) * 4) = make_float4(v[k][0], v[k][1], v[k][2], v[k][3]);
-            *(float4*)(s2 + (base + k) * 4) = make_float4(v[k][6], v[k][7], v[k][8], v[k][9]);
-        } else {
-#pragma unroll
-            for (int j = 0; j < S; ++j) s[(base + k) * S + j] = v[k][j], s2[(base + k) * S + j] = v[k][S + 2 + j];
-        }
-    }
+    replay_sample_body<S, G>(t, n_agents, cap, B, ring, range, seed, counter, idx, s, a, r, s2, seeds, E, M,
+                             [](long, const float(&)[4][2 * S + 2]) {});
 }
 
 }
diff --git a/avddpg_amd/csrc/replay_sample.h b/avddpg_amd/csrc/replay_sample.h
--- /dev/null
+++ b/avddpg_amd/csrc/replay_sample.h
@@ -0,0 +1,54 @@
+#pragma once
+#include "common.h"
+
+namespace avd {
+
+template <int S, bool G, class F>
+__device__ __forceinline__ void replay_sample_body(long t, int n_agents, int cap, int B, const float* __restrict__ ring,
+                                                   uint32_t range, uint64_t seed, uint64_t counter,
+                                                   int32_t* __restrict__ idx, float* __restrict__ s,
+                                                   float* __restrict__ a, float* __restrict__ r,
+                                                   float* __restrict__ s2, const uint64_t* __restrict__ seeds, int E,
+                                                   int M, F&& rows) {
+    constexpr int row = 2 * S + 2;
+    const long total = (long)n_agents * B, base = t * 4;
+    if (base >= total) return;
+    const int ag = (int)(base / B);
+    uint64_t key = seed;
+    uint32_t ti = (uint32_t)t;
+    if constexpr (G) {
+        const int g = ag / M, e = g % E;
+        key = seeds[e];
+        ti = (uint32_t)(((long)(g / E) * M + (ag - g * M)) * (B / 4) + (base - (long)ag * B) / 4);
+    }
+    const u32x4 rr = philox_at(key, counter, ti, STREAM_REPLAY);
+    const uint32_t w[4] = {rr.x, rr.y, rr.z, rr.w};
+    int ix[4];
+    float v[4][row];
+#pragma unroll
+    for (int k = 0; k < 4; ++k) {
+        ix[k] = (int32_t)(((uint64_t)w[k] * range) >> 32);
+        const float2* src = (const float2*)(ring + ((long)ag * cap + ix[k]) * row);
+#pragma unroll
+        for (int j = 0; j < row / 2; ++j) {
+            const float2 q = src[j];
+            v[k][2 * j] = q.x, v[k][2 * j + 1] = q.y;
+        }
+    }
+    *(int4*)(idx + base) = make_int4(ix[0], ix[1], ix[2], ix[3]);
+    *(float4*)(a + base) = make_float4(v[0][S], v[1][S], v[2][S], v[3][S]);
+    *(float4*)(r + base) = make_float4(v[0][S + 1], v[1][S + 1], v[2][S + 1], v[3][S + 1]);
+#pragma unroll
+    for (int k = 0; k < 4; ++k) {
+        if (S == 4) {
+            *(float4*)(s + (base + k) * 4) = make_float4(v[k][0], v[k][1], v[k][2], v[k][3]);
+            *(float4*)(s2 + (base + k) * 4) = make_float4(v[k][6], v[k][7], v[k][8], v[k][9]);
+        } else {
+#pragma unroll
+            for (int j = 0; j < S; ++j) s[(base + k) * S + j] = v[k][j], s2[(base + k) * S + j] = v[k][S + 2 + j];
+        }
+    }
+    rows(base, v);
+}
+
+}
diff --git a/avddpg_amd/trainer.py b/avddpg_amd/trainer.py
--- a/avddpg_amd/trainer.py
+++ b/avddpg_amd/trainer.py
@@ -198,6 +198,8 @@
         if self.overlap_allreduce and not can_overlap:
             raise ValueError("overlap_allreduce needs a process group and shared_engine='fused3' (the two-phase learn call)")
         self._side = None
+        self._sample_front = bool(self.shared and self.shared_engine == "fused3" and rng == "device" and self.A == 1
+                                  and self.S in (3, 4) and conf.batch_size == lay.B)
         self._xbuf = None
         self._flag_exchanged = False
         ws = 1
@@ -332,6 +334,9 @@
                 self.ep_reward += reward
             if not self.replay.buffer_counter > conf.batch_size:
                 return None
+            if self._sample_front and "sample" not in vars(self.replay):
+                self._set_buffers()
+                return self.agents.sample_split_front(self.replay, self.set_grads)
             return self.replay.sample()
 
         batch = self._timed("replay", replay_part)
@@ -377,13 +382,17 @@
         self._timed("learn", self.agents.learn, s, a, r, s2, self.set_mod, grads=self.grads, losses=self.losses)
         self._timed("update", self._update, ep, i, fed)
 
+    def _set_buffers(self):
+        if getattr(self, "set_grads", None) is None:
+            from .dist import set_exchange_buffer
+            M = self.Mf
+            self._xbuf, self.set_grads = set_exchange_buffer(M, self.agents.lay.theta_size, self.device)
+            self.set_losses = torch.zeros(M, 2, dtype=torch.float32, device=self.device)
+
     def _learn_batched(self, s, a, r, s2, weights=None):
         P, M, B = self.Pf, self.Mf, self.conf.batch_size
         sm = lambda x: x.view(P, M, *x.shape[1:]).transpose(0, 1).reshape(M, P * B, *x.shape[2:]).contiguous()
-        if getattr(self, "set_grads", None) is None:
-            from .dist import set_exchange_buffer
-            self._xbuf, self.set_grads = set_exchange_buffer(M, self.agents.lay.theta_size, self.device)
-            self.set_losses = torch.zeros(M, 2, dtype=torch.float32, device=self.device)
+        self._set_buffers()
         carry = self.env.any_done if (self.group is not None and self.auto_reset is True) else None
         rw = wsum = aw_dev = None
         if isinstance(weights, str):
@@ -397,7 +406,8 @@
                 self._flag_exchanged = carry is not None
                 return
             self.agents.learn_set_fused(s, a, r, s2, P * M, grads=self.set_grads, losses=self.set_losses, agent_weight=aw,
-                                        split=self.shared_engine == "fused3")
+                                        split=self.shared_engine == "fused3",
+                                        prepared=self._sample_front and self.agents.front_prepared_for(s, self.set_grads, P * M))
         else:
             if aw_dev is not None:
                 rw = aw_dev.view(P, M).transpose(0, 1).reshape(M, P, 1).expand(M, P, B).reshape(M, P * B).contiguous()
@@ -422,8 +432,10 @@
             self._side = dict(stream=torch.cuda.Stream(device=self.device), ready=torch.cuda.Event(),
                               crit=torch.empty(M, T - A, **f32), act=torch.empty(M * A + M + 1, **f32))
         scale = float(P) if wsum is None else wsum.view(M, 1)
+        prepared = self._sample_front and self.agents.front_prepared_for(s, self.set_grads, P * M)
         learn = lambda phase: self.agents.learn_set_fused(s, a, r, s2, P * M, grads=self.set_grads, losses=self.set_losses,
-                                                          agent_weight=aw, split=True, phase=phase)
+                                                          agent_weight=aw, split=True, phase=phase,
+                                                          prepared=prepared and phase == "critic")
         learn("critic")
         exchange_two_phase(self.set_grads, A, scale, wsum, self.total_platoons, self.group, self._side,
                            lambda: learn("actor"), timers=self.timers, flag=flag)
diff --git a/avddpg_amd/vec.py b/avddpg_amd/vec.py
--- a/avddpg_amd/vec.py
+++ b/avddpg_amd/vec.py
@@ -481,8 +481,48 @@
              self.high, ptr(grads), ptr(losses), ptr(ws), ws.numel(), stream_handle())
         return grads
 
-    def learn_set_fused(self, s, a, r, s2, n_agents, grads=None, losses=None, agent_weight=None, split=False, phase=None):
+    def _split_workspace(self, n_agents):
         import ctypes
+        need = ctypes.c_size_t(0)
+        call("avd_learn_set_split_workspace", self._layp, n_agents, self.n_sets, ctypes.byref(need))
+        ws = getattr(self, "_fsplit_ws", None)
+        if ws is None or ws.numel() < need.value:
+            ws = self._fsplit_ws = torch.empty(need.value, dtype=torch.uint8, device=self.device)
+        return ws
+
+    def sample_split_front(self, replay, grads):
+        lay = self.lay
+        if (replay.rng == "host" or (replay.S, replay.A, replay.B) != (lay.S, lay.A, lay.B) or lay.A != 1 or lay.S not in (3, 4)
+                or replay.n % self.n_sets):
+            raise _hip.AvdError("sample_split_front: needs device-side sampling of the learner's own shape (A = 1, S in {3, 4}, the layout's "
+                                f"batch size), got rng={replay.rng!r} S={replay.S} A={replay.A} B={replay.B} n={replay.n}")
+        if tuple(grads.shape) != (self.n_sets, lay.theta_size) or grads.dtype != torch.float32 or not grads.is_contiguous():
+            raise _hip.AvdError(f"sample_split_front: grads must be contiguous float32 {(self.n_sets, lay.theta_size)}")
+        ws = self._split_workspace(replay.n)
+        tail = (replay.samples, ptr(replay.idx), ptr(replay.s), ptr(replay.a), ptr(replay.r), ptr(replay.s2), ptr(self.theta),
+                ptr(self.stats), ptr(self.theta_t), ptr(self.stats_t), ptr(grads), ptr(ws), ws.numel(), stream_handle())
+        if replay.seeds is not None:
+            call("avd_replay_sample_seeds_split_front_f32", self._layp, replay.n, self.n_sets, replay.cap, ptr(replay.ring),
+                 replay.sample_range(), ptr(replay.d_seeds), len(replay.seeds), replay.agents_per_platoon, *tail)
+        else:
+            call("avd_replay_sample_split_front_f32", self._layp, replay.n, self.n_sets, replay.cap, ptr(replay.ring),
+                 replay.sample_range(), replay.seed, *tail)
+        replay.samples += 1
+        self._front = (ws.data_ptr(), grads.data_ptr(), replay.n, replay.s.data_ptr())
+        return replay.s, replay.a, replay.r, replay.s2
+
+    def front_prepared_for(self, s, grads, n_agents):
+        ws = getattr(self, "_fsplit_ws", None)
+        return (getattr(self, "_front", None) is not None and ws is not None and grads is not None
+                and self._front == (ws.data_ptr(), grads.data_ptr(), n_agents, s.data_ptr()))
+
+    def learn_set_fused(self, s, a, r, s2, n_agents, grads=None, losses=None, agent_weight=None, split=False, phase=None, prepared=False):
+        import ctypes
+        if prepared:
+            if not split or phase == "actor" or not self.front_prepared_for(s, grads, n_agents):
+                raise _hip.AvdError("learn_set_fused(prepared=True): no sample_split_front on this batch, slab and workspace precedes the call")
+        if split and phase != "actor":
+            self._front = None
         if self.hp is not None and not (split and phase is None):
             self._no_hp("learn_set_fused (bf16 operands, or a phase of the split call)")
         self._check_agent_major(s, a, r, s2, n_agents, agent_weight)
@@ -506,11 +546,15 @@
             raise _hip.AvdError(f"phase={phase!r}")
         if self.hp is not None:
             tbl, E, blk = self.hp
-            call("avd_learn_set_split_hp_f16x3", self._layp, n_agents, self.n_sets, ptr(self.theta), ptr(self.stats), ptr(self.theta_t),
+            call("avd_learn_set_split_hp_prepared_f16x3" if prepared else "avd_learn_set_split_hp_f16x3", self._layp, n_agents, self.n_sets, ptr(self.theta), ptr(self.stats), ptr(self.theta_t),
                  ptr(self.stats_t), ptr(s), ptr(a), ptr(r), ptr(s2), ptr(agent_weight), self.high, ptr(grads), ptr(losses), ptr(ws),
                  ws.numel(), ptr(tbl), E, blk, stream_handle())
             return grads
-        call("avd_learn_set_split_critic" if phase == "critic" else fn, self._layp, n_agents, self.n_sets, ptr(self.theta), ptr(self.stats),
+        if prepared:
+            fn = "avd_learn_set_split_critic_prepared" if phase == "critic" else "avd_learn_set_split_prepared_f16x3"
+        elif phase == "critic":
+            fn = "avd_learn_set_split_critic"
+        call(fn, self._layp, n_agents, self.n_sets, ptr(self.theta), ptr(self.stats),
              ptr(self.theta_t), ptr(self.stats_t), ptr(s), ptr(a), ptr(r), ptr(s2), ptr(agent_weight), self.config.gamma, self.high,
              ptr(grads), ptr(losses), ptr(ws), ws.numel(), stream_handle())
         return grads
diff --git a/include/avddpg_hip.h b/include/avddpg_hip.h
--- a/include/avddpg_hip.h
+++ b/include/avddpg_hip.h
@@ -241,6 +241,29 @@
                                const float* s2, const float* agent_weight, float gamma, float high, float* grads, float* losses,
                                void* workspace, size_t workspace_bytes, void* stream);
 
+int avd_replay_sample_split_front_f32(const avd_mlp_layout* lay, int n_agents, int n_sets, int cap, const float* ring, int range,
+                                      uint64_t seed, uint64_t counter, int32_t* idx, float* s, float* a, float* r, float* s2,
+                                      const float* theta, const float* stats, const float* theta_t, const float* stats_t, float* grads,
+                                      void* workspace, size_t workspace_bytes, void* stream);
+int avd_replay_sample_seeds_split_front_f32(const avd_mlp_layout* lay, int n_agents, int n_sets, int cap, const float* ring, int range,
+                                            const uint64_t* d_seeds, int n_groups, int agents_per_platoon, uint64_t counter,
+                                            int32_t* idx, float* s, float* a, float* r, float* s2, const float* theta,
+                                            const float* stats, const float* theta_t, const float* stats_t, float* grads,
+                                            void* workspace, size_t workspace_bytes, void* stream);
+int avd_learn_set_split_prepared_f16x3(const avd_mlp_layout* lay, int n_agents, int n_sets, const float* theta, const float* stats,
+                                       const float* theta_t, const float* stats_t, const float* s, const float* a, const float* r,
+                                       const float* s2, const float* agent_weight, float gamma, float high, float* grads, float* losses,
+                                       void* workspace, size_t workspace_bytes, void* stream);
+int avd_learn_set_split_hp_prepared_f16x3(const avd_mlp_layout* lay, int n_agents, int n_sets, const float* theta, const float* stats,
+                                          const float* theta_t, const float* stats_t, const float* s, const float* a, const float* r,
+                                          const float* s2, const float* agent_weight, float high, float* grads, float* losses,
+                                          void* workspace, size_t workspace_bytes, const avd_hparams* d_hp, int n_groups, int set_block,
+                                          void* stream);
+int avd_learn_set_split_critic_prepared(const avd_mlp_layout* lay, int n_agents, int n_sets, const float* theta, const float* stats,
+                                        const float* theta_t, const float* stats_t, const float* s, const float* a, const float* r,
+                                        const float* s2, const float* agent_weight, float gamma, float high, float* grads,
+                                        float* losses, void* workspace, size_t workspace_bytes, void* stream);
+
 int avd_actor_forward_shared_workspace(const avd_mlp_layout* lay, int n_agents, int n_sets, size_t* bytes);
 int avd_actor_forward_shared_bf16(const avd_mlp_layout* lay, int n_agents, int n_sets, const float* theta,
                                   const float* stats, const float* state, float high, float* out, void* workspace,
```

New measurement: 2.084 million. -1.2%, worse.
